# Ashish424/G.P.U-PathTracer

Hardware: AMD Instinct MI355X
Metric: Mrays/sec, cornell_dragon 1920x1080 (+ achieved GB/s against the memory roofline) (higher is better)
Workload: dtype f32; 1 GPU; cornell_dragon_800k (800032 tris) 1920x1080 depth 4 diff + reference 8-sphere room, 16 spp per step; kernel=auto, parallelism=1 GPU, closed_scene=True

## Files before the change

g.p.u-pathtracer_amd/_abi.py:

```python
import ctypes as C
import os

_HERE = os.path.dirname(os.path.abspath(__file__))
PTMI_PATH = os.environ.get("PT_LIBPTMI") or os.path.join(_HERE, "csrc", "libptmi.so")
PTHOST_PATH = os.path.join(_HERE, "host", "libpthost.so")


class Camera(C.Structure):
    _fields_ = [("pos", C.c_float * 3), ("front", C.c_float * 3), ("right", C.c_float * 3),
                ("up", C.c_float * 3), ("dist", C.c_float), ("aspect", C.c_float),
                ("fov", C.c_float), ("_pad", C.c_float)]


class Sphere(C.Structure):
    _fields_ = [("pos_rad", C.c_float * 4), ("emi", C.c_float * 3), ("col", C.c_float * 3),
                ("mat", C.c_int32)]


class Material(C.Structure):
    _fields_ = [("col", C.c_float * 3), ("emi", C.c_float * 3), ("mat", C.c_int32), ("phong_expo", C.c_float)]


class DenoiseParams(C.Structure):
    _fields_ = [("width", C.c_int32), ("height", C.c_int32), ("iterations", C.c_int32),
                ("sigma_color", C.c_float), ("sigma_normal", C.c_float), ("sigma_position", C.c_float)]


class TemporalParams(C.Structure):
    _fields_ = [("width", C.c_int32), ("height", C.c_int32), ("max_history", C.c_float),
                ("plane_tolerance", C.c_float), ("normal_threshold", C.c_float), ("_pad", C.c_int32)]


class Environment(C.Structure):
    _fields_ = [("width", C.c_int32), ("height", C.c_int32), ("front", C.c_float * 3), ("right", C.c_float * 3),
                ("up", C.c_float * 3), ("scale", C.c_float * 3), ("filter", C.c_int32), ("_pad", C.c_int32)]


class CheckpointInfo(C.Structure):
    _fields_ = [("width", C.c_int32), ("height", C.c_int32), ("next_frame", C.c_uint64),
                ("constant_pdf", C.c_uint64), ("scene_tag", C.c_uint64)]


class Params(C.Structure):
    _fields_ = [("width", C.c_int32), ("height", C.c_int32), ("depth", C.c_uint32),
                ("cull_backfaces", C.c_int32), ("frame", C.c_uint64), ("sample_index", C.c_uint64),
                ("tri_mat", C.c_int32), ("tri_col", C.c_float * 3), ("tri_emi", C.c_float * 3),
                ("bk_color", C.c_float * 3), ("air_ior", C.c_float), ("glass_ior", C.c_float),
                ("phong_expo", C.c_float), ("flags", C.c_uint32),
                ("part_index", C.c_int32), ("part_count", C.c_int32), ("part_rows", C.c_int32),
                ("_pad", C.c_int32)]


class Counters(C.Structure):
    _fields_ = [("rays", C.c_uint64), ("inner", C.c_uint64), ("tris", C.c_uint64),
                ("leaves", C.c_uint64), ("hits", C.c_uint64), ("paths", C.c_uint64)]


class BuildParams(C.Structure):
    _fields_ = [("max_leaf_size", C.c_int32), ("min_leaf_size", C.c_int32), ("max_depth", C.c_int32),
                ("n_bins", C.c_int32), ("sah_node_cost", C.c_float), ("sah_tri_cost", C.c_float),
                ("split_alpha", C.c_float), ("n_spatial_bins", C.c_int32), ("optimize_passes", C.c_int32)]


class BvhStats(C.Structure):
    _fields_ = [("n_inner", C.c_uint64), ("n_leaves", C.c_uint64), ("n_tri_refs", C.c_uint64),
                ("max_depth", C.c_uint32), ("sah_cost", C.c_float), ("build_ms", C.c_double),
                ("opt_cost_before", C.c_float), ("opt_cost_after", C.c_float)]


MAT_DIFF, MAT_METAL, MAT_SPEC, MAT_REFR = 0, 1, 2, 3
FLAG_METAL_LITERAL_W = 1 << 0
FLAG_WRITE_RGBA = 1 << 1
FLAG_FACE_FORWARD, FLAG_COSINE_DIFF, FLAG_GLASS_FIX, FLAG_RUSSIAN_ROULETTE, FLAG_MISS_KEEPS_PATH = 1 << 2, 1 << 3, 1 << 4, 1 << 5, 1 << 6
FLAG_RR_CPU_TRACER = 1 << 7
FLAG_NEE = 1 << 8
FLAGS_SMALLPT = FLAG_FACE_FORWARD | FLAG_COSINE_DIFF | FLAG_RUSSIAN_ROULETTE | FLAG_MISS_KEEPS_PATH
FLAGS_CPU_TRACER = FLAG_FACE_FORWARD | FLAG_COSINE_DIFF | FLAG_RR_CPU_TRACER | FLAG_MISS_KEEPS_PATH
RAYS_CLAMPED, RAYS_HDR = 0, 1
ENV_NEAREST, ENV_BILINEAR = 0, 1
KERNEL_AUTO, KERNEL_MEGA_BVH2, KERNEL_PERSISTENT, KERNEL_WAVEFRONT = 0, 1, 3, 5
OPT_KERNEL, OPT_COUNTERS, OPT_TIMING, OPT_BATCH, OPT_TOP_NODES, OPT_OCCUPANCY, OPT_LDS_STACK, OPT_WALK, OPT_LEAF_MAX, OPT_TRI_TEST, OPT_REFILL, OPT_VOTE_NODE, OPT_VOTE_REC, OPT_WAVE_BATCH, OPT_SPHERE_LDS, OPT_BUILD_ALGO, OPT_REBUILD, OPT_PRESPLIT, OPT_WAVE_BLOCKS, OPT_OVERLAP, OPT_OPTIMIZE, OPT_WAVE_SAMPLES = 1, 2, 3, 4, 5, 6, 7, 8, 9, 10, 11, 12, 13, 14, 15, 16, 17, 18, 19, 21, 24, 25
OPT_FIRST_WALK, OPT_PACKET_STACK, OPT_FUSE_STAGES, OPT_LAST_ANYHIT = 26, 27, 28, 29
OPT_ROOT_CULL = 30
OPT_ROOT_ENTRY = 33
OPT_PATH_HISTORY = 34
OPT_ENV_LIGHT = 35

_vp, _sz, _i, _u32 = C.c_void_p, C.c_size_t, C.c_int, C.c_uint32
PTMI_SYMBOLS = [
    ("pt_abi_version", _i, []),
    ("pt_device_count", _i, []),
    ("pt_create", _i, [_i, C.POINTER(_vp)]),
    ("pt_destroy", _i, [_vp]),
    ("pt_last_error", C.c_char_p, [_vp]),
    ("pt_set_stream", _i, [_vp, _vp]),
    ("pt_set_option", _i, [_vp, _i, _i]),
    ("pt_sync", _i, [_vp]),
    ("pt_malloc", _i, [_vp, _sz, C.POINTER(_vp)]),
    ("pt_free", _i, [_vp, _vp]),
    ("pt_memset", _i, [_vp, _vp, _i, _sz]),
    ("pt_download", _i, [_vp, _vp, _vp, _sz]),
    ("pt_upload", _i, [_vp, _vp, _vp, _sz]),
    ("pt_upload_bvh", _i, [_vp, _vp, _sz, _vp, _sz, _vp, _sz]),
    ("pt_upload_spheres", _i, [_vp, C.POINTER(Sphere), _sz]),
    ("pt_render", _i, [_vp, _vp, _vp, C.POINTER(Camera), C.POINTER(Params), _u32]),
    ("pt_render_moments", _i, [_vp, _vp, _vp, _vp, C.POINTER(Camera), C.POINTER(Params), _u32]),
    ("pt_frame_error", _i, [_vp, _vp, C.c_int32, C.c_int32, C.c_uint64, C.c_float, C.POINTER(C.c_double), C.POINTER(C.c_uint64)]),
    ("pt_trace_rays", _i, [_vp, _vp, _sz, _i, _vp, _vp, _vp]),
    ("pt_closest_hits", _i, [_vp, _vp, _sz, _i, _vp, _vp, _vp]),
    ("pt_any_hits", _i, [_vp, _vp, _sz, _i, _vp]),
    ("pt_render_rays", _i, [_vp, _vp, _sz, C.c_uint64, _vp, C.POINTER(Params), _u32, _i]),
    ("pt_upload_environment", _i, [_vp, C.POINTER(Environment), _vp]),
    ("pt_eval_environment", _i, [_vp, _vp, _sz, _vp]),
    ("pt_environment_is_light", _i, [_vp, C.POINTER(_i)]),
    ("pt_sample_environment", _i, [_vp, _vp, _sz, _vp, _vp]),
    ("pt_environment_pdf", _i, [_vp, _vp, _sz, _vp]),
    ("pt_render_aux", _i, [_vp, C.POINTER(Camera), C.POINTER(Params), _vp, _vp, _vp, _vp]),
    ("pt_denoise", _i, [_vp, C.POINTER(DenoiseParams), _vp, _vp, _vp, _vp, _vp, _vp]),
    ("pt_temporal", _i, [_vp, C.POINTER(TemporalParams), C.POINTER(Camera), _vp, _vp, _vp, _vp, _vp, _vp, _vp, _vp, _vp, _vp, _vp, _vp]),
    ("pt_build_bvh", _i, [_vp, _vp, C.c_size_t, _vp, C.c_size_t]),
    ("pt_last_build_ms", _i, [_vp, C.POINTER(C.c_float)]),
    ("pt_refit_bvh", _i, [_vp, _vp, _sz, _vp]),
    ("pt_upload_tri_materials", _i, [_vp, C.POINTER(Material), C.c_size_t, C.POINTER(C.c_int32), C.c_size_t]),
    ("pt_get_counters", _i, [_vp, C.POINTER(Counters)]),
    ("pt_get_wave_stats", _i, [_vp, C.POINTER(C.c_uint64), _i]),
    ("pt_last_kernel_ms", _i, [_vp, C.POINTER(C.c_float)]),
    ("pt_get_stage_ms", _i, [_vp, C.POINTER(C.c_float), _i]),
    ("pt_auto_choice", _i, [_vp, C.POINTER(C.c_int), C.POINTER(C.c_float), C.POINTER(C.c_float)]),
    ("pt_tree_cost", _i, [_vp, C.POINTER(C.c_double), C.POINTER(C.c_double)]),
    ("pt_tree_items", _i, [_vp, C.POINTER(_vp), C.POINTER(C.c_uint64), C.POINTER(C.c_uint64), C.POINTER(C.c_uint64), C.POINTER(C.c_uint32)]),
    ("pt_scene_info", _i, [_vp, C.POINTER(C.c_uint64), C.POINTER(C.c_uint64), C.POINTER(C.c_uint64),
                           C.POINTER(C.c_uint32), C.POINTER(C.c_uint64)]),
]

PTHOST_SYMBOLS = [
    ("pth_last_error", C.c_char_p, []),
    ("pth_default_build_params", None, [C.POINTER(BuildParams)]),
    ("pth_mesh_create", _vp, [_vp, _sz, _vp, _sz]),
    ("pth_mesh_load_obj", _vp, [C.c_char_p]),
    ("pth_mesh_load_ptmesh", _vp, [C.c_char_p]),
    ("pth_mesh_append", _i, [_vp, _vp, _vp]),
    ("pth_mesh_n_verts", _sz, [_vp]),
    ("pth_mesh_n_tris", _sz, [_vp]),
    ("pth_mesh_verts", _vp, [_vp]),
    ("pth_mesh_tris", _vp, [_vp]),
    ("pth_mesh_bounds", None, [_vp, C.POINTER(C.c_float * 3), C.POINTER(C.c_float * 3)]),
    ("pth_mesh_save_ptmesh", _i, [_vp, C.c_char_p]),
    ("pth_mesh_n_materials", _sz, [_vp]),
    ("pth_mesh_materials", _vp, [_vp]),
    ("pth_mesh_tri_materials", _vp, [_vp]),
    ("pth_mesh_set_materials", _i, [_vp, C.POINTER(Material), _sz, _vp]),
    ("pth_mesh_free", None, [_vp]),
    ("pth_bvh_build", _vp, [_vp, C.POINTER(BuildParams)]),
    ("pth_bvh_nodes", _vp, [_vp]),
    ("pth_bvh_n_node_vec4", _sz, [_vp]),
    ("pth_bvh_tris", _vp, [_vp]),
    ("pth_bvh_n_tri_vec4", _sz, [_vp]),
    ("pth_bvh_index", _vp, [_vp]),
    ("pth_bvh_n_index", _sz, [_vp]),
    ("pth_bvh_get_stats", None, [_vp, C.POINTER(BvhStats)]),
    ("pth_bvh_free", None, [_vp]),
    ("pth_write_ppm", _i, [C.c_char_p, _vp, _i, _i]),
    ("pth_write_png", _i, [C.c_char_p, _vp, _i, _i]),
    ("pth_write_pfm", _i, [C.c_char_p, _vp, _i, _i]),
    ("pth_read_pfm", _i, [C.c_char_p, C.POINTER(_i), C.POINTER(_i), C.POINTER(_vp)]),
    ("pth_free_pfm", None, [_vp]),
    ("pth_checkpoint_save", _i, [C.c_char_p, C.POINTER(CheckpointInfo), _vp]),
    ("pth_checkpoint_load", _i, [C.c_char_p, C.POINTER(CheckpointInfo), _vp]),
    ("pth_frame_hash", C.c_uint64, [C.c_uint64]),
]


def _load(path, symbols):
    if not os.path.exists(path):
        raise ImportError(f"{path} is missing - run `python -c 'import __graft_entry__ as g; g.build()'` "
                          "(there is no CPU or PyTorch fallback for the path tracer)")
    lib = C.CDLL(path, mode=C.RTLD_GLOBAL)
    for name, res, args in symbols:
        fn = getattr(lib, name)
        fn.restype = res
        fn.argtypes = args
    return lib


_ptmi = None
_pthost = None


def ptmi():
    global _ptmi
    if _ptmi is None:
        _ptmi = _load(PTMI_PATH, PTMI_SYMBOLS)
    return _ptmi


def pthost():
    global _pthost
    if _pthost is None:
        _pthost = _load(PTHOST_PATH, PTHOST_SYMBOLS)
    return _pthost
```

g.p.u-pathtracer_amd/csrc/pt_ctx.h:

```cpp
#pragma once
#include <hip/hip_runtime.h>

#include <algorithm>
#include <climits>
#include <cstdint>
#include <cstring>
#include <string>
#include <type_traits>
#include <vector>

#include "../../include/ptmi.h"
#include "pt_kernels.h"

#ifndef PT_FIRST_WALK_DEFAULT
#define PT_FIRST_WALK_DEFAULT 1
#endif

struct TreeState {
    float4* d_nodes = nullptr;
    bool records_woop = false;
    bool has_bvh = false;
    uint64_t wide_root = 0;
    uint64_t n_wide = 0, n_inner = 0, n_refs = 0, n_leaves = 0, scene_bytes = 0;
    uint32_t wide_top_layout = 0, wide_depth = 0;
    uint32_t n_top_layout = 0;
    uint32_t max_depth = 0;
    int32_t max_tri_id = -1;
    float build_ms = -1.f;
    double opt_cost[2] = {0.0, 0.0};
};

struct DevTree {
    TreeState s;
    DevTree() = default;
    DevTree(DevTree&& o) noexcept : s(o.release()) {}
    DevTree& operator=(DevTree&& o) noexcept {
        if (this != &o) { (void)hipFree(s.d_nodes); s = o.release(); }
        return *this;
    }
    ~DevTree() { (void)hipFree(s.d_nodes); }
    TreeState release() { const TreeState r = s; s = TreeState(); return r; }
};

struct pt_ctx {
    int device = 0;
    hipStream_t own_stream = nullptr;
    hipStream_t stream = nullptr;
    hipEvent_t switch_ev = nullptr;
    std::string err;
    TreeState tree;
    pt_sphere_d* d_spheres = nullptr;
    int* d_tri_matid = nullptr;
    float4* d_mat_table = nullptr;
    size_t n_tri_matid = 0;
    std::vector<int32_t> emissive_ids;
    int32_t* d_light_slot = nullptr;
    float4* d_tri_lights = nullptr;
    uint64_t mat_gen = 0, lights_key = ~0ull;
    uint64_t lights_geom = 0;
    hipEvent_t lights_ev = nullptr;
    uint64_t lights_gen = 0;
    int n_spheres = 0;
    pt_sphere_d h_spheres[PT_KSPHERES];
    KEnv env = {};
    uint64_t env_gen = 0;
    int opt_kernel = PT_KERNEL_AUTO;
    int opt_counters = 0;
    int opt_timing = 0;
    unsigned long long* d_counters = nullptr;
    unsigned int* d_queue = nullptr;
    float* d_samples = nullptr;
    size_t samples_bytes = 0;
    int n_cu = 0;
    int opt_batch = 36;
    int opt_presplit = 0;
    int opt_optimize = 0;
    int opt_rebuild = 0;
    int opt_build_algo = 1;
    int opt_sph_lds = 1;
    int opt_vote_node = 1, opt_vote_rec = 1;
    int opt_refill = 8;
    int opt_top = 64;
    int opt_occ = 6;
    int opt_lstk = 16;
    int opt_walk = 2;
    int opt_leaf_max = 2;
    int opt_tri_test = 0;
    void* d_wave = nullptr;
    size_t wave_bytes = 0;
    int opt_wave_batch = 16;
    int opt_wave_samples = 16;
    int opt_wave_blocks = 8;
    int opt_first_walk = PT_FIRST_WALK_DEFAULT;
    int opt_packet_stack = PT_PACKET_STACK_MAX;
    int opt_fuse_stages = 1;
    int opt_last_anyhit = 1;
    int opt_root_cull = 1;
    int opt_root_entry = 1;
    int opt_env_light = 0;
    int opt_path_history = 1;
    struct AutoPick {
        static constexpr int TRIALS = 4, PENDING = 4, DECIDED = 5;
        uint64_t key = 0;
        int phase = 0;
        int choice = PT_KERNEL_PERSISTENT;
        hipEvent_t e[2 * TRIALS] = {nullptr, nullptr, nullptr, nullptr, nullptr, nullptr, nullptr, nullptr};
        float ms[2] = {0.f, 0.f};
        uint64_t used = 0;
    };
    static constexpr int N_PICKS = 8;
    AutoPick picks[N_PICKS];
    int pick_last = -1;
    uint64_t pick_tick = 0;
    uint64_t scene_gen = 0;
    uint64_t geom_gen = 0;
    hipEvent_t geom_ev = nullptr;
    struct Refit {
        uint64_t scene_gen = 0;
        const float4* items = nullptr;
        void* d_mem = nullptr;
        int4* bin_list = nullptr;
        int4* wide_list = nullptr;
        float* bin_box = nullptr;
        float* wide_box = nullptr;
        float* rec_box = nullptr;
        uint32_t* first_use = nullptr;
        std::vector<uint32_t> bin_off, wide_off;
    } refit;
    void* d_denoise = nullptr;
    size_t denoise_bytes = 0;
    void* d_frame_err = nullptr;
    size_t frame_err_bytes = 0;
    int opt_overlap = 1;
    struct Side {
        hipStream_t stream = nullptr;
        hipEvent_t traced = nullptr, folded = nullptr;
        bool fold_pending = false;
        float* samples = nullptr;
        size_t samples_bytes = 0;
        unsigned int* queue = nullptr;
        uint64_t lights_seen = 0;
        uint64_t geom_seen = 0;
    } side[2];
    int side_next = 0;
    hipEvent_t ev0 = nullptr, ev1 = nullptr;
    bool timed = false;
    std::vector<hipEvent_t> stage_ev;
    std::vector<int> stage_kind;
    size_t stage_used = 0;
};

namespace ptmi {

extern thread_local std::string g_err;

inline int fail(pt_ctx* c, int code, const std::string& msg) {
    if (c) c->err = msg;
    g_err = msg;
    return code;
}
inline int hip_fail(pt_ctx* c, hipError_t e, const char* what) {
    return fail(c, PT_ERR_DEVICE, std::string(what) + ": " + hipGetErrorString(e));
}

struct DevTemp {
    std::vector<void*> ptrs;
    ~DevTemp() { for (void* p : ptrs) (void)hipFree(p); }
    template <class T> hipError_t get(T** out, size_t count) {
        void* p = nullptr;
        const hipError_t e = hipMalloc(&p, std::max<size_t>(count, 1) * sizeof(T));
        if (e == hipSuccess) ptrs.push_back(p);
        *out = (T*)p;
        return e;
    }
};

inline size_t lds_fit(int& n_top, int stack_n, int block) {
    const size_t stack = (size_t)stack_n * block * 4;
    while (n_top > 0 && (size_t)n_top * 64 + stack > 160 * 1024) n_top /= 2;
    return (size_t)n_top * 64 + stack;
}

template <typename K>
hipError_t allow_lds(K kernel, size_t bytes) {
    return hipFuncSetAttribute((const void*)kernel, hipFuncAttributeMaxDynamicSharedMemorySize, (int)bytes);
}

inline bool wide_walk_fits(const TreeState& t, int cap) { return t.has_bvh && 3 * t.wide_depth + 2 <= (uint32_t)cap; }
inline int choose_walk(pt_ctx* c, const char* who, bool postponed) {
    const bool wide_ok = wide_walk_fits(c->tree, PT_STACK_CAP);
    if (c->tree.has_bvh && c->tree.records_woop)
        return wide_ok ? 3 : fail(c, PT_ERR_UNSUPPORTED, std::string(who) + ": Woop records need the wide walk and this tree is too deep for it");
    const int walk = c->opt_walk == 4 && !postponed ? 2 : c->opt_walk;
    return walk >= 2 && !wide_ok ? 1 : walk;
}
inline bool path_history_holds(const KParams& P) {
    if ((P.flags & (PT_FLAG_NEE | PT_FLAG_RUSSIAN_ROULETTE | PT_FLAG_RR_CPU_TRACER)) || P.tri_matid || P.sc.n_spheres > PT_KSPHERES ||
        P.tri_mat == PT_MAT_REFR || P.depth > PT_HIST_MAX_DEPTH)
        return false;
    for (int i = 0; i < P.sc.n_spheres; i++)
        if (P.ksph[i].mat == PT_MAT_REFR) return false;
    return true;
}
inline void scene_view(const pt_ctx* c, KScene& sc, pt_sphere_d* ksph = nullptr) {
    sc = KScene();
    sc.nodes = sc.tris = c->tree.d_nodes;
    sc.has_bvh = c->tree.has_bvh ? 1 : 0;
    sc.wide_root = (int)c->tree.wide_root;
    if (!ksph) return;
    sc.spheres = c->d_spheres; sc.n_spheres = c->n_spheres;
    std::memcpy(ksph, c->h_spheres, sizeof c->h_spheres);
}
inline size_t binary_ray_layout(const pt_ctx* c, KScene& sc) {
    sc.stack_n = PT_STACK_CAP; sc.top_base = 0;
    sc.n_top = (int)std::min<uint32_t>((uint32_t)c->opt_top, c->tree.n_top_layout);
    return lds_fit(sc.n_top, sc.stack_n, PT_BLOCK_RAYS);
}
constexpr size_t QUEUE_BYTES = PT_SHARDS * PT_SHARD_STRIDE * sizeof(unsigned int);
inline hipError_t queue_alloc(unsigned int** q) { return hipMalloc((void**)q, QUEUE_BYTES); }
inline hipError_t queue_reset(unsigned int* q, hipStream_t st) { return hipMemsetAsync(q, 0, QUEUE_BYTES, st); }
inline int queue_chunk(const pt_ctx* c, uint64_t slots) {
    const uint64_t waves = (uint64_t)c->n_cu * 20;
    return slots / 64 >= 4 * waves ? 64 : (slots / 32 >= 4 * waves ? 32 : 16);
}
inline void queue_params(const pt_ctx* c, unsigned int* queue, KParams& P) {
    P.queue = queue; P.batch = c->opt_batch;
    P.refill = std::min(c->opt_refill, c->opt_batch);
    P.vote_node = c->opt_vote_node; P.vote_rec = c->opt_vote_rec;
}
inline int lds_sphere_table(size_t& lds) { lds += 15 * PT_KSPHERES * 4; return (int)(lds / 4) - 15 * PT_KSPHERES; }
inline hipError_t span_begin(pt_ctx* c) { return c->opt_timing ? hipEventRecord(c->ev0, c->stream) : hipSuccess; }
inline hipError_t span_end(pt_ctx* c) {
    const hipError_t e = c->opt_timing ? hipEventRecord(c->ev1, c->stream) : hipSuccess;
    if (c->opt_timing && e == hipSuccess) c->timed = true;
    return e;
}

template <int V> constexpr std::integral_constant<int, V> int_c{};
template <class F>
auto with_bool(bool v, F&& f) { return v ? f(std::true_type{}) : f(std::false_type{}); }
template <int V0, int... Vs, class F>
auto with_int(int v, F&& f) {
    if constexpr (sizeof...(Vs) == 0) return f(int_c<V0>);
    else return v == V0 ? f(int_c<V0>) : with_int<Vs...>(v, f);
}

template <class K, class... A>
hipError_t launch_resident(K kernel, size_t lds, int max_per_cu, int n_cu, size_t work_cap, hipStream_t st, const A&... args) {
    int per_cu = 0;
    const hipError_t e = allow_lds(kernel, lds);
    if (e != hipSuccess) return e;
    if (hipOccupancyMaxActiveBlocksPerMultiprocessor(&per_cu, kernel, PT_BLOCK, lds) != hipSuccess || per_cu < 1) per_cu = 1;
    per_cu = std::min(per_cu, max_per_cu);
    hipLaunchKernelGGL(kernel, dim3((unsigned)std::min<size_t>((size_t)per_cu * n_cu, work_cap)), dim3(PT_BLOCK), lds, st, args...);
    return hipGetLastError();
}

struct LaunchCfg {
    bool count;
    int occ;
    int lstk;
    int walk;
    size_t lds;
    int blocks;
    int work_blocks;
    int n_cu;
    bool moments;
    int env;
};
hipError_t launch_mega(const LaunchCfg& L, const KParams& P, hipStream_t st);
hipError_t launch_rays(const KScene& sc, size_t lds, const float4* rays, size_t n, int cull, float* t_out, int* tri_out,
                       float* n_out, hipStream_t st);
hipError_t launch_persist(const LaunchCfg& L, const KParams& P, hipStream_t st);
hipError_t launch_fold(const KParams& P, float2* moments, hipStream_t st);
int render_wavefront(pt_ctx* c, KParams& P, const LaunchCfg& L, int work_tiles, bool& folded);
inline uint32_t wave_sample_group_log2(uint32_t spp, int cap) {
    for (int k = 6; k >= 2; k--)
        if ((1 << k) <= cap && (spp & ((1u << k) - 1u)) == 0u) return (uint32_t)k;
    return 0u;
}
int wave_reserve(pt_ctx* c, const KParams& P, int work_tiles);
struct QueryCall {
    const float* rays;
    size_t n;
    int cull;
    float* t;
    int32_t* tri;
    float* normal;
    uint8_t* hit;
};
hipError_t launch_query(pt_ctx* c, const QueryCall& q);
struct RaysCall {
    const float* rays;
    float* out;
    uint64_t first_index;
    size_t n;
    int hdr;
};
hipError_t launch_render_rays(const pt_ctx* c, int walk, bool nee, size_t lds, int work_blocks, const KParams& P, const RaysCall& r);
hipError_t launch_fold_rays(const pt_ctx* c, const KParams& P, const RaysCall& r);
int stage_mark(pt_ctx* c, int kind_of_work_since_last_mark);
int build_bvh_impl(pt_ctx* c, const float* verts, size_t n_verts, const int32_t* tris, size_t n_tris, DevTree& out,
                   const int32_t* id_map = nullptr);
void refit_release(pt_ctx* c);
void denoise_release(pt_ctx* c);
void env_release(pt_ctx* c);

}

#define HIP_TRY(ctx, call)                                                \
    do {                                                                  \
        hipError_t e_ = (call);                                           \
        if (e_ != hipSuccess) return ptmi::hip_fail((ctx), e_, #call);    \
    } while (0)
```

g.p.u-pathtracer_amd/csrc/pt_k_wave.hip:

```cpp
#include "pt_ctx.h"

__device__ __forceinline__ int wf_block_rank(bool keep, int& total, int* s_cnt) {
    const unsigned long long m = __ballot(keep);
    const int w = threadIdx.x >> 6;
    const int in_wave = (int)__builtin_amdgcn_mbcnt_hi((uint32_t)(m >> 32), __builtin_amdgcn_mbcnt_lo((uint32_t)m, 0u));
    if ((threadIdx.x & 63) == 0) s_cnt[w] = __popcll(m);
    __syncthreads();
    int base = 0, tot = 0;
#pragma unroll
    for (int k = 0; k < PT_BLOCK / 64; k++) {
        const int c = s_cnt[k];
        if (k < w) base += c;
        tot += c;
    }
    total = tot;
    return base + in_wave;
}

constexpr int WF_TRI_ROW = 15 * PT_KSPHERES - 4;
template <bool HIST = false>
__device__ __forceinline__ void wf_sphere_table() {
    if (threadIdx.x < 11 * PT_KSPHERES) {
        PT_KARGS(K);
        const float v = ((const __attribute__((address_space(4))) float*)&K.ksph[0])[threadIdx.x];
        ((float*)s_dyn)[threadIdx.x] = v;
        if (threadIdx.x % 11 < 4) ((float*)s_dyn)[88 + 4 * (threadIdx.x / 11) + threadIdx.x % 11] = v;
    }
    if (HIST && threadIdx.x >= 128 && threadIdx.x < 134) {
        PT_KARGS(K);
        const int k = (int)threadIdx.x - 128;
        ((float*)s_dyn)[WF_TRI_ROW + (k < 3 ? 7 + k : 1 + k)] = ((const __attribute__((address_space(4))) float*)&K.tri_col[0])[k];
    }
    __syncthreads();
}

__device__ __forceinline__ const float* wf_history_row(uint32_t code) {
    return (const float*)s_dyn + (code == PT_HIST_TRI ? (uint32_t)WF_TRI_ROW : 11u * code);
}
__device__ __forceinline__ void wf_history_replay(uint32_t word, uint32_t n, v3& mask, v3& accu) {
    mask = V3(1.f, 1.f, 1.f);
    accu = V3(0.f, 0.f, 0.f);
    for (uint32_t k = 0; k < n; k++) {
        const float* t = wf_history_row(pt_hist_code(word, k));
        accu = vadd(accu, vmul(mask, V3(t[4], t[5], t[6])));
        mask = vmul(mask, V3(t[7], t[8], t[9]));
    }
}

__global__ void __launch_bounds__(256) k_wf_prepare(const KParams P) {
    for (uint32_t i = threadIdx.x; i < P.spp; i += 256) P.wf.hashes[i] = pt_wang64(P.frame + i);
    for (uint32_t i = threadIdx.x; i < P.wf.queues_words; i += 256) P.wf.queues_all[i] = 0u;
}

__device__ __forceinline__ bool wf_slot_pixel(const KParams& P, uint32_t slot, uint32_t& s_idx, int& px, int& py) {
    if (slot >= P.wf.n_slots) return false;
    return pt_slot_pixel(P, slot, s_idx, px, py);
}

__device__ __forceinline__ float wf_anyhit_start(float ts) {
    return ts < PT_F32_MAX ? __uint_as_float(__float_as_uint(ts) + 1u) : ts;
}

template <bool COUNT, int OCC, int LSTK, bool FIRST, bool ANY = false, bool ENTRY = false>
__global__ void __launch_bounds__(PT_BLOCK, OCC) k_wf_extend(const KParams P) {
    static_assert(!(FIRST && ENTRY), "bounce 0's rays come from the camera: nobody ran their root step");
    const int tid = threadIdx.x;
    const int lane = tid & 63;
    TravOverflow<LSTK> stk_ovf;
    TravStack<LSTK, PT_BLOCK> stk(__builtin_amdgcn_readfirstlane(tid & ~63), stk_ovf);
    const bool cull = P.cull != 0;
    const uint32_t n_regions = (uint32_t)P.wf.n_regions;
    const uint32_t shard_regions = (n_regions + PT_SHARDS - 1) / PT_SHARDS;
    const int batch = P.batch;

    uint32_t next = 0, end = 0;
    bool empty = false;
    int shard = (int)(blockIdx.x & (PT_SHARDS - 1));

    bool live = false;
    uint32_t idx = 0;
    v3 o = V3(0.f, 0.f, 0.f), d = V3(0.f, 0.f, 0.f);
    TravState ts;
    ts.idx = ts.idy = ts.idz = ts.oodx = ts.oody = ts.oodz = 0.f;
    ts.node = PT_SENTINEL; ts.leaf = 0; ts.sp = 0;
    ts.h = pt_no_hit();
    TravCount tc;
    uint32_t n_rays = 0, it_begin = 0, act_begin = 0, it_loop = 0;
    int root_l0 = 0, root_l1 = 0, root_l2 = 0, root_l3 = 0;
    if (ENTRY) {
        const float4 q2 = pt_uld4(P.sc.nodes, P.sc.wide_root + 2), q3 = pt_uld4(P.sc.nodes, P.sc.wide_root + 3);
        root_l0 = __float_as_int(q2.z); root_l1 = __float_as_int(q2.w);
        root_l2 = __float_as_int(q3.x); root_l3 = __float_as_int(q3.y);
    }

    for (;;) {
        if (COUNT) it_loop++;
        const unsigned long long idle = __ballot(!live);
        const int n_idle = __popcll(idle);
        if (!empty && (n_idle >= batch || n_idle == 64)) {
            const uint32_t rank = __builtin_amdgcn_mbcnt_hi((uint32_t)(idle >> 32), __builtin_amdgcn_mbcnt_lo((uint32_t)idle, 0u));
            uint32_t served = 0;
            for (int round = 0; round < 8 && served < (uint32_t)n_idle; round++) {
                if (next == end) {
                    bool got = false;
                    for (int tries = 0; tries < PT_SHARDS && !got; tries++) {
                        uint32_t k = 0;
                        if (lane == 0) k = atomicAdd(P.wf.queue + shard * PT_SHARD_STRIDE, 1u);
                        k = (uint32_t)__builtin_amdgcn_readfirstlane((int)k);
                        const uint32_t r = k * PT_SHARDS + (uint32_t)shard;
                        if (k < shard_regions && r < n_regions) {
                            next = r * PT_REGION;
                            if (FIRST) end = min(next + (uint32_t)PT_REGION, P.wf.n_slots);
                            else end = next + (uint32_t)__builtin_amdgcn_readfirstlane(P.wf.walk_in[r]);
                            got = true;
                        } else {
                            shard = (shard + 1) & (PT_SHARDS - 1);
                        }
                    }
                    if (!got) { empty = true; break; }
                }
                const uint32_t take = min((uint32_t)n_idle - served, end - next);
                if (!live && rank >= served && rank < served + take) {
                    idx = next + (rank - served);
                    float bound = PT_F32_MAX, b_w = 0.f;
                    if (FIRST) {
                        uint32_t s_idx = 0;
                        int px = 0, py = 0;
                        if (wf_slot_pixel(P, idx, s_idx, px, py)) {
                            PathState ps;
                            path_begin_hashed(P, px, py, (uint64_t)((uint32_t)py * (uint32_t)P.W + (uint32_t)px), P.wf.hashes[s_idx], ps);
                            o = ps.o;
                            d = ps.d;
                            live = true;
                        }
                    } else {
                        const float4 a = pt_sld4(P.wf.ray0_in + idx), b = pt_sld4(P.wf.ray1_in + idx);
                        if (ANY) bound = pt_sld1((const float*)(P.wf.hit + idx));
                        o = V3(a.x, a.y, a.z);
                        d = V3(a.w, b.x, b.y);
                        b_w = b.w;
                        live = true;
                    }
                    if (live) trav_begin(ts, o, d, stk, P.sc.wide_root);
                    if (ANY) ts.h.t = wf_anyhit_start(bound);
                    if constexpr (ENTRY) {
                        const uint32_t code = __float_as_uint(b_w) >> PT_REC_ENTRY_SHIFT, n = pt_entry_count(code);
                        auto link = [&](uint32_t k) {
                            const uint32_t c = pt_entry_child(code, k);
                            return c == 0u ? root_l0 : (c == 1u ? root_l1 : (c == 2u ? root_l2 : root_l3));
                        };
                        if (n == 4u) { ts.sp++; stk.put(ts.sp, link(3)); }
                        if (n >= 3u) { ts.sp++; stk.put(ts.sp, link(2)); }
                        if (n >= 2u) { ts.sp++; stk.put(ts.sp, link(1)); }
                        ts.node = link(0);
                        if (COUNT && ts.node < 0) tc.leaves++;
                    }
                }
                next += take;
                served += take;
            }
            if (COUNT && served) { it_begin++; act_begin += served; }
        }
        const unsigned long long busy = __ballot(live);
        if (!busy) {
            if (empty) break;
            continue;
        }
        const int n_dead = empty ? 64 - __popcll(busy) : 0;
        if (live) {
            const bool fin = trav_run_wide<COUNT, true, false, true, ANY>(ts, P.sc, o, d, cull, stk, tc, n_dead, batch);
            if (fin) {
                if (ANY) { if (ts.h.t == 0.0f) pt_sst1((float*)(P.wf.hit + idx), 0.0f); }
                else pt_sst2(P.wf.hit + idx, make_float2(ts.h.t, __int_as_float(ts.h.rec)));
                live = false;
                if (COUNT) n_rays++;
            }
        }
    }

    if (COUNT) {
        const uint32_t w_ovf = wave_sum_u32(stk.n_ovf), w_rays = ANY ? wave_sum_u32(n_rays) : 0u;
        pt_book_walk<true>(P, lane == 0, n_rays, tc);
        if (lane == 0) {
            if (ANY) atomicAdd(&P.counters[PT_CNT_ANY_RAYS], (unsigned long long)w_rays);
            atomicAdd(&P.counters[PT_CNT_IT_BEGIN], (unsigned long long)it_begin);
            atomicAdd(&P.counters[PT_CNT_ACT_BEGIN], (unsigned long long)act_begin);
            atomicAdd(&P.counters[PT_CNT_IT_LOOP], (unsigned long long)it_loop);
            atomicAdd(&P.counters[PT_CNT_STACK_OVF], (unsigned long long)w_ovf);
        }
    }
}

template <bool COUNT>
__global__ void __launch_bounds__(PT_BLOCK, 8) k_wf_extend_packet(const KParams P) {
    const uint32_t n_groups = P.wf.n_slots / 64u;
    const uint32_t stride = gridDim.x * (uint32_t)(PT_BLOCK / 64);
    TravCount tc;
    uint32_t n_rays = 0, n_walked = 0;
    for (uint32_t group = (uint32_t)__builtin_amdgcn_readfirstlane((int)(blockIdx.x * (PT_BLOCK / 64) + (threadIdx.x >> 6)));
         group < n_groups; group += stride) {
        const uint32_t slot = group * 64u + (threadIdx.x & 63u);
        uint32_t s_idx = 0;
        int px = 0, py = 0;
        v3 o = V3(0.f, 0.f, 0.f), d = V3(0.f, 0.f, 0.f);
        const bool in = wf_slot_pixel(P, slot, s_idx, px, py);
        if (in) {
            PathState ps;
            path_begin_hashed(P, px, py, (uint64_t)((uint32_t)py * (uint32_t)P.W + (uint32_t)px), P.wf.hashes[s_idx], ps);
            o = ps.o;
            d = ps.d;
        }
        const Hit h = trav_packet_wide<COUNT>(P.sc, o, d, P.cull != 0, in, tc);
        if (in) pt_sst2(P.wf.hit + slot, make_float2(h.t, __int_as_float(h.rec)));
        if (COUNT) { n_rays += in ? 1u : 0u; n_walked++; }
    }
    if (COUNT && n_walked) {
        pt_book_walk<true>(P, (threadIdx.x & 63) == 0, n_rays, tc);
        if ((threadIdx.x & 63) == 0) atomicAdd(&P.counters[PT_CNT_PACKET_GROUPS], (unsigned long long)n_walked);
    }
}

#ifndef PT_SURVIVOR_RANK
#define PT_SURVIVOR_RANK(P, alive, ps, total, s_cnt) wf_block_rank(alive, total, s_cnt)
#endif

template <bool FIRST>
__device__ __forceinline__ void wf_shade_miss(float* smp, v3 mask) {
    PT_KARGS(K);
    if (FIRST && (K.flags & PT_FLAG_MISS_KEEPS_PATH)) {
        smp[0] = 0.f + mask.x * K.bk[0]; smp[1] = 0.f + mask.y * K.bk[1]; smp[2] = 0.f + mask.z * K.bk[2];
    } else if (K.flags & PT_FLAG_MISS_KEEPS_PATH) {
        smp[0] += mask.x * K.bk[0]; smp[1] += mask.y * K.bk[1]; smp[2] += mask.z * K.bk[2];
    } else {
        smp[0] = K.bk[0]; smp[1] = K.bk[1]; smp[2] = K.bk[2];
    }
}
__device__ __forceinline__ void wf_shade_miss_history(float* smp, v3 accu, v3 mask) {
    PT_KARGS(K);
    if (K.flags & PT_FLAG_MISS_KEEPS_PATH) pt_sst3(smp, V3(accu.x + mask.x * K.bk[0], accu.y + mask.y * K.bk[1], accu.z + mask.z * K.bk[2]));
    else pt_sst3(smp, V3(K.bk[0], K.bk[1], K.bk[2]));
}
__device__ __forceinline__ void wf_add_emission(float* smp, v3 e) {
    if (!(e.x == 0.f) || !(e.y == 0.f) || !(e.z == 0.f)) {
        smp[0] += e.x; smp[1] += e.y; smp[2] += e.z;
    }
}

template <bool NEE, bool FIRST, bool LAST, bool HIST = false>
__device__ __forceinline__ bool wf_shade_segment(const KParams& P, PathState& ps, const Hit& h, bool tri_hit, float* smp, NeeReq* req, uint32_t& code) {
    static_assert(!(NEE && HIST), "k_wf_resolve adds to the sample colour in place");
    v3 tri_n = V3(0.f, 0.f, 0.f);
    if (!LAST && tri_hit) {
        const float4 q3 = P.sc.nodes[h.rec + 3];
        tri_n = V3(q3.x, q3.y, q3.z);
    }
    const SceneHit sh = pt_closest_sphere(P, ps.o, ps.d, h, 0);
    if (sh.geom == 3) {
        if (HIST) wf_shade_miss_history(smp, ps.accu, ps.mask);
        else wf_shade_miss<FIRST>(smp, ps.mask);
        return false;
    }
    v3 col;
    if (HIST) {
        code = sh.geom == 1 ? (uint32_t)sh.sph_id : PT_HIST_TRI;
        if (LAST) {
            pt_sst3(smp, vadd(ps.accu, path_last_emission(P, ps, h, sh, 0)));
            return false;
        }
        const bool ended = path_shade_hit(P, ps, h, sh, tri_n, col, 0, nullptr);
        if (ended) pt_sst3(smp, FIRST ? V3(0.f + col.x, 0.f + col.y, 0.f + col.z) : col);
        return !ended;
    }
    const bool done = LAST ? true : path_shade_hit(P, ps, h, sh, tri_n, col, 0, NEE ? req : nullptr);
    if (LAST) col = path_last_emission(P, ps, h, sh, 0);
    const v3 e = done ? col : ps.accu;
    if (FIRST) {
        pt_sst3(smp, V3(0.f + e.x, 0.f + e.y, 0.f + e.z));
    } else wf_add_emission(smp, e);
    return !done;
}

template <int LP>
__device__ __forceinline__ void wf_fold_region(const KParams& P, uint32_t region) {
    if (threadIdx.x >= 64) return;
    uint32_t s_idx = 0;
    int px = 0, py = 0;
    const bool in = wf_slot_pixel(P, region * PT_REGION + (threadIdx.x / LP) * (4u * LP), s_idx, px, py);
    pt_fold_pixel_grouped<LP>(P, in, in ? (size_t)py * (size_t)P.W + (size_t)px : 0, (int)(threadIdx.x % LP));
}

__device__ __forceinline__ float2 wf_sphere_bound(const KParams& P, const PathState& ps) {
    const SceneHit sh = pt_closest_sphere(P, ps.o, ps.d, pt_no_hit(), 0);
    return make_float2(sh.t, __int_as_float(sh.sph_id));
}

template <bool BOUND>
__device__ __forceinline__ int wf_survivor_slot(const KParams& P, bool alive, const PathState& ps, float ts, bool& walk_free, int& n_walk,
                                                int& total, int* s_cnt, int* s_cnt_free, uint32_t& entry) {
    walk_free = false;
    entry = 0u;
    if (P.wf.root_cull) {
        const WideNode root = wide_node_load_uniform(P.sc, P.sc.wide_root);
        if (alive) {
            TravState s;
            trav_ray(s, ps.o, ps.d);
            uint32_t key[4];
            wide_node_keys_raw(root, s.idx, s.idy, s.idz, s.oodx, s.oody, s.oodz, BOUND ? wf_anyhit_start(ts) : PT_F32_MAX, key);
            walk_free = (key[0] & key[1] & key[2] & key[3]) == 0xffffffffu;
            if (P.wf.root_entry && !walk_free) {
                wide_sort4(key);
                const uint32_t n = 1u + (key[1] != 0xffffffffu ? 1u : 0u) + (key[2] != 0xffffffffu ? 1u : 0u) + (key[3] != 0xffffffffu ? 1u : 0u);
                entry = pt_entry_pack(n, key[0], key[1], key[2]) << PT_REC_ENTRY_SHIFT;
            }
        }
    }
    const int r = PT_SURVIVOR_RANK(P, alive && !walk_free, ps, n_walk, s_cnt);
    total = n_walk;
    if (!P.wf.root_cull) return r;
    int n_free;
    const int rf = PT_SURVIVOR_RANK(P, walk_free, ps, n_free, s_cnt_free);
    total += n_free;
    return walk_free ? n_walk + rf : r;
}

template <bool COUNT>
__device__ __forceinline__ void wf_region_counts(const KParams& P, uint32_t region, int n_walk, int total) {
    if (threadIdx.x != 0) return;
    P.wf.cnt_out[region] = total;
    P.wf.walk_out[region] = n_walk;
    if (COUNT && total != n_walk) {
        atomicAdd(&P.counters[PT_CNT_RAYS], (unsigned long long)(total - n_walk));
        atomicAdd(&P.counters[PT_CNT_WALK_FREE], (unsigned long long)(total - n_walk));
    }
}

template <bool COUNT, bool NEE, bool FIRST, bool LAST = false, int FOLD = 0, bool BOUND = false, bool HIST = false>
__global__ void __launch_bounds__(PT_BLOCK) k_wf_shade(const KParams P) {
    __shared__ int s_cnt[PT_BLOCK / 64];
    __shared__ int s_cnt2[PT_BLOCK / 64];
    __shared__ int s_cnt_free[PT_BLOCK / 64];
    const uint32_t region = blockIdx.x;
    const int n_in = FIRST ? PT_REGION : P.wf.cnt_in[region];
    const bool last = LAST || P.wf.bounce + 1 >= P.depth;
    if (n_in == 0) {
        if (!last) wf_region_counts<false>(P, region, 0, 0);
        if (NEE && threadIdx.x == 0) P.wf.s_cnt[region] = 0;
        if constexpr (FOLD > 0) wf_fold_region<FOLD>(P, region);
        return;
    }
    wf_sphere_table<HIST>();
    const size_t i = (size_t)region * PT_REGION + threadIdx.x;
    bool have = (int)threadIdx.x < n_in;
    bool alive = false, tri_hit = false;
    uint32_t hist = 0, code = 0;
    PathState ps;
    NeeReq req;
    req.want = false;
    uint32_t pix = 0, s_idx = 0;
    int px = 0, py = 0;
    if (FIRST) have = wf_slot_pixel(P, (uint32_t)i, s_idx, px, py);
    if (have) {
        if (FIRST) {
            pix = (uint32_t)py * (uint32_t)P.W + (uint32_t)px;
            path_begin_hashed(P, px, py, (uint64_t)pix, P.wf.hashes[s_idx], ps);
        } else {
            const float4 a = pt_sld4(P.wf.ray0_in + i), b = pt_sld4(P.wf.ray1_in + i);
            ps.o = V3(a.x, a.y, a.z);
            ps.d = V3(a.w, b.x, b.y);
            pix = __float_as_uint(b.z);
            ps.nee_mask = 0;
            uint32_t sn = __float_as_uint(b.w);
            if (NEE) {
                ps.nee_mask = (pix >> PT_REC_PIXEL_BITS) | ((sn >> PT_REC_LIGHT_BIT) << 8);
                pix &= (1u << PT_REC_PIXEL_BITS) - 1u;
                sn &= (1u << PT_REC_LIGHT_BIT) - 1u;
            } else if (P.wf.root_entry) sn &= (1u << PT_REC_ENTRY_SHIFT) - 1u;
            s_idx = sn >> PT_REC_DRAW_BITS;
            if (HIST) {
                hist = __float_as_uint(pt_sld1(P.wf.mask_in + i));
                wf_history_replay(hist, P.wf.bounce, ps.mask, ps.accu);
            } else {
                ps.mask = V3(pt_sld1(P.wf.mask_in + i), pt_sld1(P.wf.mask_in + (size_t)P.wf.cap + i), pt_sld1(P.wf.mask_in + 2 * (size_t)P.wf.cap + i));
                ps.accu = V3(0.f, 0.f, 0.f);
            }
            ps.depth = P.wf.bounce;
            ps.rng = pt_rng_init(P.wf.hashes[s_idx], (uint64_t)pix);
            ps.rng.n = sn & (PT_REC_MAX_DRAWS - 1u);
        }
        const float2 hh = pt_sld2(P.wf.hit + i);
        Hit h;
        h.t = hh.x;
        h.rec = __float_as_int(hh.y);
        h.tri = -1;
        tri_hit = h.t < PT_F32_MAX;
        if (tri_hit) {
            h.tri = 0;
            if (P.tri_matid) h.tri = __float_as_int(P.sc.nodes[h.rec].w);
        }
        alive = wf_shade_segment<NEE, FIRST, LAST, HIST>(P, ps, h, tri_hit, pt_sample_ptr(P, s_idx, (size_t)pix), &req, code);
    }
    float2 bound = make_float2(PT_F32_MAX, __int_as_float(-1));
    if (BOUND && alive) bound = wf_sphere_bound(P, ps);
    if (COUNT) {
        const uint32_t nh = wave_sum_u32(tri_hit ? 1u : 0u), np = wave_sum_u32(have && !alive ? 1u : 0u);
        if ((threadIdx.x & 63) == 0) {
            atomicAdd(&P.counters[PT_CNT_HITS], (unsigned long long)nh);
            atomicAdd(&P.counters[PT_CNT_PATHS], (unsigned long long)np);
        }
    }
    if (NEE) {
        int n_sh;
        const int rs = wf_block_rank(req.want, n_sh, s_cnt2);
        if (req.want) {
            const size_t j = (size_t)region * PT_REGION + (size_t)rs;
            P.wf.s_ray0[j] = make_float4(req.o.x, req.o.y, req.o.z, req.d.x);
            P.wf.s_ray1[j] = make_float4(req.d.y, req.d.z, __uint_as_float(pix), __uint_as_float(s_idx));
            P.wf.s_con[j] = make_float4(req.contrib.x, req.contrib.y, req.contrib.z, req.t_max);
        }
        if (threadIdx.x == 0) P.wf.s_cnt[region] = n_sh;
    }
    if (last) {
        if constexpr (FOLD > 0) {
            __syncthreads();
            wf_fold_region<FOLD>(P, region);
        }
        return;
    }
    int n_walk, total;
    bool walk_free;
    uint32_t entry;
    const int r = wf_survivor_slot<BOUND>(P, alive, ps, bound.x, walk_free, n_walk, total, s_cnt, s_cnt_free, entry);
    if (alive) {
        const size_t j = (size_t)region * PT_REGION + (size_t)r;
        pt_sst4(P.wf.ray0_out + j, make_float4(ps.o.x, ps.o.y, ps.o.z, ps.d.x));
        pt_sst4(P.wf.ray1_out + j, make_float4(ps.d.y, ps.d.z, __uint_as_float(NEE ? (pix | ((ps.nee_mask & 0xffu) << PT_REC_PIXEL_BITS)) : pix),
                                              __uint_as_float((s_idx << PT_REC_DRAW_BITS) | ps.rng.n | (NEE ? (ps.nee_mask >> 8) << PT_REC_LIGHT_BIT : entry))));
        if (HIST) pt_sst1(P.wf.mask_out + j, __uint_as_float(pt_hist_push(hist, P.wf.bounce, code)));
        else {
            pt_sst1(P.wf.mask_out + j, ps.mask.x);
            pt_sst1(P.wf.mask_out + (size_t)P.wf.cap + j, ps.mask.y);
            pt_sst1(P.wf.mask_out + 2 * (size_t)P.wf.cap + j, ps.mask.z);
        }
        if (BOUND) pt_sst2(P.wf.hit + j, bound);
        else if (walk_free) pt_sst2(P.wf.hit + j, make_float2(pt_no_hit().t, __int_as_float(pt_no_hit().rec)));
    }
    wf_region_counts<COUNT>(P, region, n_walk, total);
}

template <bool COUNT, int FOLD, bool HIST = false>
__global__ void __launch_bounds__(PT_BLOCK) k_wf_shade_last_any(const KParams P) {
    const uint32_t region = blockIdx.x;
    const int n_in = P.wf.cnt_in[region];
    if (n_in == 0) {
        if constexpr (FOLD > 0) wf_fold_region<FOLD>(P, region);
        return;
    }
    wf_sphere_table<HIST>();
    const size_t i = (size_t)region * PT_REGION + threadIdx.x;
    const bool have = (int)threadIdx.x < n_in;
    bool tri_hit = false;
    if (have) {
        const float4 b = pt_sld4(P.wf.ray1_in + i);
        const float2 hh = pt_sld2(P.wf.hit + i);
        v3 mask, accu = V3(0.f, 0.f, 0.f);
        if (HIST) wf_history_replay(__float_as_uint(pt_sld1(P.wf.mask_in + i)), P.wf.bounce, mask, accu);
        else mask = V3(pt_sld1(P.wf.mask_in + i), pt_sld1(P.wf.mask_in + (size_t)P.wf.cap + i), pt_sld1(P.wf.mask_in + 2 * (size_t)P.wf.cap + i));
        const uint32_t pix = __float_as_uint(b.z);
        const uint32_t s_idx = (__float_as_uint(b.w) & (P.wf.root_entry ? (1u << PT_REC_ENTRY_SHIFT) - 1u : ~0u)) >> PT_REC_DRAW_BITS;
        float* smp = pt_sample_ptr(P, s_idx, (size_t)pix);
        const int sph = __float_as_int(hh.y);
        tri_hit = hh.x == 0.0f;
        if (HIST) {
            if (tri_hit) pt_sst3(smp, accu);
            else if (sph >= 0) {
                const float* t = (const float*)s_dyn + 11 * sph;
                pt_sst3(smp, vadd(accu, vadd(V3(0.f, 0.f, 0.f), vmul(mask, V3(t[4], t[5], t[6])))));
            } else wf_shade_miss_history(smp, accu, mask);
        } else if (!tri_hit && sph >= 0) {
            const float* t = (const float*)s_dyn + 11 * sph;
            wf_add_emission(smp, vadd(V3(0.f, 0.f, 0.f), vmul(mask, V3(t[4], t[5], t[6]))));
        } else if (!tri_hit) {
            wf_shade_miss<false>(smp, mask);
        }
    }
    if (COUNT) {
        const uint32_t nh = wave_sum_u32(tri_hit ? 1u : 0u), np = wave_sum_u32(have ? 1u : 0u);
        if ((threadIdx.x & 63) == 0) {
            atomicAdd(&P.counters[PT_CNT_HITS], (unsigned long long)nh);
            atomicAdd(&P.counters[PT_CNT_PATHS], (unsigned long long)np);
        }
    }
    if constexpr (FOLD > 0) {
        __syncthreads();
        wf_fold_region<FOLD>(P, region);
    }
}

template <bool BOUND, bool HIST = false>
__global__ void __launch_bounds__(PT_BLOCK, 8) k_wf_extend_packet_shade(const KParams P) {
    __shared__ int s_cnt[PT_BLOCK / 64];
    __shared__ int s_cnt_free[PT_BLOCK / 64];
    wf_sphere_table<HIST>();
    const uint32_t region = blockIdx.x;
    const size_t i = (size_t)region * PT_REGION + threadIdx.x;
    uint32_t s_idx = 0;
    int px = 0, py = 0;
    const bool have = wf_slot_pixel(P, (uint32_t)i, s_idx, px, py);
    const uint32_t pix = (uint32_t)py * (uint32_t)P.W + (uint32_t)px;
    PathState ps;
    ps.o = ps.d = V3(0.f, 0.f, 0.f);
    if (have) path_begin_hashed(P, px, py, (uint64_t)pix, P.wf.hashes[s_idx], ps);
    TravCount tc;
    Hit h = trav_packet_wide<false>(P.sc, ps.o, ps.d, P.cull != 0, have, tc);
    bool alive = false;
    uint32_t code = 0;
    if (have) {
        const bool tri_hit = h.t < PT_F32_MAX;
        if (tri_hit && !P.tri_matid) h.tri = 0;
        alive = wf_shade_segment<false, true, false, HIST>(P, ps, h, tri_hit, pt_sample_ptr(P, s_idx, (size_t)pix), nullptr, code);
    }
    if (P.wf.bounce + 1 >= P.depth) return;
    float2 bound = make_float2(PT_F32_MAX, __int_as_float(-1));
    if (BOUND && alive) bound = wf_sphere_bound(P, ps);
    int n_walk, total;
    bool walk_free;
    uint32_t entry;
    const int r = wf_survivor_slot<BOUND>(P, alive, ps, bound.x, walk_free, n_walk, total, s_cnt, s_cnt_free, entry);
    if (alive) {
        const size_t j = (size_t)region * PT_REGION + (size_t)r;
        pt_sst4(P.wf.ray0_out + j, make_float4(ps.o.x, ps.o.y, ps.o.z, ps.d.x));
        pt_sst4(P.wf.ray1_out + j, make_float4(ps.d.y, ps.d.z, __uint_as_float(pix), __uint_as_float((s_idx << PT_REC_DRAW_BITS) | ps.rng.n | entry)));
        if (HIST) pt_sst1(P.wf.mask_out + j, __uint_as_float(pt_hist_push(0u, 0u, code)));
        else {
            pt_sst1(P.wf.mask_out + j, ps.mask.x);
            pt_sst1(P.wf.mask_out + (size_t)P.wf.cap + j, ps.mask.y);
            pt_sst1(P.wf.mask_out + 2 * (size_t)P.wf.cap + j, ps.mask.z);
        }
        if (BOUND) pt_sst2(P.wf.hit + j, bound);
        else if (walk_free) pt_sst2(P.wf.hit + j, make_float2(pt_no_hit().t, __int_as_float(pt_no_hit().rec)));
    }
    wf_region_counts<false>(P, region, n_walk, total);
}

__global__ void __launch_bounds__(PT_BLOCK) k_wf_resolve(const KParams P) {
    const int n_in = P.wf.s_cnt[blockIdx.x];
    if ((int)threadIdx.x >= n_in) return;
    const size_t i = (size_t)blockIdx.x * PT_REGION + threadIdx.x;
    const float4 c = P.wf.s_con[i];
    const float2 hh = P.wf.s_hit[i];
    if (hh.x < c.w) return;
    const float4 b = P.wf.s_ray1[i];
    const uint32_t pix = __float_as_uint(b.z), s_idx = __float_as_uint(b.w);
    float* smp = pt_sample_ptr(P, s_idx, (size_t)pix);
    smp[0] += c.x; smp[1] += c.y; smp[2] += c.z;
}

namespace ptmi {

struct WaveLayout {
    size_t n_regions, cap, b_ray, b_mask, b_hit, b_cnt, b_hash, q_words, b_q, b_nee, need;
    bool nee;
};

static uint32_t draws_per_bounce(uint32_t flags) {
    uint32_t k = (flags & PT_FLAG_COSINE_DIFF) ? 2u : 4u;
    if (flags & PT_FLAG_NEE) k += 3u;
    if (flags & PT_FLAG_RUSSIAN_ROULETTE) k += 1u;
    if (flags & PT_FLAG_RR_CPU_TRACER) k += 1u;
    return k;
}

static int wave_layout(pt_ctx* c, const KParams& P, int work_tiles, WaveLayout& w) {
    if ((uint64_t)P.depth * draws_per_bounce(P.flags) + 2u >= PT_REC_MAX_DRAWS || P.spp >= PT_REC_MAX_SAMPLES)
        return fail(c, PT_ERR_UNSUPPORTED, "pt_render: PT_KERNEL_WAVEFRONT packs < " + std::to_string(PT_REC_MAX_DRAWS) + " RNG draws per path (2 + depth x 4..9, by flags) and < " +
                                           std::to_string(PT_REC_MAX_SAMPLES) + " samples per call into a path record");
    w.n_regions = ((size_t)work_tiles + PT_REGION / 64 - 1) / (PT_REGION / 64);
    w.cap = w.n_regions * PT_REGION;
    if (w.cap >= (1ull << 31)) return fail(c, PT_ERR_INVALID, "pt_render: too many path records for one call");
    w.b_ray = w.cap * 16; w.b_mask = w.cap * 12; w.b_hit = w.cap * 8; w.b_cnt = ((w.n_regions * 4 + 255) / 256) * 256;
    w.b_hash = (((size_t)P.spp * 8 + 255) / 256) * 256;
    w.nee = (P.flags & PT_FLAG_NEE) != 0;
    if (w.nee && P.spp >= PT_REC_MAX_SAMPLES_NEE) return fail(c, PT_ERR_UNSUPPORTED, "pt_render: PT_FLAG_NEE in the stage-split pipeline packs < " + std::to_string(PT_REC_MAX_SAMPLES_NEE) + " samples per call into a path record");
    w.q_words = (size_t)P.depth * (w.nee ? 2 : 1) * PT_SHARDS * PT_SHARD_STRIDE;
    w.b_q = w.q_words * 4;
    w.b_nee = w.nee ? 3 * w.b_ray + w.b_hit + w.b_cnt : 0;
    w.need = 4 * w.b_ray + 2 * w.b_mask + w.b_hit + 4 * w.b_cnt + w.b_hash + w.b_q + w.b_nee;
    return PT_OK;
}

static int wave_reserve(pt_ctx* c, const WaveLayout& w) {
    if (w.need > c->wave_bytes) {
        HIP_TRY(c, hipStreamSynchronize(c->stream));
        (void)hipFree(c->d_wave);
        c->d_wave = nullptr;
        c->wave_bytes = 0;
        HIP_TRY(c, hipMalloc(&c->d_wave, w.need));
        c->wave_bytes = w.need;
    }
    return PT_OK;
}

int wave_reserve(pt_ctx* c, const KParams& P, int work_tiles) {
    WaveLayout w;
    const int rc = wave_layout(c, P, work_tiles, w);
    return rc != PT_OK ? rc : wave_reserve(c, w);
}

struct WaveBuffers {
    float4 *ray0[2], *ray1[2];
    float* mask[2];
    float2* hit;
    int* cnt[2];
    int* walk[2];
    unsigned long long* hashes;
    unsigned int* queues;
    char* nee;
};
static WaveBuffers wave_carve(char* base, const WaveLayout& w) {
    WaveBuffers b;
    for (int g = 0; g < 2; g++) {
        b.ray0[g] = (float4*)(base + g * w.b_ray);
        b.ray1[g] = (float4*)(base + (2 + g) * w.b_ray);
        b.mask[g] = (float*)(base + 4 * w.b_ray + g * w.b_mask);
    }
    base += 4 * w.b_ray + 2 * w.b_mask;
    b.hit = (float2*)base;
    base += w.b_hit;
    b.cnt[0] = (int*)base;
    b.cnt[1] = (int*)(base + w.b_cnt);
    b.walk[0] = (int*)(base + 2 * w.b_cnt);
    b.walk[1] = (int*)(base + 3 * w.b_cnt);
    base += 4 * w.b_cnt;
    b.hashes = (unsigned long long*)base;
    base += w.b_hash;
    b.queues = (unsigned int*)base;
    b.nee = base + w.b_q;
    return b;
}

enum WaveExtend { EXT_CLOSEST, EXT_ANY, EXT_FIRST, EXT_PACKET, EXT_FUSED };
enum WaveShade { SHADE_PLAIN, SHADE_BOUND, SHADE_LAST, SHADE_LAST_ANY, SHADE_NONE };
struct WavePlan {
    bool count, nee, deep_stack;
    bool packet;
    bool fuse_first;
    int fold_lp;
    bool anyhit;
    bool root_cull;
    bool root_entry;
    bool history;
    WaveExtend extend(uint32_t b, uint32_t depth) const {
        if (b == 0) return fuse_first ? EXT_FUSED : packet ? EXT_PACKET : EXT_FIRST;
        return anyhit && b + 1 == depth ? EXT_ANY : EXT_CLOSEST;
    }
    WaveShade shade(uint32_t b, uint32_t depth) const {
        if (b == 0 && fuse_first) return SHADE_NONE;
        if (anyhit && b + 1 >= depth) return SHADE_LAST_ANY;
        if (anyhit && b + 2 == depth) return SHADE_BOUND;
        if (b != 0 && !nee && !count && b + 1 >= depth) return SHADE_LAST;
        return SHADE_PLAIN;
    }
};
static WavePlan wave_plan(const pt_ctx* c, const KParams& P, const LaunchCfg& L, bool nee) {
    WavePlan p;
    p.count = L.count; p.nee = nee; p.deep_stack = L.lstk == 24;
    p.packet = c->opt_first_walk == 1 && wide_walk_fits(c->tree, c->opt_packet_stack);
    const bool fuse = c->opt_fuse_stages != 0 && !nee && !L.count, tri_dark = P.tri_emi[0] == 0.f && P.tri_emi[1] == 0.f && P.tri_emi[2] == 0.f;
    p.fuse_first = fuse && p.packet;
    p.fold_lp = fuse && !L.moments && P.depth >= 2 && P.sgroup_log2 >= 2 && P.sgroup_log2 <= 4 && P.spp == (1u << P.sgroup_log2) ? (int)P.spp / 4 : 0;
    p.anyhit = (L.count ? c->opt_last_anyhit == 2 : c->opt_last_anyhit >= 1) && P.depth >= 2 && !nee && !P.tri_matid && tri_dark &&
               P.sc.n_spheres <= PT_KSPHERES && !c->tree.records_woop;
    p.root_cull = L.count ? c->opt_root_cull == 2 : c->opt_root_cull >= 1;
    p.history = (L.count ? c->opt_path_history == 2 : c->opt_path_history >= 1) && path_history_holds(P);
    p.root_entry = p.root_cull && !nee && P.spp < PT_REC_MAX_SAMPLES_ENTRY && (L.count ? c->opt_root_entry == 2 : c->opt_root_entry >= 1);
    return p;
}

constexpr size_t WF_LDS_SHADE = (15 * PT_KSPHERES + 6) * 4;
static hipError_t launch_extend(const WavePlan& p, WaveExtend kind, const KParams& Q, const LaunchCfg& L, int blocks_per_cu, hipStream_t s) {
    auto plain = [&](auto kernel, size_t n_blk, size_t lds) {
        hipLaunchKernelGGL(kernel, dim3((unsigned)n_blk), dim3(PT_BLOCK), lds, s, Q);
        return hipGetLastError();
    };
    const size_t n_reg = (size_t)Q.wf.n_regions;
    if (kind == EXT_FUSED)
        return with_bool(p.history, [&](auto hist) {
            return p.anyhit && Q.depth == 2 ? plain(k_wf_extend_packet_shade<true, hist()>, n_reg, WF_LDS_SHADE) : plain(k_wf_extend_packet_shade<false, hist()>, n_reg, WF_LDS_SHADE);
        });
    if (kind == EXT_PACKET) {
#ifdef PT_PACKET_RESIDENT_GRID
        const bool resident = true;
#else
        const bool resident = p.count;
#endif
        const size_t n_blk = resident ? std::min<size_t>(n_reg, (size_t)8 * L.n_cu) : n_reg;
        return p.count ? plain(k_wf_extend_packet<true>, n_blk, 0) : plain(k_wf_extend_packet<false>, n_blk, 0);
    }
    return with_bool(p.count, [&](auto count) {
        return with_bool(p.deep_stack, [&](auto deep) {
            constexpr int OCC = deep() ? 6 : 8, LSTK = deep() ? 24 : 16;
            auto go = [&](auto first, auto any, auto entry) {
                return launch_resident(k_wf_extend<count(), OCC, LSTK, first(), any(), entry()>, (size_t)LSTK * PT_BLOCK * 4, blocks_per_cu, L.n_cu,
                                       (size_t)Q.wf.n_regions, s, Q);
            };
            if (kind == EXT_FIRST) return go(std::true_type{}, std::false_type{}, std::false_type{});
            return with_bool(p.root_entry, [&](auto entry) {
                if (kind == EXT_ANY) return go(std::false_type{}, std::true_type{}, entry);
                return go(std::false_type{}, std::false_type{}, entry);
            });
        });
    });
}

static hipError_t launch_shade(const WavePlan& p, WaveShade kind, bool first, const KParams& Q, hipStream_t s) {
    auto go = [&](auto kernel) {
        hipLaunchKernelGGL(kernel, dim3((unsigned)Q.wf.n_regions), dim3(PT_BLOCK), WF_LDS_SHADE, s, Q);
        return hipGetLastError();
    };
    if (p.nee) return with_bool(p.count, [&](auto count) {
        return with_bool(first, [&](auto f) { return go(k_wf_shade<count(), true, f()>); });
    });
    return with_bool(p.history, [&](auto hist) {
        if (p.count) {
            if (kind == SHADE_LAST_ANY) return go(k_wf_shade_last_any<true, 0, hist()>);
            return with_bool(first, [&](auto f) {
                if (kind == SHADE_BOUND) return go(k_wf_shade<true, false, f(), false, 0, true, hist()>);
                return go(k_wf_shade<true, false, f(), false, 0, false, hist()>);
            });
        }
        if (kind == SHADE_LAST_ANY) return with_int<4, 2, 1, 0>(p.fold_lp, [&](auto lp) { return go(k_wf_shade_last_any<false, lp(), hist()>); });
        if (kind == SHADE_LAST) return with_int<4, 2, 1, 0>(p.fold_lp, [&](auto lp) { return go(k_wf_shade<false, false, false, true, lp(), false, hist()>); });
        return with_bool(first, [&](auto f) {
            if (kind == SHADE_BOUND) return go(k_wf_shade<false, false, f(), false, 0, true, hist()>);
            return go(k_wf_shade<false, false, f(), false, 0, false, hist()>);
        });
    });
}

int render_wavefront(pt_ctx* c, KParams& P, const LaunchCfg& L, int work_tiles, bool& folded) {
    folded = false;
    WaveLayout w;
    int rc = wave_layout(c, P, work_tiles, w);
    if (rc == PT_OK) rc = wave_reserve(c, w);
    if (rc != PT_OK) return rc;
    const WaveBuffers buf = wave_carve((char*)c->d_wave, w);
    const WavePlan plan = wave_plan(c, P, L, w.nee);
    folded = plan.fold_lp != 0;
    P.wf.nee = w.nee ? 1 : 0;
    P.wf.root_cull = plan.root_cull ? 1 : 0;
    P.wf.root_entry = plan.root_entry ? 1 : 0;
    if (w.nee) {
        P.wf.s_ray0 = (float4*)buf.nee;
        P.wf.s_ray1 = (float4*)(buf.nee + w.b_ray);
        P.wf.s_con = (float4*)(buf.nee + 2 * w.b_ray);
        P.wf.s_hit = (float2*)(buf.nee + 3 * w.b_ray);
        P.wf.s_cnt = (int*)(buf.nee + 3 * w.b_ray + w.b_hit);
    }

    hipStream_t st = c->stream;
    P.sc.n_top = 0;
    P.sph_tab = 0;
    P.batch = c->opt_wave_batch;
    P.wf.hit = buf.hit;
    P.wf.hashes = buf.hashes;
    P.wf.queues_all = buf.queues;
    P.wf.queues_words = (uint32_t)w.q_words;
    P.wf.cap = (uint32_t)w.cap;
    P.wf.n_regions = (int)w.n_regions;
    P.wf.n_slots = (uint32_t)((size_t)work_tiles * 64);
    P.wf.bounce = 0;
    hipLaunchKernelGGL(k_wf_prepare, dim3(1), dim3(256), 0, st, P);
    HIP_TRY(c, hipGetLastError());
    if (stage_mark(c, PT_STAGE_GENERATE) != PT_OK) return PT_ERR_DEVICE;

    for (uint32_t b = 0; b < P.depth; b++) {
        const int g = (int)(b & 1u);
        P.wf.bounce = b;
        P.wf.ray0_in = buf.ray0[g]; P.wf.ray1_in = buf.ray1[g]; P.wf.mask_in = buf.mask[g]; P.wf.cnt_in = buf.cnt[g]; P.wf.walk_in = buf.walk[g];
        P.wf.ray0_out = buf.ray0[g ^ 1]; P.wf.ray1_out = buf.ray1[g ^ 1]; P.wf.mask_out = buf.mask[g ^ 1]; P.wf.cnt_out = buf.cnt[g ^ 1]; P.wf.walk_out = buf.walk[g ^ 1];
        P.wf.queue = buf.queues + (size_t)b * PT_SHARDS * PT_SHARD_STRIDE;
        HIP_TRY(c, launch_extend(plan, plan.extend(b, P.depth), P, L, c->opt_wave_blocks, st));
        if (stage_mark(c, PT_STAGE_EXTEND) != PT_OK) return PT_ERR_DEVICE;
        const WaveShade shade = plan.shade(b, P.depth);
        if (shade == SHADE_NONE) continue;
        HIP_TRY(c, launch_shade(plan, shade, b == 0, P, st));
        if (stage_mark(c, PT_STAGE_SHADE) != PT_OK) return PT_ERR_DEVICE;
        if (w.nee) {
            KParams S = P;
            S.wf.ray0_in = P.wf.s_ray0; S.wf.ray1_in = P.wf.s_ray1; S.wf.cnt_in = S.wf.walk_in = P.wf.s_cnt; S.wf.hit = P.wf.s_hit;
            S.wf.queue = buf.queues + ((size_t)P.depth + b) * PT_SHARDS * PT_SHARD_STRIDE;
            HIP_TRY(c, launch_extend(plan, EXT_CLOSEST, S, L, c->opt_wave_blocks, st));
            if (stage_mark(c, PT_STAGE_EXTEND) != PT_OK) return PT_ERR_DEVICE;
            hipLaunchKernelGGL(k_wf_resolve, dim3((unsigned)w.n_regions), dim3(PT_BLOCK), 0, st, P);
            HIP_TRY(c, hipGetLastError());
            if (stage_mark(c, PT_STAGE_SHADE) != PT_OK) return PT_ERR_DEVICE;
        }
    }
    return PT_OK;
}

}
```

g.p.u-pathtracer_amd/csrc/pt_kernels.h:

```cpp
#pragma once
#include "pt_math.h"
#include "pt_env.h"
#include "../../include/ptmi.h"

#define PT_BLOCK 256
#define PT_BLOCK_RAYS 256
#define PT_TILE 8
#define PT_MAX_TOP 1024
#define PT_STACK_CAP 72
#define PT_SHARDS 8
#define PT_SHARD_STRIDE 32
#define PT_REGION 256

struct KScene {
    const float4* __restrict__ nodes;
    const float4* __restrict__ tris;
    const pt_sphere_d* __restrict__ spheres;
    int n_spheres;
    int has_bvh;
    int n_top;
    int stack_n;
    int top_base;
    int wide_root;
};

#define PT_KSPHERES 8

constexpr uint32_t PT_REC_DRAW_BITS = 12;
constexpr uint32_t PT_REC_LIGHT_BIT = 31;
constexpr uint32_t PT_REC_PIXEL_BITS = 24;
constexpr uint32_t PT_REC_MAX_DRAWS = 1u << PT_REC_DRAW_BITS, PT_REC_MAX_SAMPLES = 1u << (32 - PT_REC_DRAW_BITS),
                   PT_REC_MAX_SAMPLES_NEE = 1u << (PT_REC_LIGHT_BIT - PT_REC_DRAW_BITS);
constexpr uint32_t PT_REC_ENTRY_BITS = 8, PT_REC_ENTRY_SHIFT = 32 - PT_REC_ENTRY_BITS;
constexpr uint32_t PT_REC_MAX_SAMPLES_ENTRY = 1u << (PT_REC_ENTRY_SHIFT - PT_REC_DRAW_BITS);
constexpr uint32_t pt_entry_pack(uint32_t n, uint32_t c0, uint32_t c1, uint32_t c2) {
    return (c0 & 3u) | ((c1 & 3u) << 2) | ((c2 & 3u) << 4) | ((n - 1u) << 6);
}
constexpr uint32_t pt_entry_count(uint32_t code) { return (code >> 6) + 1u; }
constexpr uint32_t pt_entry_child(uint32_t code, uint32_t k) {
    return k < 3u ? (code >> (2u * k)) & 3u : (code ^ (code >> 2) ^ (code >> 4)) & 3u;
}
constexpr bool pt_entry_round_trips() {
    uint32_t seen = 0;
    for (uint32_t n = 1; n <= 4; n++)
        for (uint32_t s = 0; s < 256; s++) {
            const uint32_t c[4] = {s & 3u, (s >> 2) & 3u, (s >> 4) & 3u, (s >> 6) & 3u};
            bool distinct = true;
            for (uint32_t i = 0; i < n; i++)
                for (uint32_t j = i + 1; j < n; j++) distinct = distinct && c[i] != c[j];
            bool rest_zero = true;
            for (uint32_t i = n; i < 4; i++) rest_zero = rest_zero && c[i] == 0u;
            if (!distinct || !rest_zero) continue;
            const uint32_t code = pt_entry_pack(n, c[0], c[1], c[2]);
            if (code >= (1u << PT_REC_ENTRY_BITS) || pt_entry_count(code) != n) return false;
            for (uint32_t k = 0; k < n; k++)
                if (pt_entry_child(code, k) != c[k]) return false;
            seen++;
        }
    return seen == 64u;
}
static_assert(pt_entry_round_trips(), "the entry code of PT_OPT_ROOT_ENTRY");
constexpr uint32_t PT_HIST_BITS = 4, PT_HIST_TRI = 8, PT_HIST_MAX_DEPTH = 32 / PT_HIST_BITS + 1;
constexpr uint32_t pt_hist_push(uint32_t word, uint32_t bounce, uint32_t code) { return word | (code << (PT_HIST_BITS * bounce)); }
constexpr uint32_t pt_hist_code(uint32_t word, uint32_t bounce) { return (word >> (PT_HIST_BITS * bounce)) & ((1u << PT_HIST_BITS) - 1u); }
constexpr bool pt_hist_round_trips() {
    for (uint32_t b = 0; b + 1 < PT_HIST_MAX_DEPTH; b++)
        for (uint32_t code = 0; code <= PT_HIST_TRI; code++) {
            uint32_t w = 0;
            for (uint32_t k = 0; k < b; k++) w = pt_hist_push(w, k, (code + k) % (PT_HIST_TRI + 1u));
            w = pt_hist_push(w, b, code);
            if (pt_hist_code(w, b) != code) return false;
            for (uint32_t k = 0; k < b; k++)
                if (pt_hist_code(w, k) != (code + k) % (PT_HIST_TRI + 1u)) return false;
        }
    return PT_HIST_TRI >= PT_KSPHERES && PT_HIST_TRI < (1u << PT_HIST_BITS);
}
static_assert(pt_hist_round_trips(), "the history word of PT_OPT_PATH_HISTORY");
struct KWave {
    const float4* __restrict__ ray0_in;
    const float4* __restrict__ ray1_in;
    const float* __restrict__ mask_in;
    float4* __restrict__ ray0_out;
    float4* __restrict__ ray1_out;
    float* __restrict__ mask_out;
    float2* __restrict__ hit;
    const int* __restrict__ walk_in;
    const int* __restrict__ cnt_in;
    int* __restrict__ cnt_out;
    int* __restrict__ walk_out;
    unsigned long long* hashes;
    unsigned int* queue;
    unsigned int* queues_all;
    uint32_t queues_words;
    uint32_t cap;
    int n_regions;
    uint32_t n_slots;
    float4* __restrict__ s_ray0;
    float4* __restrict__ s_ray1;
    float4* __restrict__ s_con;
    float2* __restrict__ s_hit;
    int* __restrict__ s_cnt;
    int nee;
    int root_cull;
    int root_entry;
    uint32_t bounce;
};

struct KParams {
    KScene sc;
    pt_sphere_d ksph[PT_KSPHERES];
    float* __restrict__ accum;
    uint32_t* __restrict__ rgba;
    unsigned long long* counters;
    pt_camera cam;
    int W, H;
    uint32_t depth;
    int cull;
    uint64_t frame, sample_index;
    uint32_t spp;
    int tri_mat;
    float tri_col[3], tri_emi[3], bk[3];
    float air_ior, glass_ior, phong;
    const int* tri_matid;
    const float4* mat_table;
    const float4* tri_lights;
    int n_tri_lights;
    uint32_t flags;
    int tiles_x, tile_rows, n_tiles;
    int part_index, part_count, stripe_tr;
    unsigned int* queue;
    int batch;
    int refill;
    int sph_tab;
    int vote_node, vote_rec;
    int chunk;
    float* __restrict__ samples;
    unsigned long long smp_ss;
    uint32_t smp_ps;
    uint32_t sgroup_log2;
    KWave wf;
};
static_assert(sizeof(KEnv) <= sizeof(KWave) && alignof(KEnv) <= alignof(KWave) && sizeof(KParams) == 872, "KParams must not grow: the map lies over wf");
#define PT_KENV(K) (*(pt_kenv*)&(K).wf)
inline void pt_set_env(KParams& P, const KEnv& e) { __builtin_memcpy(&P.wf, &e, sizeof e); }

__device__ __forceinline__ float* pt_sample_ptr(const KParams& P, uint32_t s, size_t pix) {
    return P.samples + 3 * ((size_t)s * (size_t)P.smp_ss + pix * (size_t)P.smp_ps);
}

struct Hit {
    float t;
    int tri;
    int rec;
};
__device__ __forceinline__ Hit pt_no_hit() {
    Hit h;
    h.t = PT_F32_MAX; h.tri = -1; h.rec = 0;
    return h;
}

__device__ __forceinline__ v3 pt_hit_normal(const KScene& sc, const Hit& h) {
    const float4 q3 = sc.nodes[h.rec + 3];
    return V3(q3.x, q3.y, q3.z);
}

__device__ __forceinline__ bool pt_first_active_lane() {
    const unsigned long long m = __ballot(true);
    return (__ffsll((long long)m) - 1) == (int)(__builtin_amdgcn_mbcnt_hi(~0u, __builtin_amdgcn_mbcnt_lo(~0u, 0u)));
}

struct TravCount {
    uint32_t inner = 0, tris = 0, leaves = 0;
    uint32_t it_node = 0, act_node = 0, it_rec = 0, act_rec = 0;
};

enum {
    PT_CNT_RAYS, PT_CNT_INNER, PT_CNT_TRIS, PT_CNT_LEAVES, PT_CNT_HITS, PT_CNT_PATHS,
    PT_CNT_WAVE, PT_CNT_IT_NODE = PT_CNT_WAVE, PT_CNT_ACT_NODE, PT_CNT_IT_REC, PT_CNT_ACT_REC,
    PT_CNT_IT_SHADE, PT_CNT_ACT_SHADE,
    PT_CNT_IT_BEGIN, PT_CNT_ACT_BEGIN,
    PT_CNT_IT_LOOP, PT_CNT_STACK_OVF,
    PT_CNT_WALK_FREE,
    PT_CNT_N,
    PT_CNT_PACKET_GROUPS = PT_CNT_IT_SHADE,
    PT_CNT_ANY_RAYS = PT_CNT_ACT_SHADE
};
static_assert(PT_CNT_WAVE == sizeof(pt_counters) / sizeof(uint64_t) && PT_CNT_N - PT_CNT_WAVE == PT_WAVE_STATS, "include/ptmi.h");

#include "pt_walks.h"
#include "pt_shade.h"

template <bool COUNT, int ALG, int ENV, class STK>
__device__ __forceinline__ v3 pt_get_sample(const KParams& P, int px, int py, uint64_t pix, uint64_t frame,
                                            STK& stk, const float4* __restrict__ s_top, TravCount& tc,
                                            uint32_t& n_rays, uint32_t& n_hits) {
    PathState ps;
    path_begin(P, px, py, pix, frame, ps);
    const bool cull = P.cull != 0;
    v3 col = V3(0.f, 0.f, 0.f);
    if (P.depth == 0) return col;
    for (;;) {
        Hit h = pt_no_hit();
        if (P.sc.has_bvh) {
            if (ALG >= 2) {
                TravState ts;
                trav_begin(ts, ps.o, ps.d, stk, P.sc.wide_root);
                trav_run_wide<COUNT, false, ALG == 3>(ts, P.sc, ps.o, ps.d, cull, stk, tc, 0, 0);
                h = ts.h;
            } else if (ALG == 1) {
                TravState ts;
                trav_begin(ts, ps.o, ps.d, stk);
                trav_run_unified<COUNT, false, STK>(ts, P.sc, ps.o, ps.d, cull, stk, tc, 0, 0);
                h = ts.h;
            } else {
                h = trav_bvh2<COUNT, true, STK>(P.sc, ps.o, ps.d, cull, stk, tc, s_top);
            }
        }
        if (COUNT) { n_rays++; n_hits += (h.tri != -1); }
        NeeReq req;
        req.want = false;
        const bool done = path_shade<ENV>(P, ps, h, col, -1, (P.flags & PT_FLAG_NEE) ? &req : nullptr);
        int done_v = done ? 1 : 0;
        asm volatile("" : "+v"(done_v));
        if (req.want) {
            Hit h2 = pt_no_hit();
            if (P.sc.has_bvh) {
                TravState ts;
                if (ALG >= 2) {
                    trav_begin(ts, req.o, req.d, stk, P.sc.wide_root);
                    trav_run_wide<COUNT, false, ALG == 3>(ts, P.sc, req.o, req.d, cull, stk, tc, 0, 0);
                } else if (ALG == 1) {
                    trav_begin(ts, req.o, req.d, stk);
                    trav_run_unified<COUNT, false, STK>(ts, P.sc, req.o, req.d, cull, stk, tc, 0, 0);
                } else {
                    trav_begin(ts, req.o, req.d, stk);
                    trav_run<COUNT, false, true, STK>(ts, P.sc, req.o, req.d, cull, stk, tc, 0, 0, s_top);
                }
                h2 = ts.h;
            }
            if (COUNT) n_rays++;
            if (!(h2.t < req.t_max)) {
                ps.accu = vadd(ps.accu, req.contrib);
                if (done) col = vadd(col, req.contrib);
            }
        }
        if (done_v) break;
    }
    return col;
}

__device__ __forceinline__ uint32_t wave_sum_u32(uint32_t v) {
#pragma unroll
    for (int off = 32; off > 0; off >>= 1) v += __shfl_xor(v, off, 64);
    return v;
}

template <bool STEPS>
__device__ __forceinline__ void pt_book_walk(const KParams& P, bool booker, uint32_t n_rays, const TravCount& tc) {
    const uint32_t v[8] = {n_rays, tc.inner, tc.tris, tc.leaves, tc.it_node, tc.act_node, tc.it_rec, tc.act_rec};
    const int word[8] = {PT_CNT_RAYS, PT_CNT_INNER, PT_CNT_TRIS, PT_CNT_LEAVES, PT_CNT_IT_NODE, PT_CNT_ACT_NODE, PT_CNT_IT_REC, PT_CNT_ACT_REC};
    uint32_t sum[8];
#pragma unroll
    for (int k = 0; k < (STEPS ? 8 : 4); k++) sum[k] = wave_sum_u32(v[k]);
    if (!booker) return;
#pragma unroll
    for (int k = 0; k < (STEPS ? 8 : 4); k++) atomicAdd(&P.counters[word[k]], (unsigned long long)sum[k]);
}

__device__ __forceinline__ bool pt_tile_coords(const KParams& P, int tile, int& tx, int& ty) {
    if (tile >= P.n_tiles) return false;
    const int lrow = tile / P.tiles_x;
    tx = tile - lrow * P.tiles_x;
    if (P.part_count > 1) {
        const int k = lrow / P.stripe_tr, within = lrow - k * P.stripe_tr;
        ty = (P.part_index + k * P.part_count) * P.stripe_tr + within;
    } else {
        ty = lrow;
    }
    return ty < P.tile_rows;
}

__device__ __forceinline__ bool pt_slot_pixel(const KParams& P, uint32_t slot, uint32_t& s_idx, int& px, int& py) {
    const uint32_t lg = P.sgroup_log2;
    int wt = (int)(slot >> 6);
    uint32_t k = slot & 63u, s_in = 0u;
    if (lg) {
        const uint32_t g1 = (1u << lg) - 1u;
        s_in = k & g1;
        k = ((uint32_t)wt & g1) * (64u >> lg) + (k >> lg);
        wt >>= lg;
    }
    const uint32_t grp = (uint32_t)(wt / P.n_tiles);
    wt -= (int)grp * P.n_tiles;
    s_idx = (grp << lg) + s_in;
    int tx = 0, ty = 0;
    if (s_idx >= P.spp || !pt_tile_coords(P, wt, tx, ty)) return false;
    if (lg) {
        px = tx * PT_TILE + (int)((k & 1u) | ((k >> 1) & 2u) | ((k >> 2) & 4u));
        py = ty * PT_TILE + (int)(((k >> 1) & 1u) | ((k >> 2) & 2u) | ((k >> 3) & 4u));
    } else {
        px = tx * PT_TILE + (int)(k & 7u);
        py = ty * PT_TILE + (int)((k >> 3) & 7u);
    }
    return px < P.W && py < P.H;
}
```

g.p.u-pathtracer_amd/csrc/pt_refit.hip:

```cpp
#include <cstring>
#include <vector>

#include "pt_ctx.h"
#include "pt_items.h"

#define PTR_BLOCK 256
#define PTR_LEAF_CAP 65535

namespace {

struct RefitArgs {
    float4* items;
    const float* verts;
    uint32_t n_rec;
    uint64_t rec_base;
    uint64_t wide_root;
    float* rec_box;
    float* bin_box;
    float* wide_box;
    const uint32_t* first_use;
    uint32_t* n_dropped;
};

__device__ __forceinline__ void ptr_set_empty(float* b) {
    for (int a = 0; a < 3; a++) { b[a] = 3.402823466e+38f; b[3 + a] = -3.402823466e+38f; }
}
__device__ __forceinline__ bool ptr_empty(const float* b) { return !(b[0] <= b[3]); }
__device__ __forceinline__ void ptr_grow(float* u, const float* b) {
    for (int a = 0; a < 3; a++) { u[a] = fminf(u[a], b[a]); u[3 + a] = fmaxf(u[3 + a], b[3 + a]); }
}
__device__ __forceinline__ void ptr_leaf_box(const float* __restrict__ rec_box, uint64_t j0, int n, float* b) {
    ptr_set_empty(b);
    for (int r = 0; r < n; r++) ptr_grow(b, rec_box + 6 * (j0 + (uint64_t)r));
}
template <int N>
__device__ __forceinline__ void ptr_fill_empty(float (*b)[6], int n) {
    float p[3] = {0.f, 0.f, 0.f};
    bool found = false;
#pragma unroll
    for (int k = 0; k < N; k++)
        if (k < n && !found && !ptr_empty(b[k])) { p[0] = b[k][0]; p[1] = b[k][1]; p[2] = b[k][2]; found = true; }
#pragma unroll
    for (int k = 0; k < N; k++)
        if (k < n && ptr_empty(b[k]))
            for (int a = 0; a < 3; a++) b[k][a] = b[k][3 + a] = p[a];
}

__global__ void __launch_bounds__(PTR_BLOCK) k_refit_records(const RefitArgs A) {
    const uint32_t i = blockIdx.x * PTR_BLOCK + threadIdx.x;
    bool count = false;
    if (i < A.n_rec) {
        float4* r = A.items + A.rec_base + 4 * (size_t)i;
        const int32_t id = __float_as_int(r[0].w), last = __float_as_int(r[1].w);
        float box[6];
        ptr_set_empty(box);
        if (id >= 0) {
            float v[9];
            bool finite = true;
            for (int k = 0; k < 9; k++) {
                v[k] = A.verts[9 * (size_t)id + k];
                finite = finite && fabsf(v[k]) <= 3.0e38f;
            }
            float rec[16];
            if (finite) {
                for (int a = 0; a < 3; a++) {
                    box[a] = fminf(v[a], fminf(v[3 + a], v[6 + a]));
                    box[3 + a] = fmaxf(v[a], fmaxf(v[3 + a], v[6 + a]));
                }
                if (v[0] == 0.f) v[0] = 0.f;
                pt_encode_record(v, v + 3, v + 6, id, last, rec);
            } else {
                const float z[3] = {0.f, 0.f, 0.f};
                pt_encode_record(z, z, z, id, last, rec);
                count = (A.first_use[i >> 5] >> (i & 31)) & 1u;
            }
            for (int k = 0; k < 4; k++) r[k] = make_float4(rec[4 * k], rec[4 * k + 1], rec[4 * k + 2], rec[4 * k + 3]);
        }
        for (int a = 0; a < 6; a++) A.rec_box[6 * (size_t)i + a] = box[a];
    }
    if (A.n_dropped) {
        const unsigned long long m = __ballot(count);
        if ((threadIdx.x & 63) == 0 && m) atomicAdd(A.n_dropped, (uint32_t)__popcll(m));
    }
}

__device__ __forceinline__ void ptr_binary_node(const RefitArgs& A, const int4 e) {
    float4* nd = A.items + 4 * (size_t)e.x;
    const float4 q3 = nd[3];
    const int32_t link[2] = {__float_as_int(q3.x), __float_as_int(q3.y)};
    const int cnt[2] = {e.y, e.z};
    float b[2][6], u[6];
    ptr_set_empty(u);
    for (int k = 0; k < 2; k++) {
        if (link[k] < 0) {
            ptr_leaf_box(A.rec_box, ((uint64_t)(uint32_t)~link[k] - A.rec_base) >> 2, cnt[k], b[k]);
        } else {
            const float* s = A.bin_box + 6 * (size_t)(link[k] >> 2);
            for (int a = 0; a < 6; a++) b[k][a] = s[a];
        }
        if (!ptr_empty(b[k])) ptr_grow(u, b[k]);
    }
    ptr_fill_empty<2>(b, 2);
    nd[0] = make_float4(b[0][0], b[0][3], b[0][1], b[0][4]);
    nd[1] = make_float4(b[1][0], b[1][3], b[1][1], b[1][4]);
    nd[2] = make_float4(b[0][2], b[0][5], b[1][2], b[1][5]);
    for (int a = 0; a < 6; a++) A.bin_box[6 * (size_t)e.x + a] = u[a];
}

__device__ __forceinline__ void ptr_wide_node(const RefitArgs& A, const int4 e) {
    float4* nd = A.items + A.wide_root + 4 * (size_t)e.x;
    const float4 q2 = nd[2], q3 = nd[3];
    const int32_t link[4] = {__float_as_int(q2.z), __float_as_int(q2.w), __float_as_int(q3.x), __float_as_int(q3.y)};
    const int n = e.y;
    const int cnt[4] = {e.z & 0xffff, (int)((uint32_t)e.z >> 16), e.w & 0xffff, (int)((uint32_t)e.w >> 16)};
    float b[4][6], u[6];
    ptr_set_empty(u);
#pragma unroll
    for (int k = 0; k < 4; k++) {
        if (k >= n) continue;
        if (link[k] < 0) {
            ptr_leaf_box(A.rec_box, ((uint64_t)(uint32_t)(~link[k] & ~3) - A.rec_base) >> 2, cnt[k], b[k]);
        } else {
            const float* s = A.wide_box + 6 * (size_t)(((uint64_t)(uint32_t)link[k] - A.wide_root) >> 2);
            for (int a = 0; a < 6; a++) b[k][a] = s[a];
        }
        if (!ptr_empty(b[k])) ptr_grow(u, b[k]);
    }
    ptr_fill_empty<4>(b, n);
    PtBox cb[4];
#pragma unroll
    for (int k = 0; k < 4; k++)
        for (int a = 0; a < 3; a++) { cb[k].lo[a] = b[k][a]; cb[k].hi[a] = b[k][3 + a]; }
    float d[16];
    switch (n) {
        case 1: pt_encode_wide_node(cb, 1, link, d); break;
        case 2: pt_encode_wide_node(cb, 2, link, d); break;
        case 3: pt_encode_wide_node(cb, 3, link, d); break;
        default: pt_encode_wide_node(cb, 4, link, d); break;
    }
    for (int k = 0; k < 4; k++) nd[k] = make_float4(d[4 * k], d[4 * k + 1], d[4 * k + 2], d[4 * k + 3]);
    for (int a = 0; a < 6; a++) A.wide_box[6 * (size_t)e.x + a] = u[a];
}

__global__ void __launch_bounds__(PTR_BLOCK) k_refit_shape(const float4* __restrict__ items, uint64_t n_bin, uint64_t n_rec, uint64_t n_wide,
                                                           int32_t* __restrict__ out) {
    const uint64_t i = (uint64_t)blockIdx.x * PTR_BLOCK + threadIdx.x;
    if (i < n_bin) {
        const float4 q3 = items[4 * i + 3];
        out[2 * i] = __float_as_int(q3.x);
        out[2 * i + 1] = __float_as_int(q3.y);
    } else if (i < n_bin + n_rec) {
        const uint64_t j = i - n_bin;
        const float4* r = items + 4 * n_bin + 4 * j;
        out[2 * i] = __float_as_int(r[0].w);
        out[2 * i + 1] = __float_as_int(r[1].w);
    } else if (i < n_bin + n_rec + n_wide) {
        const uint64_t k = i - n_bin - n_rec;
        const float4* w = items + 4 * (n_bin + n_rec) + 4 * k;
        const float4 q2 = w[2], q3 = w[3];
        int32_t* o = out + 2 * (n_bin + n_rec) + 4 * k;
        o[0] = __float_as_int(q2.z); o[1] = __float_as_int(q2.w); o[2] = __float_as_int(q3.x); o[3] = __float_as_int(q3.y);
    }
}

__global__ void __launch_bounds__(PTR_BLOCK) k_refit_level(const RefitArgs A, const int4* __restrict__ bin, uint32_t n_bin,
                                                           const int4* __restrict__ wide, uint32_t n_wide) {
    const uint32_t i = blockIdx.x * PTR_BLOCK + threadIdx.x;
    if (i < n_bin) ptr_binary_node(A, bin[i]);
    else if (i - n_bin < n_wide) ptr_wide_node(A, wide[i - n_bin]);
}

}

namespace ptmi {

void refit_release(pt_ctx* c) {
    (void)hipFree(c->refit.d_mem);
    c->refit = pt_ctx::Refit();
}

static int refit_prepare(pt_ctx* c) {
    refit_release(c);
    const uint64_t n_bin = c->tree.n_inner, n_rec = c->tree.n_refs, n_wide = c->tree.n_wide;
    const uint64_t rec_base = 4 * n_bin, wide_root = c->tree.wide_root;
    if (n_bin == 0 || n_rec == 0 || n_wide == 0 || wide_root != rec_base + 4 * n_rec || n_rec >= (1ull << 31))
        return fail(c, PT_ERR_UNSUPPORTED, "pt_refit_bvh: the tree on this context lacks the [binary nodes][records][wide nodes] layout");
    std::vector<int32_t> h(2 * (n_bin + n_rec) + 4 * n_wide);
    {
        int32_t* d_shape = nullptr;
        HIP_TRY(c, hipMalloc((void**)&d_shape, h.size() * sizeof(int32_t)));
        const uint64_t n_all = n_bin + n_rec + n_wide;
        hipLaunchKernelGGL(k_refit_shape, dim3((unsigned)((n_all + PTR_BLOCK - 1) / PTR_BLOCK)), dim3(PTR_BLOCK), 0, c->stream, c->tree.d_nodes, n_bin,
                           n_rec, n_wide, d_shape);
        hipError_t e = hipGetLastError();
        if (e == hipSuccess) e = hipMemcpyAsync(h.data(), d_shape, h.size() * sizeof(int32_t), hipMemcpyDeviceToHost, c->stream);
        if (e == hipSuccess) e = hipStreamSynchronize(c->stream);
        (void)hipFree(d_shape);
        if (e != hipSuccess) return hip_fail(c, e, "pt_refit_bvh: reading the tree's shape");
    }
    const int32_t* bl_links = h.data();
    const int32_t* rec_w = h.data() + 2 * n_bin;
    const int32_t* wl_links = h.data() + 2 * (n_bin + n_rec);
    auto bad = [&](const char* why) { return fail(c, PT_ERR_DEVICE, std::string("pt_refit_bvh: malformed tree: ") + why); };
    auto leaf_count = [&](int64_t r) -> int {
        if (r < (int64_t)rec_base || ((r - (int64_t)rec_base) & 3) != 0 || (uint64_t)(r - (int64_t)rec_base) / 4 >= n_rec) return 0;
        uint64_t j = (uint64_t)(r - (int64_t)rec_base) / 4;
        for (int n = 1; n <= PTR_LEAF_CAP && j < n_rec; n++, j++)
            if (rec_w[2 * j + 1] != 0) return n;
        return 0;
    };

    std::vector<int32_t> order{0}, hb(n_bin, -1);
    std::vector<int4> ent{make_int4(0, 0, 0, 0)};
    std::vector<uint8_t> seen(n_bin, 0);
    seen[0] = 1;
    for (size_t k = 0; k < order.size(); k++) {
        const int32_t link[2] = {bl_links[2 * (size_t)order[k]], bl_links[2 * (size_t)order[k] + 1]};
        int cnt[2] = {0, 0};
        for (int i = 0; i < 2; i++) {
            if (link[i] < 0) {
                if (!(cnt[i] = leaf_count((int64_t)(uint32_t)~link[i]))) return bad("binary leaf link");
            } else {
                const uint64_t ch = (uint64_t)link[i] / 4;
                if ((link[i] & 3) || ch >= n_bin || seen[ch]) return bad("binary inner link");
                seen[ch] = 1;
                order.push_back((int32_t)ch);
                ent.push_back(make_int4((int32_t)ch, 0, 0, 0));
            }
        }
        ent[k] = make_int4(order[k], cnt[0], cnt[1], 0);
    }
    int max_h = 0;
    for (size_t k = order.size(); k-- > 0;) {
        int ht = 0;
        for (int32_t l : {bl_links[2 * (size_t)order[k]], bl_links[2 * (size_t)order[k] + 1]})
            if (l >= 0) ht = std::max(ht, hb[(size_t)l / 4] + 1);
        hb[(size_t)order[k]] = ht;
        max_h = std::max(max_h, ht);
    }

    std::vector<int32_t> worder{0}, hw(n_wide, -1);
    std::vector<int4> went;
    std::vector<uint8_t> wseen(n_wide, 0);
    wseen[0] = 1;
    for (size_t k = 0; k < worder.size(); k++) {
        const int32_t* link = wl_links + 4 * (size_t)worder[k];
        int n = 1;
        while (n < 4 && link[n] != link[0]) n++;
        int cnt[4] = {0, 0, 0, 0};
        for (int i = 0; i < n; i++) {
            if (link[i] < 0) {
                if (!(cnt[i] = leaf_count((int64_t)(uint32_t)(~link[i] & ~3)))) return bad("wide leaf link");
            } else {
                const int64_t off = (int64_t)link[i] - (int64_t)wide_root;
                if (off < 0 || (off & 3) || (uint64_t)off / 4 >= n_wide || wseen[(size_t)off / 4]) return bad("wide inner link");
                wseen[(size_t)off / 4] = 1;
                worder.push_back((int32_t)(off / 4));
            }
        }
        went.push_back(make_int4(worder[k], n, (int32_t)((uint32_t)cnt[0] | (uint32_t)cnt[1] << 16), (int32_t)((uint32_t)cnt[2] | (uint32_t)cnt[3] << 16)));
    }
    for (size_t k = worder.size(); k-- > 0;) {
        const int32_t* link = wl_links + 4 * (size_t)worder[k];
        int ht = 0;
        for (int32_t l : {link[0], link[1], link[2], link[3]})
            if (l >= 0) ht = std::max(ht, hw[(size_t)(((int64_t)l - (int64_t)wide_root) / 4)] + 1);
        hw[(size_t)worder[k]] = ht;
        max_h = std::max(max_h, ht);
    }

    pt_ctx::Refit& R = c->refit;
    auto by_height = [&](const std::vector<int4>& in, const std::vector<int32_t>& ht, std::vector<uint32_t>& off) {
        off.assign((size_t)max_h + 2, 0);
        for (const int4& e : in) off[(size_t)ht[(size_t)e.x] + 1]++;
        for (size_t i = 1; i < off.size(); i++) off[i] += off[i - 1];
        std::vector<uint32_t> pos(off.begin(), off.end() - 1);
        std::vector<int4> out(in.size());
        for (const int4& e : in) out[pos[(size_t)ht[(size_t)e.x]]++] = e;
        return out;
    };
    const std::vector<int4> bl = by_height(ent, hb, R.bin_off), wl = by_height(went, hw, R.wide_off);
    std::vector<uint32_t> first((n_rec + 31) / 32, 0u);
    {
        std::vector<uint8_t> id_seen((size_t)std::max<int32_t>(c->tree.max_tri_id, 0) + 1, 0);
        for (uint64_t j = 0; j < n_rec; j++) {
            const int32_t id = rec_w[2 * j];
            if (id < 0 || id > c->tree.max_tri_id || id_seen[(size_t)id]) continue;
            id_seen[(size_t)id] = 1;
            first[j >> 5] |= 1u << (j & 31);
        }
    }
    auto up16 = [](size_t b) { return (b + 15) & ~(size_t)15; };
    const size_t b_bl = up16(bl.size() * sizeof(int4)), b_wl = up16(wl.size() * sizeof(int4));
    const size_t b_bb = up16(6 * n_bin * sizeof(float)), b_wb = up16(6 * n_wide * sizeof(float)), b_rb = up16(6 * n_rec * sizeof(float));
    const size_t b_fu = up16(first.size() * sizeof(uint32_t));
    char* m = nullptr;
    HIP_TRY(c, hipMalloc((void**)&m, b_bl + b_wl + b_bb + b_wb + b_rb + b_fu));
    R.d_mem = m;
    R.bin_list = (int4*)m; m += b_bl;
    R.wide_list = (int4*)m; m += b_wl;
    R.bin_box = (float*)m; m += b_bb;
    R.wide_box = (float*)m; m += b_wb;
    R.rec_box = (float*)m; m += b_rb;
    R.first_use = (uint32_t*)m;
    HIP_TRY(c, hipMemcpy(R.bin_list, bl.data(), bl.size() * sizeof(int4), hipMemcpyHostToDevice));
    HIP_TRY(c, hipMemcpy(R.wide_list, wl.data(), wl.size() * sizeof(int4), hipMemcpyHostToDevice));
    HIP_TRY(c, hipMemcpy(R.first_use, first.data(), first.size() * sizeof(uint32_t), hipMemcpyHostToDevice));
    R.scene_gen = c->scene_gen;
    R.items = c->tree.d_nodes;
    return PT_OK;
}

}

using namespace ptmi;

extern "C" int pt_refit_bvh(pt_ctx* c, const float* tri_verts_dev, size_t n_tris, uint32_t* n_dropped_dev) {
    if (!c) return fail(nullptr, PT_ERR_INVALID, "null ctx");
    if (!tri_verts_dev) return fail(c, PT_ERR_INVALID, "pt_refit_bvh: null vertex array");
    if (!c->tree.has_bvh) return fail(c, PT_ERR_NO_SCENE, "pt_refit_bvh: no BVH on this context");
    if (c->tree.records_woop) return fail(c, PT_ERR_UNSUPPORTED, "pt_refit_bvh: Woop records are made on the host only (PT_OPT_TRI_TEST 0)");
    if (c->tree.max_tri_id < 0 || n_tris <= (size_t)c->tree.max_tri_id)
        return fail(c, PT_ERR_INVALID, "pt_refit_bvh: n_tris does not cover the triangle ids of the tree");
    HIP_TRY(c, hipSetDevice(c->device));
    pt_ctx::Refit& R = c->refit;
    if (!R.d_mem || R.scene_gen != c->scene_gen || R.items != c->tree.d_nodes) {
        const int rc = refit_prepare(c);
        if (rc != PT_OK) { refit_release(c); return rc; }
    }
    RefitArgs A;
    A.items = c->tree.d_nodes;
    A.verts = tri_verts_dev;
    A.n_rec = (uint32_t)c->tree.n_refs;
    A.rec_base = 4 * c->tree.n_inner;
    A.wide_root = c->tree.wide_root;
    A.rec_box = R.rec_box;
    A.bin_box = R.bin_box;
    A.wide_box = R.wide_box;
    A.first_use = R.first_use;
    A.n_dropped = n_dropped_dev;
    hipStream_t st = c->stream;
    HIP_TRY(c, span_begin(c));
    if (n_dropped_dev) HIP_TRY(c, hipMemsetAsync(n_dropped_dev, 0, sizeof(uint32_t), st));
    hipLaunchKernelGGL(k_refit_records, dim3((A.n_rec + PTR_BLOCK - 1) / PTR_BLOCK), dim3(PTR_BLOCK), 0, st, A);
    for (size_t ht = 0; ht + 1 < R.bin_off.size(); ht++) {
        const uint32_t nb = R.bin_off[ht + 1] - R.bin_off[ht], nw = R.wide_off[ht + 1] - R.wide_off[ht];
        if (nb + nw == 0) continue;
        hipLaunchKernelGGL(k_refit_level, dim3((nb + nw + PTR_BLOCK - 1) / PTR_BLOCK), dim3(PTR_BLOCK), 0, st, A, R.bin_list + R.bin_off[ht], nb,
                           R.wide_list + R.wide_off[ht], nw);
    }
    HIP_TRY(c, hipGetLastError());
    HIP_TRY(c, span_end(c));
    if (!c->geom_ev) HIP_TRY(c, hipEventCreateWithFlags(&c->geom_ev, hipEventDisableTiming));
    HIP_TRY(c, hipEventRecord(c->geom_ev, st));
    c->geom_gen++;
    return PT_OK;
}
```

g.p.u-pathtracer_amd/csrc/pt_tree.hip:

```cpp
#include <cstring>
#include <utility>

#include "pt_ctx.h"
#include "pt_scene_build.h"

using namespace ptmi;

extern "C" __global__ void __launch_bounds__(256) k_tree_cost(const float4* __restrict__ items, uint64_t wide_root, uint32_t n_wide, double* out) {
    const uint32_t i = blockIdx.x * 256u + threadIdx.x;
    double inner = 0.0, leaf = 0.0, root = 0.0;
    if (i < n_wide) {
        const float4* nd = items + wide_root + 4 * (size_t)i;
        const float4 q0 = nd[0], q1 = nd[1], q2 = nd[2], q3 = nd[3];
        const float sc[3] = {q0.w, q3.z, q3.w};
        const uint32_t ql[3] = {__float_as_uint(q1.x), __float_as_uint(q1.y), __float_as_uint(q1.z)};
        const uint32_t qh[3] = {__float_as_uint(q1.w), __float_as_uint(q2.x), __float_as_uint(q2.y)};
        const int link[4] = {__float_as_int(q2.z), __float_as_int(q2.w), __float_as_int(q3.x), __float_as_int(q3.y)};
        float lo[3] = {3.0e38f, 3.0e38f, 3.0e38f}, hi[3] = {-3.0e38f, -3.0e38f, -3.0e38f};
        for (int k = 0; k < 4; k++) {
            float d[3];
            bool used = true;
            for (int a = 0; a < 3; a++) {
                const int l = (int)((ql[a] >> (8 * k)) & 0xffu), h = (int)((qh[a] >> (8 * k)) & 0xffu);
                if (l > h) used = false;
                d[a] = (float)(h - l) * sc[a];
                if (l <= h) { lo[a] = fminf(lo[a], (float)l * sc[a]); hi[a] = fmaxf(hi[a], (float)h * sc[a]); }
            }
            if (!used) continue;
            const double area = 2.0 * ((double)d[0] * d[1] + (double)d[1] * d[2] + (double)d[2] * d[0]);
            if (link[k] >= 0) {
                inner += area;
            } else {
                int n = 0;
                for (size_t r = (size_t)(~link[k] & ~3);; r += 4) {
                    n++;
                    if (__float_as_int(items[r + 1].w) != 0 || n >= 64) break;
                }
                leaf += area * (double)n;
            }
        }
        if (i == 0) {
            const double dx = hi[0] - lo[0], dy = hi[1] - lo[1], dz = hi[2] - lo[2];
            root = 2.0 * (dx * dy + dy * dz + dz * dx);
        }
    }
    __shared__ double s_in[256], s_lf[256];
    s_in[threadIdx.x] = inner; s_lf[threadIdx.x] = leaf;
    __syncthreads();
    for (int off = 128; off > 0; off >>= 1) {
        if ((int)threadIdx.x < off) { s_in[threadIdx.x] += s_in[threadIdx.x + off]; s_lf[threadIdx.x] += s_lf[threadIdx.x + off]; }
        __syncthreads();
    }
    if (threadIdx.x == 0) { out[1 + 2 * (size_t)blockIdx.x] = s_in[0]; out[2 + 2 * (size_t)blockIdx.x] = s_lf[0]; }
    if (i == 0) out[0] = root;
}

namespace ptmi {

static int tree_cost(pt_ctx* c, const TreeState& t, double* node_visits, double* tri_tests) {
    const unsigned n_blocks = (unsigned)((t.n_wide + 255) / 256);
    const size_t n_out = 1 + 2 * (size_t)n_blocks;
    double* d_out = nullptr;
    HIP_TRY(c, hipMalloc((void**)&d_out, n_out * sizeof(double)));
    hipLaunchKernelGGL(k_tree_cost, dim3(n_blocks), dim3(256), 0, c->stream, t.d_nodes, t.wide_root, (uint32_t)t.n_wide, d_out);
    hipError_t e = hipGetLastError();
    std::vector<double> h(n_out, 0.0);
    if (e == hipSuccess) e = hipMemcpyAsync(h.data(), d_out, n_out * sizeof(double), hipMemcpyDeviceToHost, c->stream);
    if (e == hipSuccess) e = hipStreamSynchronize(c->stream);
    (void)hipFree(d_out);
    if (e != hipSuccess) return hip_fail(c, e, "tree cost (k_tree_cost)");
    if (!(h[0] > 0.0)) return fail(c, PT_ERR_INVALID, "tree cost: degenerate root box");
    double inner = 0.0, leaf = 0.0;
    for (unsigned b = 0; b < n_blocks; b++) { inner += h[1 + 2 * (size_t)b]; leaf += h[2 + 2 * (size_t)b]; }
    *node_visits = (h[0] + inner) / h[0];
    *tri_tests = leaf / h[0];
    return PT_OK;
}

static int tree_from_host(pt_ctx* c, ptscene::Tree& X, int32_t max_id, DevTree& out) {
    DevTree made;
    TreeState& t = made.s;
    ptscene::refine(X, (uint32_t)c->opt_leaf_max);
    if (c->opt_optimize > 0 && c->opt_tri_test == 0) {
        double before = 0.0, after = 0.0;
        if (ptscene::optimize(X, c->opt_optimize, 64, before, after)) { t.opt_cost[0] = before; t.opt_cost[1] = after; }
    }
    ptscene::Output O;
    ptscene::emit(X, PT_MAX_TOP, O, c->opt_tri_test == 1);
    const size_t nb = O.bin.size() * sizeof(float), tb = O.rec.size() * sizeof(float), wb = O.wide.size() * sizeof(float);
    if ((nb + tb + wb) / 16 >= (size_t)PT_SENTINEL) return fail(c, PT_ERR_INVALID, "tree from a host hierarchy: too large for 32-bit links");
    HIP_TRY(c, hipSetDevice(c->device));
    HIP_TRY(c, hipMalloc((void**)&t.d_nodes, nb + tb + wb));
    HIP_TRY(c, hipMemcpy(t.d_nodes, O.bin.data(), nb, hipMemcpyHostToDevice));
    HIP_TRY(c, hipMemcpy((char*)t.d_nodes + nb, O.rec.data(), tb, hipMemcpyHostToDevice));
    HIP_TRY(c, hipMemcpy((char*)t.d_nodes + nb + tb, O.wide.data(), wb, hipMemcpyHostToDevice));
    t.records_woop = c->opt_tri_test == 1;
    t.wide_root = O.wide_root_f4;
    t.wide_top_layout = O.n_top_wide;
    t.wide_depth = O.depth_wide;
    t.n_wide = O.wide.size() / 16;
    t.n_top_layout = O.n_top_bin;
    t.n_inner = O.bin.size() / 16;
    t.n_refs = O.n_refs;
    t.n_leaves = O.n_leaves;
    t.max_depth = O.depth_bin;
    t.scene_bytes = nb + tb + wb;
    t.max_tri_id = max_id;
    t.has_bvh = true;
    out = std::move(made);
    return PT_OK;
}

static int optimise_device_tree(pt_ctx* c, DevTree& tree, const float* soup, const int32_t* ids, size_t n) {
    const TreeState& in = tree.s;
    if (c->opt_optimize <= 0 || in.records_woop) return PT_OK;
    std::vector<const float*> by_id((size_t)in.max_tri_id + 1, nullptr);
    for (size_t k = 0; k < n; k++) by_id[ids ? (size_t)ids[k] : k] = soup + 9 * k;
    std::vector<float> bin(16 * (size_t)in.n_inner), rec(16 * (size_t)in.n_refs);
    HIP_TRY(c, hipSetDevice(c->device));
    HIP_TRY(c, hipStreamSynchronize(c->stream));
    HIP_TRY(c, hipMemcpy(bin.data(), in.d_nodes, bin.size() * sizeof(float), hipMemcpyDeviceToHost));
    HIP_TRY(c, hipMemcpy(rec.data(), (const char*)in.d_nodes + bin.size() * sizeof(float), rec.size() * sizeof(float), hipMemcpyDeviceToHost));
    ptscene::Tree X;
    std::string why;
    if (!ptscene::from_items(bin.data(), (size_t)in.n_inner, rec.data(), (size_t)in.n_refs, by_id, X, why))
        return fail(c, PT_ERR_DEVICE, "device-built tree: " + why);
    const float device_ms = in.build_ms;
    const int rc = tree_from_host(c, X, in.max_tri_id, tree);
    if (rc == PT_OK) tree.s.build_ms = device_ms;
    return rc;
}

static int adopt_tree(pt_ctx* c, DevTree&& t) {
    HIP_TRY(c, hipSetDevice(c->device));
    HIP_TRY(c, hipStreamSynchronize(c->stream));
    refit_release(c);
    (void)hipFree(c->tree.d_nodes);
    c->tree = t.release();
    c->scene_gen++;
    return PT_OK;
}
}

extern "C" {

int pt_upload_bvh(pt_ctx* c, const float* nodes, size_t n_node_vec4, const float* tri_verts, size_t n_tri_vec4,
                  const int32_t* tri_index, size_t n_index) {
    if (!c) return fail(nullptr, PT_ERR_INVALID, "null ctx");
    if (!nodes || !tri_verts || !tri_index) return fail(c, PT_ERR_INVALID, "pt_upload_bvh: null array");
    if (n_node_vec4 < 4 || (n_node_vec4 % 4) != 0) return fail(c, PT_ERR_INVALID, "pt_upload_bvh: node array must hold whole 4-vec4 nodes");
    if (n_index != n_tri_vec4) return fail(c, PT_ERR_INVALID, "pt_upload_bvh: index array must parallel the triangle array");
    if (n_node_vec4 * 16 >= (size_t)PT_SENTINEL || n_tri_vec4 >= (size_t)0x7fffffff)
        return fail(c, PT_ERR_INVALID, "pt_upload_bvh: scene too large for 32-bit links");

    ptscene::Tree T;
    std::string perr;
    if (!ptscene::parse(nodes, n_node_vec4, tri_verts, n_tri_vec4, tri_index, T, perr))
        return fail(c, PT_ERR_INVALID, "pt_upload_bvh: " + perr);
    int32_t max_id = -1;
    for (const ptscene::Ref& r : T.refs) max_id = std::max(max_id, r.id);
    if (c->d_tri_matid && (size_t)max_id >= c->n_tri_matid)
        return fail(c, PT_ERR_INVALID, "pt_upload_bvh: the triangle-material array on this context does not cover this BVH's triangle ids (clear or re-upload it first)");
    const int rebuild = c->opt_tri_test == 0 ? c->opt_rebuild : 0;
    std::vector<int32_t> ids;
    std::vector<float> verts;
    if (rebuild) {
        std::vector<const ptscene::Ref*> sorted;
        sorted.reserve(T.refs.size());
        for (const ptscene::Ref& r : T.refs) sorted.push_back(&r);
        std::sort(sorted.begin(), sorted.end(), [](const ptscene::Ref* a, const ptscene::Ref* b) { return a->id < b->id; });
        for (const ptscene::Ref* r : sorted) {
            if (!ids.empty() && ids.back() == r->id) continue;
            ids.push_back(r->id);
            verts.insert(verts.end(), r->v, r->v + 9);
        }
    }
    auto reclustered = [&](DevTree& out) -> int {
        std::vector<int32_t> tri_rows(3 * ids.size());
        for (size_t i = 0; i < tri_rows.size(); i++) tri_rows[i] = (int32_t)i;
        const int rc = build_bvh_impl(c, verts.data(), verts.size() / 3, tri_rows.data(), ids.size(), out, ids.data());
        return rc == PT_OK ? optimise_device_tree(c, out, verts.data(), ids.data(), ids.size()) : rc;
    };
    DevTree a;
    int rc = rebuild == 1 ? reclustered(a) : tree_from_host(c, T, max_id, a);
    if (rc != PT_OK) return rc;
    double cost_a = 0.0, cost_b = 0.0, unused = 0.0;
    if (rebuild == 2 && a.s.n_wide > 0 && tree_cost(c, a.s, &cost_a, &unused) == PT_OK) {
        DevTree b;
        if (reclustered(b) == PT_OK && tree_cost(c, b.s, &cost_b, &unused) == PT_OK && cost_b < cost_a) a = std::move(b);
        else c->err.clear();
    }
    return adopt_tree(c, std::move(a));
}

int pt_build_bvh(pt_ctx* c, const float* verts, size_t n_verts, const int32_t* tris, size_t n_tris) {
    if (!c) return fail(nullptr, PT_ERR_INVALID, "null ctx");
    DevTree t;
    int rc = build_bvh_impl(c, verts, n_verts, tris, n_tris, t);
    if (rc == PT_OK && c->opt_optimize > 0 && c->opt_presplit == 0) {
        std::vector<float> flat(9 * n_tris);
        for (size_t i = 0; i < 3 * n_tris; i++) std::memcpy(&flat[3 * i], verts + 3 * (size_t)tris[i], 3 * sizeof(float));
        rc = optimise_device_tree(c, t, flat.data(), nullptr, n_tris);
    }
    return rc == PT_OK ? adopt_tree(c, std::move(t)) : rc;
}

int pt_last_build_ms(pt_ctx* c, float* ms) {
    if (!c || !ms) return fail(c, PT_ERR_INVALID, "pt_last_build_ms: null argument");
    if (c->tree.build_ms < 0.f) return fail(c, PT_ERR_INVALID, "pt_last_build_ms: the tree on this context was not built on the device");
    *ms = c->tree.build_ms;
    return PT_OK;
}

int pt_scene_info(pt_ctx* c, uint64_t* n_inner, uint64_t* n_refs, uint64_t* n_leaves, uint32_t* max_depth, uint64_t* bytes) {
    if (!c) return fail(nullptr, PT_ERR_INVALID, "null ctx");
    if (!c->tree.has_bvh) return fail(c, PT_ERR_NO_SCENE, "pt_scene_info: no BVH uploaded");
    if (n_inner) *n_inner = c->tree.n_inner;
    if (n_refs) *n_refs = c->tree.n_refs;
    if (n_leaves) *n_leaves = c->tree.n_leaves;
    if (max_depth) *max_depth = c->tree.max_depth;
    if (bytes) *bytes = c->tree.scene_bytes;
    return PT_OK;
}

int pt_tree_cost(pt_ctx* c, double* node_visits, double* tri_tests) {
    if (!c || !node_visits || !tri_tests) return fail(c, PT_ERR_INVALID, "pt_tree_cost: null argument");
    if (!c->tree.has_bvh || c->tree.wide_root == 0 || c->tree.n_wide == 0) return fail(c, PT_ERR_NO_SCENE, "pt_tree_cost: no 4-wide tree on this context");
    if (c->tree.records_woop) return fail(c, PT_ERR_UNSUPPORTED, "pt_tree_cost: reads the Moller-Trumbore records' leaf terminators");
    HIP_TRY(c, hipSetDevice(c->device));
    return tree_cost(c, c->tree, node_visits, tri_tests);
}

int pt_tree_items(pt_ctx* c, const void** items_dev, uint64_t* n_binary, uint64_t* n_records, uint64_t* n_wide, uint32_t* wide_depth) {
    if (!c || !items_dev) return fail(c, PT_ERR_INVALID, "pt_tree_items: null argument");
    if (!c->tree.has_bvh || !c->tree.d_nodes) return fail(c, PT_ERR_NO_SCENE, "pt_tree_items: no BVH on this context");
    HIP_TRY(c, hipSetDevice(c->device));
    HIP_TRY(c, hipStreamSynchronize(c->stream));
    *items_dev = c->tree.d_nodes;
    if (n_binary) *n_binary = c->tree.n_inner;
    if (n_records) *n_records = c->tree.n_refs;
    if (n_wide) *n_wide = c->tree.n_wide;
    if (wide_depth) *wide_depth = c->tree.wide_depth;
    return PT_OK;
}

}
```

g.p.u-pathtracer_amd/csrc/ptmi.hip:

```cpp
#include <hip/hip_runtime.h>

#include <algorithm>
#include <cmath>
#include <cstdio>
#include <cstring>
#include <string>
#include <vector>

#include "pt_ctx.h"

static_assert(sizeof(pt_sphere) == 44, "pt_sphere must match the reference Sphere (44 B)");
static_assert(sizeof(pt_sphere_d) == sizeof(pt_sphere), "device sphere mirror");
static_assert(sizeof(pt_params) == 104 && sizeof(pt_camera) == 64 && sizeof(pt_counters) == 48, "ABI struct sizes (tests/test_host_and_abi.py)");

namespace ptmi {
thread_local std::string g_err;
}
using namespace ptmi;

namespace ptmi {
static bool auto_decide(pt_ctx* c, pt_ctx::AutoPick& a, bool wait) {
    using AP = pt_ctx::AutoPick;
    if (a.phase != AP::PENDING) return a.phase == AP::DECIDED;
    for (int t = 0; t < AP::TRIALS; t++) {
        const hipError_t e = wait ? hipEventSynchronize(a.e[2 * t + 1]) : hipEventQuery(a.e[2 * t + 1]);
        if (e != hipSuccess) { (void)hipGetLastError(); return false; }
    }
    float best[2] = {3.0e38f, 3.0e38f};
    bool ok = true;
    for (int t = 0; t < AP::TRIALS; t++) {
        float ms = 0.f;
        ok = ok && hipEventElapsedTime(&ms, a.e[2 * t], a.e[2 * t + 1]) == hipSuccess;
        best[t & 1] = std::min(best[t & 1], ms);
    }
    a.ms[0] = best[0]; a.ms[1] = best[1];
    a.choice = ok && a.ms[1] < a.ms[0] ? PT_KERNEL_WAVEFRONT : PT_KERNEL_PERSISTENT;
    a.phase = AP::DECIDED;
    bool wave_wanted = false;
    for (const AP& o : c->picks)
        if (o.key && (o.phase < AP::DECIDED || o.choice == PT_KERNEL_WAVEFRONT)) wave_wanted = true;
    if (!wave_wanted && c->d_wave) {
        (void)hipFree(c->d_wave);
        c->d_wave = nullptr;
        c->wave_bytes = 0;
    }
    return true;
}

int stage_mark(pt_ctx* c, int kind) {
    if (!c->opt_timing) return PT_OK;
    if (c->stage_used == c->stage_ev.size()) {
        hipEvent_t e = nullptr;
        HIP_TRY(c, hipEventCreate(&e));
        c->stage_ev.push_back(e);
        c->stage_kind.push_back(0);
    }
    HIP_TRY(c, hipEventRecord(c->stage_ev[c->stage_used], c->stream));
    c->stage_kind[c->stage_used] = kind;
    c->stage_used++;
    return PT_OK;
}

struct OptionRow {
    enum Rule { FLAG, RANGE, SET };
    int id;
    int pt_ctx::*field;
    Rule rule;
    int v[4];
    int code;
    const char* msg;
};
static const OptionRow OPTIONS[] = {
    {PT_OPT_KERNEL, &pt_ctx::opt_kernel, OptionRow::SET, {PT_KERNEL_AUTO, PT_KERNEL_MEGA_BVH2, PT_KERNEL_PERSISTENT, PT_KERNEL_WAVEFRONT}, PT_ERR_UNSUPPORTED, "pt_set_option: kernel variant not available in this build"},
    {PT_OPT_COUNTERS, &pt_ctx::opt_counters, OptionRow::FLAG, {}, PT_OK, ""},
    {PT_OPT_TIMING, &pt_ctx::opt_timing, OptionRow::FLAG, {}, PT_OK, ""},
    {PT_OPT_SPHERE_LDS, &pt_ctx::opt_sph_lds, OptionRow::FLAG, {}, PT_OK, ""},
    {PT_OPT_OVERLAP, &pt_ctx::opt_overlap, OptionRow::FLAG, {}, PT_OK, ""},
    {PT_OPT_TOP_NODES, &pt_ctx::opt_top, OptionRow::RANGE, {0, PT_MAX_TOP}, PT_ERR_INVALID, "pt_set_option: top nodes must be 0..1024"},
    {PT_OPT_OCCUPANCY, &pt_ctx::opt_occ, OptionRow::SET, {4, 5, 6, 8}, PT_ERR_INVALID, "pt_set_option: occupancy must be 4, 5 (runs as 6), 6 or 8 waves per SIMD"},
    {PT_OPT_TRI_TEST, &pt_ctx::opt_tri_test, OptionRow::RANGE, {0, 1}, PT_ERR_INVALID, "pt_set_option: tri test must be 0 (Moller-Trumbore) or 1 (Woop)"},
    {PT_OPT_LEAF_MAX, &pt_ctx::opt_leaf_max, OptionRow::RANGE, {0, 1024}, PT_ERR_INVALID, "pt_set_option: leaf_max must be 0 (keep) .. 1024"},
    {PT_OPT_WALK, &pt_ctx::opt_walk, OptionRow::SET, {0, 1, 2, 4}, PT_ERR_INVALID, "pt_set_option: walk must be 0 (while-while), 1 (unified-step), 2 (wide) or 4 (wide, postponed leaf)"},
    {PT_OPT_REBUILD, &pt_ctx::opt_rebuild, OptionRow::RANGE, {0, 2}, PT_ERR_INVALID, "pt_set_option: rebuild must be 0 (keep the hierarchy), 1 (re-cluster) or 2 (keep the cheaper tree)"},
    {PT_OPT_PRESPLIT, &pt_ctx::opt_presplit, OptionRow::RANGE, {0, 100000}, PT_ERR_INVALID, "pt_set_option: presplit must be 0 (off) .. 100000 (per cent of diag/sqrt(n))"},
    {PT_OPT_BUILD_ALGO, &pt_ctx::opt_build_algo, OptionRow::RANGE, {0, 1}, PT_ERR_INVALID, "pt_set_option: build algorithm must be 0 (LBVH) or 1 (PLOC)"},
    {PT_OPT_WAVE_BATCH, &pt_ctx::opt_wave_batch, OptionRow::RANGE, {1, 64}, PT_ERR_INVALID, "pt_set_option: wave batch must be 1..64"},
    {PT_OPT_VOTE_NODE, &pt_ctx::opt_vote_node, OptionRow::RANGE, {1, 64}, PT_ERR_INVALID, "pt_set_option: vote weight must be 1..64"},
    {PT_OPT_VOTE_REC, &pt_ctx::opt_vote_rec, OptionRow::RANGE, {1, 64}, PT_ERR_INVALID, "pt_set_option: vote weight must be 1..64"},
    {PT_OPT_OPTIMIZE, &pt_ctx::opt_optimize, OptionRow::RANGE, {0, 16}, PT_ERR_INVALID, "pt_set_option: optimize passes must be 0 (off) .. 16"},
    {PT_OPT_WAVE_SAMPLES, &pt_ctx::opt_wave_samples, OptionRow::RANGE, {1, 64}, PT_ERR_INVALID, "pt_set_option: wave samples must be 1 (one sample of a tile per wave) .. 64"},
    {PT_OPT_WAVE_BLOCKS, &pt_ctx::opt_wave_blocks, OptionRow::RANGE, {1, 8}, PT_ERR_INVALID, "pt_set_option: wave blocks must be 1..8 per CU"},
    {PT_OPT_LDS_STACK, &pt_ctx::opt_lstk, OptionRow::SET, {0, 16, 24, 24}, PT_ERR_INVALID, "pt_set_option: LDS stack must be 0 (all 72 entries in LDS), 16 or 24 entries"},
    {PT_OPT_REFILL, &pt_ctx::opt_refill, OptionRow::RANGE, {1, 64}, PT_ERR_INVALID, "pt_set_option: refill must be 1..64"},
    {PT_OPT_BATCH, &pt_ctx::opt_batch, OptionRow::RANGE, {1, 64}, PT_ERR_INVALID, "pt_set_option: batch must be 1..64"},
    {PT_OPT_FIRST_WALK, &pt_ctx::opt_first_walk, OptionRow::RANGE, {0, 1}, PT_ERR_INVALID, "pt_set_option: first walk must be 0 (per lane) or 1 (wave-wide packets)"},
    {PT_OPT_PACKET_STACK, &pt_ctx::opt_packet_stack, OptionRow::RANGE, {2, PT_PACKET_STACK_MAX}, PT_ERR_INVALID, "pt_set_option: packet stack must be 2..72 entries"},
    {PT_OPT_FUSE_STAGES, &pt_ctx::opt_fuse_stages, OptionRow::RANGE, {0, 1}, PT_ERR_INVALID, "pt_set_option: fuse stages must be 0 (separate launches) or 1"},
    {PT_OPT_LAST_ANYHIT, &pt_ctx::opt_last_anyhit, OptionRow::RANGE, {0, 2}, PT_ERR_INVALID, "pt_set_option: last any-hit must be 0 (off), 1 (product launches) or 2 (instrumented launches too)"},
    {PT_OPT_ROOT_CULL, &pt_ctx::opt_root_cull, OptionRow::RANGE, {0, 2}, PT_ERR_INVALID, "pt_set_option: root cull must be 0 (off), 1 (product launches) or 2 (instrumented launches too)"},
    {PT_OPT_ROOT_ENTRY, &pt_ctx::opt_root_entry, OptionRow::RANGE, {0, 2}, PT_ERR_INVALID, "pt_set_option: root entry must be 0 (off), 1 (product launches) or 2 (instrumented launches too)"},
    {PT_OPT_ENV_LIGHT, &pt_ctx::opt_env_light, OptionRow::RANGE, {0, 1}, PT_ERR_INVALID, "pt_set_option: env light must be 0 (the map is no light) or 1 (sampled under PT_FLAG_NEE)"},
    {PT_OPT_PATH_HISTORY, &pt_ctx::opt_path_history, OptionRow::RANGE, {0, 2}, PT_ERR_INVALID, "pt_set_option: path history must be 0 (off), 1 (product launches) or 2 (instrumented launches too)"},
};
}

extern "C" {

int pt_abi_version(void) { return PTMI_ABI_VERSION; }

int pt_device_count(void) {
    int n = 0;
    hipError_t e = hipGetDeviceCount(&n);
    if (e != hipSuccess) { g_err = std::string("hipGetDeviceCount: ") + hipGetErrorString(e); return PT_ERR_DEVICE; }
    return n;
}

const char* pt_last_error(const pt_ctx* ctx) { return ctx ? ctx->err.c_str() : g_err.c_str(); }

int pt_create(int device, pt_ctx** out) {
    if (!out) return fail(nullptr, PT_ERR_INVALID, "pt_create: out is null");
    *out = nullptr;
    int n = 0;
    hipError_t e = hipGetDeviceCount(&n);
    if (e != hipSuccess) return hip_fail(nullptr, e, "hipGetDeviceCount");
    if (device < 0 || device >= n) return fail(nullptr, PT_ERR_INVALID, "pt_create: no such device");
    pt_ctx* c = new pt_ctx();
    c->device = device;
    if ((e = hipSetDevice(device)) != hipSuccess) { delete c; return hip_fail(nullptr, e, "hipSetDevice"); }
    if ((e = hipStreamCreateWithFlags(&c->own_stream, hipStreamNonBlocking)) != hipSuccess) { delete c; return hip_fail(nullptr, e, "hipStreamCreate"); }
    c->stream = c->own_stream;
    if ((e = hipMalloc(&c->d_counters, PT_CNT_N * sizeof(unsigned long long))) != hipSuccess) { pt_destroy(c); return hip_fail(nullptr, e, "hipMalloc"); }
    if ((e = hipMemset(c->d_counters, 0, PT_CNT_N * sizeof(unsigned long long))) != hipSuccess) { pt_destroy(c); return hip_fail(nullptr, e, "hipMemset"); }
    if ((e = queue_alloc(&c->d_queue)) != hipSuccess) { pt_destroy(c); return hip_fail(nullptr, e, "hipMalloc"); }
    hipDeviceProp_t prop;
    if ((e = hipGetDeviceProperties(&prop, device)) != hipSuccess) { pt_destroy(c); return hip_fail(nullptr, e, "hipGetDeviceProperties"); }
    c->n_cu = prop.multiProcessorCount;
    if ((e = hipEventCreate(&c->ev0)) != hipSuccess || (e = hipEventCreate(&c->ev1)) != hipSuccess) { pt_destroy(c); return hip_fail(nullptr, e, "hipEventCreate"); }
    *out = c;
    return PT_OK;
}

int pt_destroy(pt_ctx* c) {
    if (!c) return PT_OK;
    (void)hipSetDevice(c->device);
    if (c->stream) (void)hipStreamSynchronize(c->stream);
    (void)hipFree(c->tree.d_nodes);
    (void)hipFree(c->d_spheres);
    (void)hipFree(c->d_tri_matid);
    (void)hipFree(c->d_mat_table);
    (void)hipFree(c->d_light_slot);
    (void)hipFree(c->d_tri_lights);
    (void)hipFree(c->d_counters);
    (void)hipFree(c->d_queue);
    (void)hipFree(c->d_samples);
    (void)hipFree(c->d_wave);
    refit_release(c);
    denoise_release(c);
    for (pt_ctx::Side& s : c->side) {
        if (s.stream) (void)hipStreamSynchronize(s.stream);
        (void)hipFree(s.samples);
        (void)hipFree(s.queue);
        if (s.traced) (void)hipEventDestroy(s.traced);
        if (s.folded) (void)hipEventDestroy(s.folded);
        if (s.stream) (void)hipStreamDestroy(s.stream);
    }
    env_release(c);
    for (hipEvent_t e : c->stage_ev) (void)hipEventDestroy(e);
    for (pt_ctx::AutoPick& a : c->picks)
        for (hipEvent_t e : a.e) if (e) (void)hipEventDestroy(e);
    if (c->lights_ev) (void)hipEventDestroy(c->lights_ev);
    if (c->geom_ev) (void)hipEventDestroy(c->geom_ev);
    if (c->switch_ev) (void)hipEventDestroy(c->switch_ev);
    if (c->ev0) (void)hipEventDestroy(c->ev0);
    if (c->ev1) (void)hipEventDestroy(c->ev1);
    if (c->own_stream) (void)hipStreamDestroy(c->own_stream);
    delete c;
    return PT_OK;
}

int pt_set_stream(pt_ctx* c, void* s) {
    if (!c) return fail(nullptr, PT_ERR_INVALID, "null ctx");
    hipStream_t next = s ? (hipStream_t)s : c->own_stream;
    if (next != c->stream) {
        HIP_TRY(c, hipSetDevice(c->device));
        if (!c->switch_ev) HIP_TRY(c, hipEventCreateWithFlags(&c->switch_ev, hipEventDisableTiming));
        HIP_TRY(c, hipEventRecord(c->switch_ev, c->stream));
        HIP_TRY(c, hipStreamWaitEvent(next, c->switch_ev, 0));
    }
    c->stream = next;
    return PT_OK;
}

int pt_set_option(pt_ctx* c, int option, int value) {
    if (!c) return fail(nullptr, PT_ERR_INVALID, "null ctx");
    for (const OptionRow& o : OPTIONS) {
        if (o.id != option) continue;
        bool ok = true;
        if (o.rule == OptionRow::RANGE) ok = value >= o.v[0] && value <= o.v[1];
        if (o.rule == OptionRow::SET) ok = std::find(o.v, o.v + 4, value) != o.v + 4;
        if (!ok) return fail(c, o.code, o.msg);
        c->*o.field = o.rule == OptionRow::FLAG ? value != 0 : value;
        return PT_OK;
    }
    return fail(c, PT_ERR_INVALID, "pt_set_option: unknown option");
}

int pt_sync(pt_ctx* c) {
    if (!c) return fail(nullptr, PT_ERR_INVALID, "null ctx");
    HIP_TRY(c, hipSetDevice(c->device));
    HIP_TRY(c, hipStreamSynchronize(c->stream));
    return PT_OK;
}

int pt_malloc(pt_ctx* c, size_t bytes, void** out) {
    if (!c || !out || bytes == 0) return fail(c, PT_ERR_INVALID, "pt_malloc: bad argument");
    HIP_TRY(c, hipSetDevice(c->device));
    HIP_TRY(c, hipMalloc(out, bytes));
    return PT_OK;
}
int pt_free(pt_ctx* c, void* p) {
    if (!c) return fail(nullptr, PT_ERR_INVALID, "null ctx");
    HIP_TRY(c, hipSetDevice(c->device));
    HIP_TRY(c, hipStreamSynchronize(c->stream));
    HIP_TRY(c, hipFree(p));
    return PT_OK;
}
int pt_memset(pt_ctx* c, void* p, int v, size_t bytes) {
    if (!c || !p) return fail(c, PT_ERR_INVALID, "pt_memset: bad argument");
    HIP_TRY(c, hipSetDevice(c->device));
    HIP_TRY(c, hipMemsetAsync(p, v, bytes, c->stream));
    return PT_OK;
}
int pt_download(pt_ctx* c, void* dst, const void* src, size_t bytes) {
    if (!c || !dst || !src) return fail(c, PT_ERR_INVALID, "pt_download: bad argument");
    HIP_TRY(c, hipSetDevice(c->device));
    HIP_TRY(c, hipMemcpyAsync(dst, src, bytes, hipMemcpyDeviceToHost, c->stream));
    HIP_TRY(c, hipStreamSynchronize(c->stream));
    return PT_OK;
}
int pt_upload(pt_ctx* c, void* dst, const void* src, size_t bytes) {
    if (!c || !dst || !src) return fail(c, PT_ERR_INVALID, "pt_upload: bad argument");
    HIP_TRY(c, hipSetDevice(c->device));
    HIP_TRY(c, hipMemcpyAsync(dst, src, bytes, hipMemcpyHostToDevice, c->stream));
    HIP_TRY(c, hipStreamSynchronize(c->stream));
    return PT_OK;
}

int pt_upload_tri_materials(pt_ctx* c, const pt_material* table, size_t n_materials, const int32_t* tri_material, size_t n_tris) {
    if (!c) return fail(nullptr, PT_ERR_INVALID, "null ctx");
    HIP_TRY(c, hipSetDevice(c->device));
    if (n_materials == 0) {
        HIP_TRY(c, hipStreamSynchronize(c->stream));
        (void)hipFree(c->d_tri_matid); c->d_tri_matid = nullptr;
        (void)hipFree(c->d_mat_table); c->d_mat_table = nullptr;
        (void)hipFree(c->d_light_slot); c->d_light_slot = nullptr;
        (void)hipFree(c->d_tri_lights); c->d_tri_lights = nullptr;
        c->emissive_ids.clear();
        c->n_tri_matid = 0;
        c->mat_gen++;
        return PT_OK;
    }
    if (!table || !tri_material) return fail(c, PT_ERR_INVALID, "pt_upload_tri_materials: null array");
    if (n_materials > (1u << 24) || n_tris >= (size_t)0x7fffffff) return fail(c, PT_ERR_INVALID, "pt_upload_tri_materials: table too large");
    if (c->tree.has_bvh && (size_t)c->tree.max_tri_id >= n_tris && c->tree.max_tri_id >= 0)
        return fail(c, PT_ERR_INVALID, "pt_upload_tri_materials: n_tris does not cover the triangle ids of the uploaded BVH");
    for (size_t i = 0; i < n_materials; i++)
        if (table[i].mat < PT_MAT_DIFF || table[i].mat > PT_MAT_REFR) return fail(c, PT_ERR_INVALID, "pt_upload_tri_materials: bad material type");
    for (size_t i = 0; i < n_tris; i++)
        if (tri_material[i] < 0 || (size_t)tri_material[i] >= n_materials) return fail(c, PT_ERR_INVALID, "pt_upload_tri_materials: material index out of range");
    static_assert(sizeof(pt_material) == 32, "pt_material is two float4 rows");
    HIP_TRY(c, hipStreamSynchronize(c->stream));
    (void)hipFree(c->d_tri_matid); c->d_tri_matid = nullptr;
    (void)hipFree(c->d_mat_table); c->d_mat_table = nullptr;
    c->n_tri_matid = 0;
    HIP_TRY(c, hipMalloc((void**)&c->d_tri_matid, n_tris * sizeof(int32_t)));
    HIP_TRY(c, hipMalloc((void**)&c->d_mat_table, n_materials * sizeof(pt_material)));
    HIP_TRY(c, hipMemcpy(c->d_tri_matid, tri_material, n_tris * sizeof(int32_t), hipMemcpyHostToDevice));
    HIP_TRY(c, hipMemcpy(c->d_mat_table, table, n_materials * sizeof(pt_material), hipMemcpyHostToDevice));
    c->n_tri_matid = n_tris;
    (void)hipFree(c->d_light_slot); c->d_light_slot = nullptr;
    (void)hipFree(c->d_tri_lights); c->d_tri_lights = nullptr;
    c->emissive_ids.clear();
    c->mat_gen++;
    std::vector<int32_t> slot(n_tris, -1);
    for (size_t i = 0; i < n_tris; i++) {
        const pt_material& m = table[tri_material[i]];
        if (!(m.emi[0] == 0.0f && m.emi[1] == 0.0f && m.emi[2] == 0.0f)) {
            slot[i] = (int32_t)c->emissive_ids.size();
            c->emissive_ids.push_back((int32_t)i);
        }
    }
    if (!c->emissive_ids.empty()) {
        HIP_TRY(c, hipMalloc((void**)&c->d_light_slot, n_tris * sizeof(int32_t)));
        HIP_TRY(c, hipMalloc((void**)&c->d_tri_lights, c->emissive_ids.size() * 3 * sizeof(float4)));
        HIP_TRY(c, hipMemcpy(c->d_light_slot, slot.data(), n_tris * sizeof(int32_t), hipMemcpyHostToDevice));
    }
    return PT_OK;
}

__global__ void __launch_bounds__(256) k_collect_tri_lights(const float4* __restrict__ rec, uint32_t n_rec, const int32_t* __restrict__ slot,
                                                            uint32_t n_ids, const int* __restrict__ tri_matid, const float4* __restrict__ mat_table,
                                                            float4* __restrict__ lights) {
    const uint32_t i = blockIdx.x * 256u + threadIdx.x;
    if (i >= n_rec) return;
    const float4 q0 = rec[4 * (size_t)i];
    const int id = __float_as_int(q0.w);
    if (id < 0 || (uint32_t)id >= n_ids) return;
    const int s = slot[id];
    if (s < 0) return;
    const float4 q1 = rec[4 * (size_t)i + 1], q2 = rec[4 * (size_t)i + 2];
    const int row = tri_matid[id];
    const float4 m0 = mat_table[2 * row], m1 = mat_table[2 * row + 1];
    lights[3 * (size_t)s + 0] = make_float4(q0.x, q0.y, q0.z, m0.w);
    lights[3 * (size_t)s + 1] = make_float4(q1.x, q1.y, q1.z, m1.x);
    lights[3 * (size_t)s + 2] = make_float4(q2.x, q2.y, q2.z, m1.y);
}

int pt_upload_spheres(pt_ctx* c, const pt_sphere* spheres, size_t n) {
    if (!c) return fail(nullptr, PT_ERR_INVALID, "null ctx");
    if (n > 0 && !spheres) return fail(c, PT_ERR_INVALID, "pt_upload_spheres: null array");
    if (n > 4096) return fail(c, PT_ERR_INVALID, "pt_upload_spheres: too many spheres");
    for (size_t i = 0; i < n; i++)
        if (spheres[i].mat < PT_MAT_DIFF || spheres[i].mat > PT_MAT_REFR) return fail(c, PT_ERR_INVALID, "pt_upload_spheres: bad material");
    HIP_TRY(c, hipSetDevice(c->device));
    HIP_TRY(c, hipStreamSynchronize(c->stream));
    (void)hipFree(c->d_spheres); c->d_spheres = nullptr;
    c->n_spheres = 0;
    if (n) {
        HIP_TRY(c, hipMalloc((void**)&c->d_spheres, n * sizeof(pt_sphere)));
        HIP_TRY(c, hipMemcpy(c->d_spheres, spheres, n * sizeof(pt_sphere), hipMemcpyHostToDevice));
        c->n_spheres = (int)n;
        std::memcpy(c->h_spheres, spheres, std::min<size_t>(n, PT_KSPHERES) * sizeof(pt_sphere));
    }
    return PT_OK;
}

namespace ptmi {
static int check_call(pt_ctx* c, const float* accum_dev, const uint32_t* rgba_dev, const pt_camera* cam, const pt_params* p, uint32_t spp) {
    if (!c) return fail(nullptr, PT_ERR_INVALID, "null ctx");
    if (!accum_dev || !cam || !p) return fail(c, PT_ERR_INVALID, "pt_render: null argument");
    if (p->width < 2 || p->height < 2) return fail(c, PT_ERR_INVALID, "pt_render: image must be at least 2x2 (the camera divides by w-1, h-1)");
    if (spp == 0) return fail(c, PT_ERR_INVALID, "pt_render: spp must be >= 1");
    if (p->sample_index == 0) return fail(c, PT_ERR_INVALID, "pt_render: sample_index (constantPdf) starts at 1");
    if (p->tri_mat < PT_MAT_DIFF || p->tri_mat > PT_MAT_REFR) return fail(c, PT_ERR_INVALID, "pt_render: bad triangle material");
    if ((p->flags & PT_FLAG_WRITE_RGBA) && !rgba_dev) return fail(c, PT_ERR_INVALID, "pt_render: PT_FLAG_WRITE_RGBA needs rgba_dev");
    if ((p->flags & PT_FLAG_NEE) && !(p->flags & PT_FLAG_COSINE_DIFF)) return fail(c, PT_ERR_INVALID, "pt_render: PT_FLAG_NEE needs PT_FLAG_COSINE_DIFF (the reference's DIFF lobe has no density to weigh a light sample against)");
    if (!c->tree.has_bvh && c->n_spheres == 0) return fail(c, PT_ERR_NO_SCENE, "pt_render: no scene uploaded");
    if (p->part_count > 1) {
        if (p->part_index < 0 || p->part_index >= p->part_count) return fail(c, PT_ERR_INVALID, "pt_render: part_index out of range");
        if (p->part_rows <= 0 || (p->part_rows % PT_TILE) != 0) return fail(c, PT_ERR_INVALID, "pt_render: part_rows must be a positive multiple of 8");
    }
    return PT_OK;
}

static bool samples_tri_lights(const pt_ctx* c, const pt_params* p) {
    return (p->flags & PT_FLAG_NEE) && c->tree.has_bvh && !c->emissive_ids.empty();
}

static int refresh_tri_lights(pt_ctx* c, const pt_params* p) {
    if (!samples_tri_lights(c, p)) return PT_OK;
    if (c->tree.records_woop) return fail(c, PT_ERR_UNSUPPORTED, "pt_render: PT_FLAG_NEE over emissive triangles needs the exact (Moller-Trumbore) records");
    const uint64_t key = (c->scene_gen << 32) ^ c->mat_gen;
    if (c->lights_key == key && c->lights_geom == c->geom_gen) return PT_OK;
    const uint32_t n_rec = (uint32_t)c->tree.n_refs;
    HIP_TRY(c, hipMemsetAsync(c->d_tri_lights, 0, c->emissive_ids.size() * 3 * sizeof(float4), c->stream));
    hipLaunchKernelGGL(k_collect_tri_lights, dim3((n_rec + 255) / 256), dim3(256), 0, c->stream, c->tree.d_nodes + 4 * (size_t)c->tree.n_inner, n_rec,
                       c->d_light_slot, (uint32_t)c->n_tri_matid, c->d_tri_matid, c->d_mat_table, c->d_tri_lights);
    HIP_TRY(c, hipGetLastError());
    c->lights_key = key;
    c->lights_geom = c->geom_gen;
    if (!c->lights_ev) HIP_TRY(c, hipEventCreateWithFlags(&c->lights_ev, hipEventDisableTiming));
    HIP_TRY(c, hipEventRecord(c->lights_ev, c->stream));
    c->lights_gen++;
    return PT_OK;
}

static void fill_path_params(const pt_ctx* c, const pt_params* p, uint32_t spp, KParams& P) {
    std::memset(&P, 0, sizeof P);
    scene_view(c, P.sc, P.ksph);
    P.counters = c->d_counters;
    P.W = p->width; P.H = p->height;
    P.depth = p->depth;
    P.cull = p->cull_backfaces;
    P.frame = p->frame; P.sample_index = p->sample_index; P.spp = spp;
    P.tri_mat = p->tri_mat;
    for (int i = 0; i < 3; i++) { P.tri_col[i] = p->tri_col[i]; P.tri_emi[i] = p->tri_emi[i]; P.bk[i] = p->bk_color[i]; }
    P.air_ior = p->air_ior; P.glass_ior = p->glass_ior; P.phong = p->phong_expo;
    P.tri_matid = c->d_tri_matid;
    P.mat_table = c->d_mat_table;
    P.flags = p->flags;
    if (samples_tri_lights(c, p)) {
        P.tri_lights = c->d_tri_lights;
        P.n_tri_lights = (int)c->emissive_ids.size();
    }
    pt_set_env(P, c->env);
}

static int fill_params(pt_ctx* c, float* accum_dev, uint32_t* rgba_dev, const pt_camera* cam, const pt_params* p, uint32_t spp, KParams& P) {
    fill_path_params(c, p, spp, P);
    P.accum = accum_dev;
    P.rgba = rgba_dev;
    P.cam = *cam;
    P.smp_ss = (unsigned long long)p->width * (unsigned long long)p->height;
    P.smp_ps = 1u;
    P.tiles_x = (p->width + PT_TILE - 1) / PT_TILE;
    P.tile_rows = (p->height + PT_TILE - 1) / PT_TILE;
    if (p->part_count > 1) {
        P.part_index = p->part_index; P.part_count = p->part_count; P.stripe_tr = p->part_rows / PT_TILE;
        const int n_stripes = (P.tile_rows + P.stripe_tr - 1) / P.stripe_tr;
        const int owned = (n_stripes - p->part_index + p->part_count - 1) / p->part_count;
        P.n_tiles = owned * P.stripe_tr * P.tiles_x;
    } else {
        P.part_index = 0; P.part_count = 1; P.stripe_tr = 1;
        P.n_tiles = P.tile_rows * P.tiles_x;
    }
    if (P.n_tiles <= 0) return PT_OK;
    if ((uint64_t)P.n_tiles * 64u * (uint64_t)spp >= (1ull << 31)) return fail(c, PT_ERR_INVALID, "pt_render: width*height*spp too large for one call (split the samples over several calls)");
    return PT_OK;
}

static int auto_lookup(pt_ctx* c, const pt_params* p, uint32_t spp, bool moments, pt_ctx::AutoPick*& pick, int& probe) {
    using AP = pt_ctx::AutoPick;
    uint64_t key = 0xcbf29ce484222325ull;
    const uint64_t parts[] = {(uint64_t)p->width, (uint64_t)p->height, (uint64_t)spp, (uint64_t)p->depth,
                              (uint64_t)(p->part_count > 1 ? p->part_count : 1), (uint64_t)(p->part_count > 1 ? p->part_rows : 0), c->scene_gen,
                              (uint64_t)c->n_spheres, (uint64_t)p->tri_mat, (uint64_t)(p->flags & ~(uint32_t)PT_FLAG_WRITE_RGBA),
                              (uint64_t)moments, c->env_gen, c->mat_gen};
    for (uint64_t v : parts) { key ^= v; key *= 0x100000001b3ull; }
    if (key == 0) key = 1;
    int slot = -1, lru = 0;
    for (int i = 0; i < pt_ctx::N_PICKS; i++) {
        if (c->picks[i].key == key) { slot = i; break; }
        if (c->picks[i].used < c->picks[lru].used) lru = i;
    }
    if (slot < 0) {
        slot = lru;
        AP& n = c->picks[slot];
        if (n.phase > 0 && n.phase < AP::DECIDED)
            for (hipEvent_t e : n.e) if (e) (void)hipEventSynchronize(e);
        n.key = key; n.phase = 0; n.choice = PT_KERNEL_PERSISTENT; n.ms[0] = n.ms[1] = 0.f;
    }
    AP& a = c->picks[slot];
    a.used = ++c->pick_tick;
    c->pick_last = slot;
    pick = &a;
    probe = -1;
    (void)auto_decide(c, a, false);
    if (a.phase < AP::TRIALS) {
        for (hipEvent_t& e : a.e)
            if (!e) HIP_TRY(c, hipEventCreate(&e));
        probe = a.phase++;
    }
    return PT_OK;
}

struct CallPlan {
    int kernel;
    int probe;
    pt_ctx::AutoPick* pick;
    bool side;
    bool samples;
    uint32_t sgroup_log2;
    int n_top, sph_tab;
    int chunk, work_tiles;
    LaunchCfg L;
};

static int plan_call(pt_ctx* c, const pt_params* p, const KParams& P, uint32_t spp, bool moments, CallPlan& plan) {
    const TreeState& t = c->tree;
    LaunchCfg& L = plan.L;
    const bool nee = (p->flags & PT_FLAG_NEE) != 0;
    if ((L.walk = choose_walk(c, "pt_render", true)) < 0) return L.walk;
    const bool wave_ok = t.has_bvh && P.depth > 0 && L.walk == 2 && !c->env.texels;
    int kernel = c->opt_kernel;
    plan.probe = -1;
    plan.pick = nullptr;
    if (kernel == PT_KERNEL_AUTO) {
        kernel = PT_KERNEL_PERSISTENT;
        if (wave_ok && !c->opt_counters && !nee) {
            const int rc = auto_lookup(c, p, spp, moments, plan.pick, plan.probe);
            if (rc != PT_OK) return rc;
            if (plan.probe >= 0) kernel = (plan.probe & 1) ? PT_KERNEL_WAVEFRONT : PT_KERNEL_PERSISTENT;
            else if (plan.pick->phase == pt_ctx::AutoPick::DECIDED) kernel = plan.pick->choice;
        }
    }
    if (nee && kernel != PT_KERNEL_MEGA_BVH2)
        kernel = wave_ok && (uint64_t)p->width * (uint64_t)p->height <= (1ull << PT_REC_PIXEL_BITS) ? PT_KERNEL_WAVEFRONT : PT_KERNEL_MEGA_BVH2;
    if (kernel == PT_KERNEL_WAVEFRONT && !wave_ok) kernel = PT_KERNEL_PERSISTENT;
    if (kernel == PT_KERNEL_MEGA_BVH2 && L.walk == 3) kernel = PT_KERNEL_PERSISTENT;
    plan.kernel = kernel;
    const bool persistent = kernel == PT_KERNEL_PERSISTENT, wavefront = kernel == PT_KERNEL_WAVEFRONT;

    bool caller_idle = false;
    if (c->opt_overlap && !wavefront) {
        caller_idle = hipStreamQuery(c->stream) == hipSuccess;
        if (!caller_idle) (void)hipGetLastError();
    }
    plan.side = c->opt_overlap && !wavefront && !c->opt_counters && !c->opt_timing && plan.probe < 0 && !caller_idle;
    plan.samples = spp > 1 || wavefront || plan.side || moments;
    plan.sgroup_log2 = plan.samples && (wavefront || persistent) ? wave_sample_group_log2(spp, c->opt_wave_samples) : 0u;
    plan.work_tiles = P.n_tiles * (plan.samples ? (int)spp : 1);

    L.lstk = c->opt_lstk ? c->opt_lstk : PT_STACK_CAP;
    plan.n_top = t.has_bvh ? (int)std::min<uint32_t>((uint32_t)c->opt_top, L.walk >= 2 ? t.wide_top_layout : t.n_top_layout) : 0;
    if (L.walk >= 1) plan.n_top = 0;
    L.lds = lds_fit(plan.n_top, L.lstk, PT_BLOCK);
    plan.sph_tab = persistent && c->opt_sph_lds ? lds_sphere_table(L.lds) : -1;
    const long slots = (long)plan.work_tiles * 64;
    plan.chunk = queue_chunk(c, (uint64_t)slots);
    const int waves_per_block = PT_BLOCK / 64;
    L.count = c->opt_counters != 0;
    L.occ = c->opt_occ;
    L.blocks = (plan.work_tiles + waves_per_block - 1) / waves_per_block;
    L.work_blocks = (int)((slots + plan.chunk * waves_per_block - 1) / (plan.chunk * waves_per_block));
    L.n_cu = c->n_cu;
    L.moments = moments;
    L.env = c->env.texels ? (c->env.cx ? 2 : 1) : 0;
    return PT_OK;
}

static int side_acquire(pt_ctx* c, pt_ctx::Side*& sd) {
    sd = &c->side[c->side_next];
    c->side_next ^= 1;
    if (sd->stream) return PT_OK;
    int prio_lo = 0, prio_hi = 0;
    HIP_TRY(c, hipDeviceGetStreamPriorityRange(&prio_lo, &prio_hi));
    HIP_TRY(c, hipStreamCreateWithPriority(&sd->stream, hipStreamNonBlocking, prio_hi));
    HIP_TRY(c, hipEventCreateWithFlags(&sd->traced, hipEventDisableTiming));
    HIP_TRY(c, hipEventCreateWithFlags(&sd->folded, hipEventDisableTiming));
    HIP_TRY(c, queue_alloc(&sd->queue));
    return PT_OK;
}

static int samples_reserve(pt_ctx* c, pt_ctx::Side* sd, size_t need, KParams& P) {
    float*& buf = sd ? sd->samples : c->d_samples;
    size_t& have = sd ? sd->samples_bytes : c->samples_bytes;
    if (need > have) {
        HIP_TRY(c, hipStreamSynchronize(c->stream));
        (void)hipFree(buf);
        buf = nullptr;
        have = 0;
        HIP_TRY(c, hipMalloc((void**)&buf, need));
        have = need;
    }
    P.samples = buf;
    return PT_OK;
}

static int side_order(pt_ctx* c, pt_ctx::Side* sd, bool reads_lights) {
    if (sd->fold_pending) HIP_TRY(c, hipStreamWaitEvent(sd->stream, sd->folded, 0));
    if (reads_lights && sd->lights_seen != c->lights_gen) {
        HIP_TRY(c, hipStreamWaitEvent(sd->stream, c->lights_ev, 0));
        sd->lights_seen = c->lights_gen;
    }
    if (sd->geom_seen != c->geom_gen) {
        HIP_TRY(c, hipStreamWaitEvent(sd->stream, c->geom_ev, 0));
        sd->geom_seen = c->geom_gen;
    }
    return PT_OK;
}

static void apply_plan(const pt_ctx* c, const CallPlan& plan, const pt_ctx::Side* sd, KParams& P) {
    P.sgroup_log2 = plan.sgroup_log2;
    if (plan.sgroup_log2) {
        P.smp_ss = 1ull;
        P.smp_ps = P.spp;
    }
    P.sc.stack_n = plan.L.lstk;
    P.sc.top_base = plan.L.walk >= 2 ? P.sc.wide_root : 0;
    P.sc.n_top = plan.n_top;
    P.sph_tab = plan.sph_tab;
    P.chunk = plan.chunk;
    if (plan.kernel == PT_KERNEL_PERSISTENT) queue_params(c, sd ? sd->queue : c->d_queue, P);
}
}

int pt_render(pt_ctx* c, float* accum_dev, uint32_t* rgba_dev, const pt_camera* cam, const pt_params* p, uint32_t spp) {
    return pt_render_moments(c, accum_dev, rgba_dev, nullptr, cam, p, spp);
}

int pt_render_moments(pt_ctx* c, float* accum_dev, uint32_t* rgba_dev, float* moments_dev, const pt_camera* cam, const pt_params* p,
                      uint32_t spp) {
    int rc = check_call(c, accum_dev, rgba_dev, cam, p, spp);
    if (rc != PT_OK) return rc;
    HIP_TRY(c, hipSetDevice(c->device));
    if ((rc = refresh_tri_lights(c, p)) != PT_OK) return rc;
    KParams P;
    if ((rc = fill_params(c, accum_dev, rgba_dev, cam, p, spp, P)) != PT_OK || P.n_tiles <= 0) return rc;
    CallPlan plan;
    if ((rc = plan_call(c, p, P, spp, moments_dev != nullptr, plan)) != PT_OK) return rc;
    const int probe = plan.probe;

    pt_ctx::Side* sd = nullptr;
    if (plan.side && (rc = side_acquire(c, sd)) != PT_OK) return rc;
    if (plan.samples && (rc = samples_reserve(c, sd, (size_t)spp * (size_t)p->width * (size_t)p->height * 3 * sizeof(float), P)) != PT_OK) return rc;
    if (sd && (rc = side_order(c, sd, P.tri_lights != nullptr)) != PT_OK) return rc;
    hipStream_t trace_stream = sd ? sd->stream : c->stream;
    apply_plan(c, plan, sd, P);

    if (c->opt_counters) HIP_TRY(c, hipMemsetAsync(c->d_counters, 0, PT_CNT_N * sizeof(unsigned long long), c->stream));
    if (probe >= 0 && (probe & 1)) {
        rc = wave_reserve(c, P, plan.work_tiles);
        if (rc != PT_OK) return rc;
    }
    if (probe >= 0) HIP_TRY(c, hipEventRecord(plan.pick->e[2 * probe], c->stream));
    HIP_TRY(c, span_begin(c));
    if (c->opt_timing) {
        c->stage_used = 0;
        if (stage_mark(c, PT_STAGE_NONE) != PT_OK) return PT_ERR_DEVICE;
    }
    bool folded = false;
    if (plan.kernel == PT_KERNEL_WAVEFRONT) {
        rc = render_wavefront(c, P, plan.L, plan.work_tiles, folded);
        if (rc != PT_OK) return rc;
    } else if (plan.kernel == PT_KERNEL_PERSISTENT) {
        HIP_TRY(c, queue_reset(P.queue, trace_stream));
        HIP_TRY(c, launch_persist(plan.L, P, trace_stream));
        if (stage_mark(c, PT_STAGE_FRAME) != PT_OK) return PT_ERR_DEVICE;
    } else {
        HIP_TRY(c, launch_mega(plan.L, P, trace_stream));
        if (stage_mark(c, PT_STAGE_FRAME) != PT_OK) return PT_ERR_DEVICE;
    }
    if (sd) {
        HIP_TRY(c, hipEventRecord(sd->traced, sd->stream));
        HIP_TRY(c, hipStreamWaitEvent(c->stream, sd->traced, 0));
    }
    if (P.samples && !folded) {
        HIP_TRY(c, launch_fold(P, (float2*)moments_dev, c->stream));
        if (stage_mark(c, PT_STAGE_FOLD) != PT_OK) return PT_ERR_DEVICE;
    }
    if (sd) {
        HIP_TRY(c, hipEventRecord(sd->folded, c->stream));
        sd->fold_pending = true;
    }
    if (probe >= 0) HIP_TRY(c, hipEventRecord(plan.pick->e[2 * probe + 1], c->stream));
    HIP_TRY(c, span_end(c));
    return PT_OK;
}

int pt_auto_choice(pt_ctx* c, int* kernel, float* ms_persistent, float* ms_wavefront) {
    if (!c || !kernel) return fail(c, PT_ERR_INVALID, "pt_auto_choice: null argument");
    *kernel = PT_KERNEL_AUTO;
    if (ms_persistent) *ms_persistent = 0.f;
    if (ms_wavefront) *ms_wavefront = 0.f;
    if (c->pick_last < 0) return PT_OK;
    pt_ctx::AutoPick& a = c->picks[c->pick_last];
    if (auto_decide(c, a, true)) *kernel = a.choice;
    if (ms_persistent) *ms_persistent = a.ms[0];
    if (ms_wavefront) *ms_wavefront = a.ms[1];
    return PT_OK;
}

int pt_trace_rays(pt_ctx* c, const float* rays_dev, size_t n, int cull, float* t_dev, int32_t* tri_dev, float* normal_dev) {
    if (!c) return fail(nullptr, PT_ERR_INVALID, "null ctx");
    if (!c->tree.has_bvh) return fail(c, PT_ERR_NO_SCENE, "pt_trace_rays: no BVH uploaded");
    if (c->tree.records_woop) return fail(c, PT_ERR_UNSUPPORTED, "pt_trace_rays: the ray-batch kernel reads Moller-Trumbore records (upload with PT_OPT_TRI_TEST 0)");
    if (n == 0) return PT_OK;
    if (!rays_dev || !t_dev || !tri_dev) return fail(c, PT_ERR_INVALID, "pt_trace_rays: null argument");
    HIP_TRY(c, hipSetDevice(c->device));
    KScene sc;
    scene_view(c, sc);
    HIP_TRY(c, span_begin(c));
    const size_t lds = binary_ray_layout(c, sc);
    HIP_TRY(c, launch_rays(sc, lds, (const float4*)rays_dev, n, cull, t_dev, tri_dev, normal_dev, c->stream));
    HIP_TRY(c, span_end(c));
    return PT_OK;
}

static int query_call(pt_ctx* c, const char* who, bool outputs, const ptmi::QueryCall& q) {
    const std::string name(who);
    if (!c) return fail(nullptr, PT_ERR_INVALID, "null ctx");
    if (!c->tree.has_bvh) return fail(c, PT_ERR_NO_SCENE, name + ": no BVH uploaded");
    if (c->tree.records_woop) return fail(c, PT_ERR_UNSUPPORTED, name + ": ray-batch queries read Moller-Trumbore records (upload with PT_OPT_TRI_TEST 0)");
    if (q.n == 0) return PT_OK;
    if (!q.rays || !outputs) return fail(c, PT_ERR_INVALID, name + ": null argument");
    if (q.n >= (1ull << 32)) return fail(c, PT_ERR_INVALID, name + ": more than 2^32 - 1 rays in one call");
    HIP_TRY(c, hipSetDevice(c->device));
    HIP_TRY(c, span_begin(c));
    HIP_TRY(c, launch_query(c, q));
    HIP_TRY(c, span_end(c));
    return PT_OK;
}

int pt_closest_hits(pt_ctx* c, const float* rays_dev, size_t n, int cull, float* t_dev, int32_t* tri_dev, float* normal_dev) {
    return query_call(c, "pt_closest_hits", t_dev && tri_dev, ptmi::QueryCall{rays_dev, n, cull, t_dev, tri_dev, normal_dev, nullptr});
}

int pt_any_hits(pt_ctx* c, const float* rays_dev, size_t n, int cull, uint8_t* hit_dev) {
    return query_call(c, "pt_any_hits", hit_dev != nullptr, ptmi::QueryCall{rays_dev, n, cull, nullptr, nullptr, nullptr, hit_dev});
}

static constexpr uint64_t RAYS_MAX_SLOTS = 1ull << 26;

int pt_render_rays(pt_ctx* c, const float* rays_dev, size_t n_rays, uint64_t first_index, float* radiance_dev, const pt_params* p,
                   uint32_t spp, int mode) {
    if (!c) return fail(nullptr, PT_ERR_INVALID, "null ctx");
    if (!c->tree.has_bvh && c->n_spheres == 0) return fail(c, PT_ERR_NO_SCENE, "pt_render_rays: no scene uploaded");
    if (n_rays == 0 || spp == 0) return PT_OK;
    if (!rays_dev || !radiance_dev || !p) return fail(c, PT_ERR_INVALID, "pt_render_rays: null argument");
    if (mode != PT_RAYS_CLAMPED && mode != PT_RAYS_HDR) return fail(c, PT_ERR_INVALID, "pt_render_rays: mode must be PT_RAYS_CLAMPED or PT_RAYS_HDR");
    if (n_rays >= (1ull << 32)) return fail(c, PT_ERR_INVALID, "pt_render_rays: more than 2^32 - 1 rays in one call");
    if (p->sample_index == 0) return fail(c, PT_ERR_INVALID, "pt_render_rays: sample_index starts at 1");
    if (p->tri_mat < PT_MAT_DIFF || p->tri_mat > PT_MAT_REFR) return fail(c, PT_ERR_INVALID, "pt_render_rays: bad triangle material");
    if ((p->flags & PT_FLAG_NEE) && !(p->flags & PT_FLAG_COSINE_DIFF)) return fail(c, PT_ERR_INVALID, "pt_render_rays: PT_FLAG_NEE needs PT_FLAG_COSINE_DIFF");
    HIP_TRY(c, hipSetDevice(c->device));
    int rc = refresh_tri_lights(c, p);
    if (rc != PT_OK) return rc;
    const int walk = choose_walk(c, "pt_render_rays", false);
    if (walk < 0) return walk;
    KParams P;
    fill_path_params(c, p, spp, P);
    P.sc.stack_n = 16;
    P.sc.top_base = walk >= 2 ? P.sc.wide_root : 0;
    size_t lds = (size_t)16 * PT_BLOCK * 4;
    P.sph_tab = c->opt_sph_lds ? lds_sphere_table(lds) : -1;
    queue_params(c, c->d_queue, P);
    const ptmi::RaysCall R{rays_dev, radiance_dev, first_index, n_rays, mode == PT_RAYS_HDR};
    const uint32_t per_launch = (uint32_t)std::max<uint64_t>(1, std::min<uint64_t>(spp, RAYS_MAX_SLOTS / n_rays));
    if (per_launch > 1 && (rc = samples_reserve(c, nullptr, (size_t)per_launch * n_rays * 3 * sizeof(float), P)) != PT_OK) return rc;
    P.smp_ss = n_rays;
    P.smp_ps = 1u;
    HIP_TRY(c, span_begin(c));
    for (uint32_t s0 = 0; s0 < spp; s0 += per_launch) {
        P.spp = std::min(per_launch, spp - s0);
        P.frame = p->frame + s0;
        P.sample_index = p->sample_index + s0;
        const uint64_t slots = (uint64_t)n_rays * (per_launch > 1 ? P.spp : 1u);
        P.chunk = queue_chunk(c, slots);
        const int work_blocks = (int)std::min<uint64_t>((slots + (uint64_t)P.chunk * 4 - 1) / ((uint64_t)P.chunk * 4), (uint64_t)INT_MAX);
        HIP_TRY(c, queue_reset(P.queue, c->stream));
        HIP_TRY(c, launch_render_rays(c, walk, (p->flags & PT_FLAG_NEE) != 0, lds, work_blocks, P, R));
        if (per_launch > 1) HIP_TRY(c, launch_fold_rays(c, P, R));
    }
    HIP_TRY(c, span_end(c));
    return PT_OK;
}

int pt_get_counters(pt_ctx* c, pt_counters* out) {
    if (!c || !out) return fail(c, PT_ERR_INVALID, "pt_get_counters: null argument");
    unsigned long long h[PT_CNT_WAVE];
    HIP_TRY(c, hipSetDevice(c->device));
    HIP_TRY(c, hipMemcpyAsync(h, c->d_counters, sizeof h, hipMemcpyDeviceToHost, c->stream));
    HIP_TRY(c, hipStreamSynchronize(c->stream));
    out->rays = h[PT_CNT_RAYS]; out->inner = h[PT_CNT_INNER]; out->tris = h[PT_CNT_TRIS]; out->leaves = h[PT_CNT_LEAVES];
    out->hits = h[PT_CNT_HITS]; out->paths = h[PT_CNT_PATHS];
    return PT_OK;
}

int pt_get_wave_stats(pt_ctx* c, uint64_t* out, int n) {
    if (!c || !out || n < 0) return fail(c, PT_ERR_INVALID, "pt_get_wave_stats: bad argument");
    unsigned long long h[PT_CNT_N];
    HIP_TRY(c, hipSetDevice(c->device));
    HIP_TRY(c, hipMemcpyAsync(h, c->d_counters, sizeof h, hipMemcpyDeviceToHost, c->stream));
    HIP_TRY(c, hipStreamSynchronize(c->stream));
    for (int i = 0; i < n && i < PT_WAVE_STATS; i++) out[i] = h[PT_CNT_WAVE + i];
    return PT_OK;
}

int pt_get_stage_ms(pt_ctx* c, float* out, int n) {
    if (!c || !out || n < 0) return fail(c, PT_ERR_INVALID, "pt_get_stage_ms: bad argument");
    if (!c->timed || c->stage_used < 2) return fail(c, PT_ERR_INVALID, "pt_get_stage_ms: no timed pt_render (set PT_OPT_TIMING=1 first)");
    HIP_TRY(c, hipSetDevice(c->device));
    HIP_TRY(c, hipEventSynchronize(c->stage_ev[c->stage_used - 1]));
    for (int i = 0; i < n; i++) out[i] = 0.f;
    for (size_t i = 1; i < c->stage_used; i++) {
        float ms = 0.f;
        HIP_TRY(c, hipEventElapsedTime(&ms, c->stage_ev[i - 1], c->stage_ev[i]));
        const int k = c->stage_kind[i];
        if (k >= 0 && k < n) out[k] += ms;
    }
    return PT_OK;
}

int pt_last_kernel_ms(pt_ctx* c, float* ms) {
    if (!c || !ms) return fail(c, PT_ERR_INVALID, "pt_last_kernel_ms: null argument");
    if (!c->timed) return fail(c, PT_ERR_INVALID, "pt_last_kernel_ms: no timed launch (set PT_OPT_TIMING=1 first)");
    HIP_TRY(c, hipSetDevice(c->device));
    HIP_TRY(c, hipEventSynchronize(c->ev1));
    HIP_TRY(c, hipEventElapsedTime(ms, c->ev0, c->ev1));
    return PT_OK;
}

}
```

g.p.u-pathtracer_amd/tracer.py:

```python
import ctypes as C

import numpy as np

from . import _abi
from ._abi import Camera, Counters, DenoiseParams, Environment, Material, Params, Sphere, TemporalParams

DENOISE_DEFAULTS = dict(iterations=4, sigma_color=0.0, sigma_normal=1.0, sigma_position=0.03)
TEMPORAL_DEFAULTS = dict(max_history=32.0, plane_tolerance=0.02, normal_threshold=0.9)


class PtError(RuntimeError):
    def __init__(self, code, msg):
        super().__init__(f"ptmi error {code}: {msg}")
        self.code = code


class DeviceBuffer:

    def __init__(self, owner, nbytes):
        self.owner, self.nbytes = owner, nbytes
        p = C.c_void_p()
        owner._check(owner._lib.pt_malloc(owner._ctx, nbytes, C.byref(p)))
        self.ptr = p.value

    def zero(self):
        self.owner._check(self.owner._lib.pt_memset(self.owner._ctx, self.ptr, 0, self.nbytes))

    def download(self, dtype, shape):
        out = np.empty(shape, dtype)
        assert out.nbytes <= self.nbytes
        self.owner._check(self.owner._lib.pt_download(self.owner._ctx, out.ctypes.data, self.ptr, out.nbytes))
        return out

    def upload(self, arr):
        a = np.ascontiguousarray(arr)
        assert a.nbytes <= self.nbytes
        self.owner._check(self.owner._lib.pt_upload(self.owner._ctx, self.ptr, a.ctypes.data, a.nbytes))

    def free(self):
        if self.ptr:
            self.owner._lib.pt_free(self.owner._ctx, self.ptr)
            self.ptr = None


class PathTracer:
    def __init__(self, device=0):
        self._lib = _abi.ptmi()
        ctx = C.c_void_p()
        rc = self._lib.pt_create(device, C.byref(ctx))
        if rc != 0:
            raise PtError(rc, self._lib.pt_last_error(None).decode())
        self._ctx = ctx
        self.device = device

    def _check(self, rc):
        if rc != 0:
            raise PtError(rc, self._lib.pt_last_error(self._ctx).decode())

    def close(self):
        if getattr(self, "_ctx", None):
            if getattr(self, "_refit_buf", None) is not None:
                self._refit_buf.free()
                self._refit_buf = None
            self._lib.pt_destroy(self._ctx)
            self._ctx = None

    def __del__(self):
        try:
            self.close()
        except Exception:
            pass

    def set_stream(self, hip_stream_ptr):
        self._check(self._lib.pt_set_stream(self._ctx, hip_stream_ptr))

    def set_option(self, opt, value):
        self._check(self._lib.pt_set_option(self._ctx, opt, int(value)))

    def sync(self):
        self._check(self._lib.pt_sync(self._ctx))

    def malloc(self, nbytes):
        return DeviceBuffer(self, nbytes)

    def upload_bvh(self, bvh):
        n, t, i = (np.ascontiguousarray(bvh.nodes, np.float32), np.ascontiguousarray(bvh.tris, np.float32),
                   np.ascontiguousarray(bvh.index, np.int32))
        self._check(self._lib.pt_upload_bvh(self._ctx, n.ctypes.data, n.size // 4, t.ctypes.data, t.size // 4,
                                            i.ctypes.data, i.size))

    def upload_bvh_arrays(self, nodes, n_node_vec4, tris, n_tri_vec4, index, n_index):
        self._check(self._lib.pt_upload_bvh(self._ctx, nodes, n_node_vec4, tris, n_tri_vec4, index, n_index))

    def upload_spheres(self, spheres):
        n = len(spheres) if spheres is not None else 0
        self._check(self._lib.pt_upload_spheres(self._ctx, spheres if n else None, n))

    def build_bvh(self, mesh):
        v = np.ascontiguousarray(mesh.verts, np.float32)
        t = np.ascontiguousarray(mesh.tris, np.int32)
        self._check(self._lib.pt_build_bvh(self._ctx, v.ctypes.data, len(v), t.ctypes.data, len(t)))
        ms = C.c_float()
        self._check(self._lib.pt_last_build_ms(self._ctx, C.byref(ms)))
        return ms.value

    def refit_bvh(self, tri_verts, n_tris=None, n_dropped=None):
        if isinstance(tri_verts, np.ndarray):
            a = np.ascontiguousarray(tri_verts)
            if a.dtype != np.float32 or a.ndim not in (2, 3) or a.shape[1:] not in ((9,), (3, 3)):
                raise ValueError("refit_bvh: a float32 array of shape (n, 9) or (n, 3, 3) expected")
            if getattr(self, "_refit_buf", None) is None or self._refit_buf.nbytes < a.nbytes:
                if getattr(self, "_refit_buf", None) is not None:
                    self._refit_buf.free()
                self._refit_buf = DeviceBuffer(self, max(a.nbytes, 36))
            self._refit_buf.upload(a)
            ptr, n = self._refit_buf.ptr, len(a)
        elif isinstance(tri_verts, DeviceBuffer):
            ptr, n = tri_verts.ptr, tri_verts.nbytes // 36 if n_tris is None else n_tris
        else:
            if n_tris is None:
                raise ValueError("refit_bvh: a raw device pointer needs n_tris")
            ptr, n = tri_verts, n_tris
        nd = n_dropped.ptr if isinstance(n_dropped, DeviceBuffer) else n_dropped
        self._check(self._lib.pt_refit_bvh(self._ctx, ptr, int(n), nd))

    def upload_tri_materials(self, table, tri_material):
        if table is None or len(table) == 0:
            self._check(self._lib.pt_upload_tri_materials(self._ctx, None, 0, None, 0))
            return
        arr = (Material * len(table))(*table)
        ids = np.ascontiguousarray(tri_material, np.int32)
        self._check(self._lib.pt_upload_tri_materials(self._ctx, arr, len(table), ids.ctypes.data_as(C.POINTER(C.c_int32)), len(ids)))

    def scene_info(self):
        a, b, c_, e = C.c_uint64(), C.c_uint64(), C.c_uint64(), C.c_uint64()
        d = C.c_uint32()
        self._check(self._lib.pt_scene_info(self._ctx, C.byref(a), C.byref(b), C.byref(c_), C.byref(d), C.byref(e)))
        return {"n_inner": a.value, "n_tri_refs": b.value, "n_leaves": c_.value, "max_depth": d.value,
                "device_bytes": e.value}

    def alloc_frame(self, width, height):
        acc = self.malloc(width * height * 12)
        acc.zero()
        rgba = self.malloc(width * height * 4)
        rgba.zero()
        return acc, rgba

    def launch_kernel(self, accum_ptr, rgba_ptr, cam, params, spp=1, moments_ptr=None):
        if moments_ptr is None:
            self._check(self._lib.pt_render(self._ctx, accum_ptr, rgba_ptr, C.byref(cam), C.byref(params), spp))
        else:
            self._check(self._lib.pt_render_moments(self._ctx, accum_ptr, rgba_ptr, moments_ptr, C.byref(cam), C.byref(params), spp))

    def frame_error(self, moments_ptr, width, height, n_samples, threshold=0.0):
        mean, above = C.c_double(), C.c_uint64()
        self._check(self._lib.pt_frame_error(self._ctx, moments_ptr, int(width), int(height), int(n_samples), float(threshold),
                                             C.byref(mean), C.byref(above)))
        return mean.value, above.value

    def trace_rays(self, rays_ptr, n, cull, t_ptr, tri_ptr, normal_ptr=None):
        self._check(self._lib.pt_trace_rays(self._ctx, rays_ptr, n, int(cull), t_ptr, tri_ptr, normal_ptr))

    def closest_hits(self, rays_ptr, n, cull, t_ptr, tri_ptr, normal_ptr=None):
        self._check(self._lib.pt_closest_hits(self._ctx, rays_ptr, n, int(cull), t_ptr, tri_ptr, normal_ptr))

    def any_hits(self, rays_ptr, n, cull, hit_ptr):
        self._check(self._lib.pt_any_hits(self._ctx, rays_ptr, n, int(cull), hit_ptr))

    def render_rays(self, rays_ptr, n, out_ptr, params, spp=1, first_index=0, hdr=False):
        self._check(self._lib.pt_render_rays(self._ctx, rays_ptr, int(n), int(first_index), out_ptr, C.byref(params), int(spp),
                                             _abi.RAYS_HDR if hdr else _abi.RAYS_CLAMPED))

    def upload_environment(self, texels, front=(0, 0, -1), right=(1, 0, 0), up=(0, 1, 0), scale=(1, 1, 1), filter=_abi.ENV_BILINEAR, light=False):
        a = np.ascontiguousarray(texels, np.float32)
        if a.ndim != 3 or a.shape[2] != 3:
            raise ValueError("upload_environment: a float32 array of shape (H, W, 3) expected")
        ev = Environment()
        ev.width, ev.height = a.shape[1], a.shape[0]
        ev.front[:], ev.right[:], ev.up[:], ev.scale[:] = front, right, up, scale
        ev.filter = int(filter)
        self.set_option(_abi.OPT_ENV_LIGHT, 1 if light else 0)
        try:
            self._check(self._lib.pt_upload_environment(self._ctx, C.byref(ev), a.ctypes.data))
        finally:
            self.set_option(_abi.OPT_ENV_LIGHT, 0)

    def clear_environment(self):
        self._check(self._lib.pt_upload_environment(self._ctx, None, None))

    def eval_environment(self, rays_ptr, n, out_ptr):
        self._check(self._lib.pt_eval_environment(self._ctx, rays_ptr, int(n), out_ptr))

    def environment_is_light(self):
        out = C.c_int(0)
        self._check(self._lib.pt_environment_is_light(self._ctx, C.byref(out)))
        return bool(out.value)

    def sample_environment(self, u_ptr, n, dir_pdf_ptr, radiance_ptr=None):
        self._check(self._lib.pt_sample_environment(self._ctx, u_ptr, int(n), dir_pdf_ptr, radiance_ptr))

    def environment_pdf(self, rays_ptr, n, pdf_ptr):
        self._check(self._lib.pt_environment_pdf(self._ctx, rays_ptr, int(n), pdf_ptr))

    def render_aux(self, cam, params, albedo_ptr, normal_ptr, position_ptr, id_ptr=None):
        self._check(self._lib.pt_render_aux(self._ctx, C.byref(cam), C.byref(params), albedo_ptr, normal_ptr, position_ptr, id_ptr))

    def denoise(self, color_ptr, albedo_ptr, normal_ptr, position_ptr, width, height, out_ptr, rgba_ptr=None,
                iterations=DENOISE_DEFAULTS["iterations"], sigma_color=DENOISE_DEFAULTS["sigma_color"],
                sigma_normal=DENOISE_DEFAULTS["sigma_normal"], sigma_position=DENOISE_DEFAULTS["sigma_position"]):
        dp = DenoiseParams(int(width), int(height), int(iterations), float(sigma_color), float(sigma_normal), float(sigma_position))
        self._check(self._lib.pt_denoise(self._ctx, C.byref(dp), color_ptr, albedo_ptr, normal_ptr, position_ptr, out_ptr, rgba_ptr))

    def temporal(self, width, height, prev_cam, prev_color_ptr, prev_length_ptr, prev_normal_ptr, prev_position_ptr, prev_id_ptr,
                 cur_color_ptr, cur_normal_ptr, cur_position_ptr, cur_id_ptr, out_color_ptr, out_length_ptr, rgba_ptr=None,
                 max_history=TEMPORAL_DEFAULTS["max_history"], plane_tolerance=TEMPORAL_DEFAULTS["plane_tolerance"],
                 normal_threshold=TEMPORAL_DEFAULTS["normal_threshold"]):
        tp = TemporalParams(int(width), int(height), float(max_history), float(plane_tolerance), float(normal_threshold), 0)
        self._check(self._lib.pt_temporal(self._ctx, C.byref(tp), C.byref(prev_cam) if prev_cam is not None else None,
                                          prev_color_ptr, prev_length_ptr, prev_normal_ptr, prev_position_ptr, prev_id_ptr,
                                          cur_color_ptr, cur_normal_ptr, cur_position_ptr, cur_id_ptr, out_color_ptr, out_length_ptr, rgba_ptr))

    def counters(self):
        c = Counters()
        self._check(self._lib.pt_get_counters(self._ctx, C.byref(c)))
        return {f: getattr(c, f) for f, _ in Counters._fields_}

    def stage_ms(self):
        out = (C.c_float * 6)()
        self._check(self._lib.pt_get_stage_ms(self._ctx, out, 6))
        return dict(zip(("none", "frame", "generate", "extend", "shade", "fold"), [float(v) for v in out]))

    def auto_choice(self):
        k, a, b = C.c_int(), C.c_float(), C.c_float()
        self._check(self._lib.pt_auto_choice(self._ctx, C.byref(k), C.byref(a), C.byref(b)))
        return k.value, a.value, b.value

    def tree_cost(self):
        a, b = C.c_double(), C.c_double()
        self._check(self._lib.pt_tree_cost(self._ctx, C.byref(a), C.byref(b)))
        return a.value, b.value

    def tree_items(self):
        p, nb, nr, nw, d = C.c_void_p(), C.c_uint64(), C.c_uint64(), C.c_uint64(), C.c_uint32()
        self._check(self._lib.pt_tree_items(self._ctx, C.byref(p), C.byref(nb), C.byref(nr), C.byref(nw), C.byref(d)))
        n = nb.value + nr.value + nw.value
        buf = np.empty((n, 16), np.float32)
        self._check(self._lib.pt_download(self._ctx, buf.ctypes.data, p.value, buf.nbytes))
        return buf[:nb.value], buf[nb.value:nb.value + nr.value], buf[nb.value + nr.value:], d.value

    def wave_stats(self):
        out = (C.c_uint64 * 11)()
        self._check(self._lib.pt_get_wave_stats(self._ctx, out, 11))
        names = ("it_node", "act_node", "it_rec", "act_rec", "it_shade", "act_shade", "it_begin", "act_begin", "it_loop", "stack_overflows",
                 "walk_free")
        return dict(zip(names, [int(v) for v in out]))

    def last_build_ms(self):
        ms = C.c_float()
        if self._lib.pt_last_build_ms(self._ctx, C.byref(ms)) != 0:
            return -1.0
        return ms.value

    def last_kernel_ms(self):
        ms = C.c_float()
        self._check(self._lib.pt_last_kernel_ms(self._ctx, C.byref(ms)))
        return ms.value


class TemporalHistory:

    def __init__(self, tracer, width, height, with_ids=True):
        self.t, self.W, self.H = tracer, int(width), int(height)
        n = self.W * self.H
        self.color = [tracer.malloc(n * 12) for _ in range(2)]
        self.length = [tracer.malloc(n * 4) for _ in range(2)]
        self.guides = [[tracer.malloc(n * 16) for _ in range(3)] + [tracer.malloc(n * 4) if with_ids else None] for _ in range(2)]
        self.cam = None
        self.cur = 0

    def reset(self):
        self.cam = None

    def _ptrs(self, k):
        return [b.ptr if b is not None else None for b in self.guides[k]]

    def push(self, cam, params, color_ptr, rgba_ptr=None, **temporal):
        k, o = self.cur, 1 - self.cur
        alb, nrm, pos, ids = self._ptrs(k)
        self.t.render_aux(cam, params, alb, nrm, pos, ids)
        if self.cam is None:
            prev = (None,) * 6
        else:
            _, pn, pp, pi = self._ptrs(o)
            prev = (self.cam, self.color[o].ptr, self.length[o].ptr, pn, pp, pi)
        self.t.temporal(self.W, self.H, *prev, color_ptr, nrm, pos, ids, self.color[k].ptr, self.length[k].ptr, rgba_ptr, **temporal)
        self.cam = Camera.from_buffer_copy(cam)
        self.cur = o
        return self.color[k].ptr, self.length[k].ptr, (alb, nrm, pos, ids)

    def free(self):
        for b in self.color + self.length + [x for gset in self.guides for x in gset if x is not None]:
            b.free()
        self.color, self.length, self.guides, self.cam = [], [], [], None


def algorithmic_bytes(counters, n_spheres):
    return (64 * counters["inner"] + 48 * counters["tris"] + 16 * counters["leaves"] + 4 * counters["hits"]
            + 44 * n_spheres * counters["rays"] + 28 * counters["paths"])
```

include/ptmi.h:

```cpp
#ifndef PTMI_H
#define PTMI_H

#include <stddef.h>
#include <stdint.h>

#ifdef __cplusplus
extern "C" {
#endif

#define PTMI_ABI_VERSION 3

typedef struct pt_ctx pt_ctx;

typedef enum pt_status {
    PT_OK = 0,
    PT_ERR_INVALID = -1,
    PT_ERR_DEVICE = -2,
    PT_ERR_NO_SCENE = -3,
    PT_ERR_NOMEM = -4,
    PT_ERR_UNSUPPORTED = -5
} pt_status;

enum { PT_MAT_DIFF = 0, PT_MAT_METAL = 1, PT_MAT_SPEC = 2, PT_MAT_REFR = 3 };

enum {
    PT_FLAG_METAL_LITERAL_W = 1u << 0,
    PT_FLAG_WRITE_RGBA = 1u << 1,
    PT_FLAG_FACE_FORWARD = 1u << 2,
    PT_FLAG_COSINE_DIFF = 1u << 3,
    PT_FLAG_GLASS_FIX = 1u << 4,
    PT_FLAG_RUSSIAN_ROULETTE = 1u << 5,
    PT_FLAG_RR_CPU_TRACER = 1u << 7,
    PT_FLAG_NEE = 1u << 8,
    PT_FLAG_MISS_KEEPS_PATH = 1u << 6
};
#define PT_FLAGS_SMALLPT (PT_FLAG_FACE_FORWARD | PT_FLAG_COSINE_DIFF | PT_FLAG_RUSSIAN_ROULETTE | PT_FLAG_MISS_KEEPS_PATH)
#define PT_FLAGS_CPU_TRACER (PT_FLAG_FACE_FORWARD | PT_FLAG_COSINE_DIFF | PT_FLAG_RR_CPU_TRACER | PT_FLAG_MISS_KEEPS_PATH)

enum {
    PT_KERNEL_AUTO = 0,
    PT_KERNEL_MEGA_BVH2 = 1,
    PT_KERNEL_PERSISTENT = 3,
    PT_KERNEL_WAVEFRONT = 5
};

enum {
    PT_OPT_KERNEL = 1,
    PT_OPT_COUNTERS = 2,
    PT_OPT_TIMING = 3,
    PT_OPT_BATCH = 4,
    PT_OPT_TOP_NODES = 5,
    PT_OPT_OCCUPANCY = 6,
    PT_OPT_LDS_STACK = 7,
    PT_OPT_WALK = 8,
    PT_OPT_REFILL = 11,
    PT_OPT_VOTE_NODE = 12,
    PT_OPT_VOTE_REC = 13,
    PT_OPT_WAVE_BATCH = 14,
    PT_OPT_SPHERE_LDS = 15,
    PT_OPT_WAVE_BLOCKS = 19,
    PT_OPT_WAVE_SAMPLES = 25,
    PT_OPT_FIRST_WALK = 26,
    PT_OPT_PACKET_STACK = 27,
    PT_OPT_OVERLAP = 21,
    PT_OPT_BUILD_ALGO = 16,
    PT_OPT_REBUILD = 17,
    PT_OPT_OPTIMIZE = 24,
    PT_OPT_PRESPLIT = 18,
    PT_OPT_TRI_TEST = 10,
    PT_OPT_LEAF_MAX = 9,
    PT_OPT_FUSE_STAGES = 28,
    PT_OPT_LAST_ANYHIT = 29,
    PT_OPT_ROOT_CULL = 30,
    PT_OPT_ROOT_ENTRY = 33,
    PT_OPT_PATH_HISTORY = 34,
    PT_OPT_ENV_LIGHT = 35
};

typedef struct pt_camera {
    float pos[3];
    float front[3];
    float right[3];
    float up[3];
    float dist;
    float aspect;
    float fov;
    float _pad;
} pt_camera;

typedef struct pt_sphere {
    float pos_rad[4];
    float emi[3];
    float col[3];
    int32_t mat;
} pt_sphere;

typedef struct pt_params {
    int32_t width, height;
    uint32_t depth;
    int32_t cull_backfaces;
    uint64_t frame;
    uint64_t sample_index;
    int32_t tri_mat;
    float tri_col[3];
    float tri_emi[3];
    float bk_color[3];
    float air_ior;
    float glass_ior;
    float phong_expo;
    uint32_t flags;
    int32_t part_index, part_count, part_rows;
    int32_t _pad;
} pt_params;

typedef struct pt_counters {
    uint64_t rays;
    uint64_t inner;
    uint64_t tris;
    uint64_t leaves;
    uint64_t hits;
    uint64_t paths;
} pt_counters;

int pt_abi_version(void);
int pt_device_count(void);
int pt_create(int device, pt_ctx** out);
int pt_destroy(pt_ctx* ctx);
const char* pt_last_error(const pt_ctx* ctx);
int pt_set_stream(pt_ctx* ctx, void* hip_stream);
int pt_set_option(pt_ctx* ctx, int option, int value);
int pt_sync(pt_ctx* ctx);

int pt_malloc(pt_ctx* ctx, size_t bytes, void** dev_out);
int pt_free(pt_ctx* ctx, void* dev);
int pt_memset(pt_ctx* ctx, void* dev, int value, size_t bytes);
int pt_download(pt_ctx* ctx, void* host_dst, const void* dev_src, size_t bytes);
int pt_upload(pt_ctx* ctx, void* dev_dst, const void* host_src, size_t bytes);

int pt_upload_bvh(pt_ctx* ctx,
                  const float* nodes, size_t n_node_vec4,
                  const float* tri_verts, size_t n_tri_vec4,
                  const int32_t* tri_index, size_t n_index);
int pt_upload_spheres(pt_ctx* ctx, const pt_sphere* spheres, size_t n_spheres);

int pt_build_bvh(pt_ctx* ctx, const float* verts, size_t n_verts, const int32_t* tris, size_t n_tris);
int pt_last_build_ms(pt_ctx* ctx, float* ms_out);

int pt_refit_bvh(pt_ctx* ctx, const float* tri_verts_dev, size_t n_tris, uint32_t* n_dropped_dev);

typedef struct pt_material {
    float col[3];
    float emi[3];
    int32_t mat;
    float phong_expo;
} pt_material;
int pt_upload_tri_materials(pt_ctx* ctx, const pt_material* table, size_t n_materials,
                            const int32_t* tri_material, size_t n_tris);

int pt_render(pt_ctx* ctx, float* accum_dev, uint32_t* rgba_dev,
              const pt_camera* cam, const pt_params* params, uint32_t spp);

int pt_render_moments(pt_ctx* ctx, float* accum_dev, uint32_t* rgba_dev, float* moments_dev,
                      const pt_camera* cam, const pt_params* params, uint32_t spp);

int pt_frame_error(pt_ctx* ctx, const float* moments_dev, int32_t width, int32_t height,
                   uint64_t n_samples, float threshold, double* mean_rse, uint64_t* n_above);

int pt_trace_rays(pt_ctx* ctx, const float* rays_dev, size_t n_rays, int cull_backfaces,
                  float* t_dev, int32_t* tri_dev, float* normal_dev);

int pt_closest_hits(pt_ctx* ctx, const float* rays_dev, size_t n_rays, int cull_backfaces,
                    float* t_dev, int32_t* tri_dev, float* normal_dev);
int pt_any_hits(pt_ctx* ctx, const float* rays_dev, size_t n_rays, int cull_backfaces,
                uint8_t* hit_dev);

enum { PT_RAYS_CLAMPED = 0, PT_RAYS_HDR = 1 };
int pt_render_rays(pt_ctx* ctx, const float* rays_dev, size_t n_rays, uint64_t first_index,
                   float* radiance_dev, const pt_params* params, uint32_t spp, int mode);

enum { PT_ENV_NEAREST = 0, PT_ENV_BILINEAR = 1 };
typedef struct pt_environment {
    int32_t width, height;
    float front[3], right[3], up[3];
    float scale[3];
    int32_t filter;
    int32_t _pad;
} pt_environment;
int pt_upload_environment(pt_ctx* ctx, const pt_environment* env, const float* texels );
int pt_eval_environment(pt_ctx* ctx, const float* rays_dev, size_t n_rays, float* radiance_dev );
int pt_environment_is_light(pt_ctx* ctx, int* out);
int pt_sample_environment(pt_ctx* ctx, const float* u_dev, size_t n, float* dir_pdf_dev, float* radiance_dev);
int pt_environment_pdf(pt_ctx* ctx, const float* rays_dev, size_t n, float* pdf_dev);

int pt_render_aux(pt_ctx* ctx, const pt_camera* cam, const pt_params* params,
                  float* albedo_dev, float* normal_dev, float* position_dev, int32_t* id_dev);

typedef struct pt_denoise_params {
    int32_t width, height;
    int32_t iterations;
    float sigma_color, sigma_normal, sigma_position;
} pt_denoise_params;
int pt_denoise(pt_ctx* ctx, const pt_denoise_params* dp, const float* color_dev,
               const float* albedo_dev, const float* normal_dev, const float* position_dev,
               float* out_dev, uint32_t* rgba_dev);

typedef struct pt_temporal_params {
    int32_t width, height;
    float max_history;
    float plane_tolerance;
    float normal_threshold;
    int32_t _pad;
} pt_temporal_params;
int pt_temporal(pt_ctx* ctx, const pt_temporal_params* tp, const pt_camera* prev_cam,
                const float* prev_color_dev, const float* prev_length_dev,
                const float* prev_normal_dev, const float* prev_position_dev, const int32_t* prev_id_dev,
                const float* cur_color_dev,
                const float* cur_normal_dev, const float* cur_position_dev, const int32_t* cur_id_dev,
                float* out_color_dev, float* out_length_dev, uint32_t* rgba_dev);

int pt_get_counters(pt_ctx* ctx, pt_counters* out);
#define PT_WAVE_STATS 11
int pt_get_wave_stats(pt_ctx* ctx, uint64_t* out, int n);
int pt_last_kernel_ms(pt_ctx* ctx, float* ms_out);
enum {
    PT_STAGE_NONE = 0,
    PT_STAGE_FRAME = 1,
    PT_STAGE_GENERATE = 2,
    PT_STAGE_EXTEND = 3,
    PT_STAGE_SHADE = 4,
    PT_STAGE_FOLD = 5,
    PT_STAGE_COUNT = 6
};
int pt_get_stage_ms(pt_ctx* ctx, float* out, int n);
int pt_auto_choice(pt_ctx* ctx, int* kernel, float* ms_persistent, float* ms_wavefront);
int pt_tree_cost(pt_ctx* ctx, double* node_visits, double* tri_tests);
int pt_tree_items(pt_ctx* ctx, const void** items_dev, uint64_t* n_binary, uint64_t* n_records,
                  uint64_t* n_wide, uint32_t* wide_depth);
int pt_scene_info(pt_ctx* ctx, uint64_t* n_inner, uint64_t* n_tri_refs,
                  uint64_t* n_leaves, uint32_t* max_depth, uint64_t* device_bytes);

#ifdef __cplusplus
}
#endif
#endif
```

Measured before the change: 17970 Mrays/s.

## Pre-test last any-hit rays against a few large occluder triangles

```diff
diff --git a/g.p.u-pathtracer_amd/_abi.py b/g.p.u-pathtracer_amd/_abi.py
--- a/g.p.u-pathtracer_amd/_abi.py
+++ b/g.p.u-pathtracer_amd/_abi.py
@@ -85,6 +85,8 @@
 OPT_ROOT_ENTRY = 33
 OPT_PATH_HISTORY = 34
 OPT_ENV_LIGHT = 35
+OPT_LAST_OCCLUDERS = 36
+OCCLUDERS_MAX = 12
 
 _vp, _sz, _i, _u32 = C.c_void_p, C.c_size_t, C.c_int, C.c_uint32
 PTMI_SYMBOLS = [
@@ -121,6 +123,7 @@
     ("pt_build_bvh", _i, [_vp, _vp, C.c_size_t, _vp, C.c_size_t]),
     ("pt_last_build_ms", _i, [_vp, C.POINTER(C.c_float)]),
     ("pt_refit_bvh", _i, [_vp, _vp, _sz, _vp]),
+    ("pt_occluder_ids", _i, [_vp, _sz, _vp, _sz, _vp, _i]),
     ("pt_upload_tri_materials", _i, [_vp, C.POINTER(Material), C.c_size_t, C.POINTER(C.c_int32), C.c_size_t]),
     ("pt_get_counters", _i, [_vp, C.POINTER(Counters)]),
     ("pt_get_wave_stats", _i, [_vp, C.POINTER(C.c_uint64), _i]),
diff --git a/g.p.u-pathtracer_amd/csrc/pt_ctx.h b/g.p.u-pathtracer_amd/csrc/pt_ctx.h
--- a/g.p.u-pathtracer_amd/csrc/pt_ctx.h
+++ b/g.p.u-pathtracer_amd/csrc/pt_ctx.h
@@ -15,6 +15,10 @@
 #ifndef PT_FIRST_WALK_DEFAULT
 #define PT_FIRST_WALK_DEFAULT 1
 #endif
+#ifndef PT_OCCLUDERS_MAX
+#define PT_OCCLUDERS_MAX 12
+#endif
+#define PT_OCCLUDER_AREA_DIV 24
 
 struct TreeState {
     float4* d_nodes = nullptr;
@@ -28,6 +32,8 @@
     int32_t max_tri_id = -1;
     float build_ms = -1.f;
     double opt_cost[2] = {0.0, 0.0};
+    int32_t occ_ids[PT_OCCLUDERS_MAX] = {};
+    uint32_t n_occ = 0;
 };
 
 struct DevTree {
@@ -98,6 +104,7 @@
     int opt_root_cull = 1;
     int opt_root_entry = 1;
     int opt_env_light = 0;
+    int opt_last_occluders = 1;
     int opt_path_history = 1;
     struct AutoPick {
         static constexpr int TRIALS = 4, PENDING = 4, DECIDED = 5;
@@ -115,6 +122,7 @@
     uint64_t scene_gen = 0;
     uint64_t geom_gen = 0;
     hipEvent_t geom_ev = nullptr;
+    float4* d_occ = nullptr;
     struct Refit {
         uint64_t scene_gen = 0;
         const float4* items = nullptr;
@@ -202,6 +210,7 @@
         if (P.ksph[i].mat == PT_MAT_REFR) return false;
     return true;
 }
+inline bool last_occluders_hold(const TreeState& t, bool anyhit_launch, bool root_cull) { return anyhit_launch && root_cull && t.n_occ > 0; }
 inline void scene_view(const pt_ctx* c, KScene& sc, pt_sphere_d* ksph = nullptr) {
     sc = KScene();
     sc.nodes = sc.tris = c->tree.d_nodes;
@@ -302,6 +311,9 @@
 int stage_mark(pt_ctx* c, int kind_of_work_since_last_mark);
 int build_bvh_impl(pt_ctx* c, const float* verts, size_t n_verts, const int32_t* tris, size_t n_tris, DevTree& out,
                    const int32_t* id_map = nullptr);
+struct OccTri { int32_t id; const float *v0, *v1, *v2; };
+int select_occluders(std::vector<OccTri>& tris, int32_t* ids, int cap);
+int occluders_collect(pt_ctx* c);
 void refit_release(pt_ctx* c);
 void denoise_release(pt_ctx* c);
 void env_release(pt_ctx* c);
diff --git a/g.p.u-pathtracer_amd/csrc/pt_k_wave.hip b/g.p.u-pathtracer_amd/csrc/pt_k_wave.hip
--- a/g.p.u-pathtracer_amd/csrc/pt_k_wave.hip
+++ b/g.p.u-pathtracer_amd/csrc/pt_k_wave.hip
@@ -294,10 +294,26 @@
     return make_float2(sh.t, __int_as_float(sh.sph_id));
 }
 
-template <bool BOUND>
+__device__ __forceinline__ bool wf_occluded(const KParams& P, bool walker, const PathState& ps, float ts) {
+    const float4* tab = P.wf.s_con;
+    const float t_max = wf_anyhit_start(ts);
+    const bool cull = P.cull != 0;
+    bool open = walker, hit = false;
+    for (int a = 0; a < 3 * PT_OCCLUDERS_MAX && __ballot(open) != 0ull; a += 3) {
+        const float4 q0 = pt_uld4(tab, a), q1 = pt_uld4(tab, a + 1), q2 = pt_uld4(tab, a + 2);
+        const float t = pt_mt_intersect(V3(q0.x, q0.y, q0.z), V3(q1.x, q1.y, q1.z), V3(q2.x, q2.y, q2.z), ps.o, ps.d, cull);
+        if (open && t > 0.0f && t < t_max) { hit = true; open = false; }
+        if (__float_as_int(q1.w) != 0) break;
+    }
+    return hit;
+}
+
+template <bool BOUND, bool OCCL = false>
 __device__ __forceinline__ int wf_survivor_slot(const KParams& P, bool alive, const PathState& ps, float ts, bool& walk_free, int& n_walk,
-                                                int& total, int* s_cnt, int* s_cnt_free, uint32_t& entry) {
+                                                int& total, int* s_cnt, int* s_cnt_free, uint32_t& entry, bool& occluded) {
+    static_assert(BOUND || !OCCL, "only a last segment is an any-hit query");
     walk_free = false;
+    occluded = false;
     entry = 0u;
     if (P.wf.root_cull) {
         const WideNode root = wide_node_load_uniform(P.sc, P.sc.wide_root);
@@ -314,6 +330,10 @@
             }
         }
     }
+    if constexpr (OCCL) {
+        occluded = wf_occluded(P, alive && !walk_free, ps, ts);
+        if (occluded) { walk_free = true; entry = 0u; }
+    }
     const int r = PT_SURVIVOR_RANK(P, alive && !walk_free, ps, n_walk, s_cnt);
     total = n_walk;
     if (!P.wf.root_cull) return r;
@@ -334,7 +354,7 @@
     }
 }
 
-template <bool COUNT, bool NEE, bool FIRST, bool LAST = false, int FOLD = 0, bool BOUND = false, bool HIST = false>
+template <bool COUNT, bool NEE, bool FIRST, bool LAST = false, int FOLD = 0, bool BOUND = false, bool HIST = false, bool OCCL = false>
 __global__ void __launch_bounds__(PT_BLOCK) k_wf_shade(const KParams P) {
     __shared__ int s_cnt[PT_BLOCK / 64];
     __shared__ int s_cnt2[PT_BLOCK / 64];
@@ -427,9 +447,17 @@
         return;
     }
     int n_walk, total;
-    bool walk_free;
+    bool walk_free, occluded;
     uint32_t entry;
-    const int r = wf_survivor_slot<BOUND>(P, alive, ps, bound.x, walk_free, n_walk, total, s_cnt, s_cnt_free, entry);
+    const int r = wf_survivor_slot<BOUND, OCCL>(P, alive, ps, bound.x, walk_free, n_walk, total, s_cnt, s_cnt_free, entry, occluded);
+    if constexpr (OCCL) bound.x = occluded ? 0.0f : bound.x;
+    if (COUNT && OCCL) {
+        const unsigned long long no = (unsigned long long)__popcll(__ballot(occluded));
+        if ((threadIdx.x & 63) == 0 && no) {
+            atomicAdd(&P.counters[PT_CNT_OCCLUDED], no);
+            atomicAdd(&P.counters[PT_CNT_WALK_FREE], 0ull - no);
+        }
+    }
     if (alive) {
         const size_t j = (size_t)region * PT_REGION + (size_t)r;
         pt_sst4(P.wf.ray0_out + j, make_float4(ps.o.x, ps.o.y, ps.o.z, ps.d.x));
@@ -496,7 +524,7 @@
     }
 }
 
-template <bool BOUND, bool HIST = false>
+template <bool BOUND, bool HIST = false, bool OCCL = false>
 __global__ void __launch_bounds__(PT_BLOCK, 8) k_wf_extend_packet_shade(const KParams P) {
     __shared__ int s_cnt[PT_BLOCK / 64];
     __shared__ int s_cnt_free[PT_BLOCK / 64];
@@ -523,9 +551,10 @@
     float2 bound = make_float2(PT_F32_MAX, __int_as_float(-1));
     if (BOUND && alive) bound = wf_sphere_bound(P, ps);
     int n_walk, total;
-    bool walk_free;
+    bool walk_free, occluded;
     uint32_t entry;
-    const int r = wf_survivor_slot<BOUND>(P, alive, ps, bound.x, walk_free, n_walk, total, s_cnt, s_cnt_free, entry);
+    const int r = wf_survivor_slot<BOUND, OCCL>(P, alive, ps, bound.x, walk_free, n_walk, total, s_cnt, s_cnt_free, entry, occluded);
+    if constexpr (OCCL) bound.x = occluded ? 0.0f : bound.x;
     if (alive) {
         const size_t j = (size_t)region * PT_REGION + (size_t)r;
         pt_sst4(P.wf.ray0_out + j, make_float4(ps.o.x, ps.o.y, ps.o.z, ps.d.x));
@@ -649,6 +678,7 @@
     bool root_cull;
     bool root_entry;
     bool history;
+    bool occluders;
     WaveExtend extend(uint32_t b, uint32_t depth) const {
         if (b == 0) return fuse_first ? EXT_FUSED : packet ? EXT_PACKET : EXT_FIRST;
         return anyhit && b + 1 == depth ? EXT_ANY : EXT_CLOSEST;
@@ -672,6 +702,7 @@
                P.sc.n_spheres <= PT_KSPHERES && !c->tree.records_woop;
     p.root_cull = L.count ? c->opt_root_cull == 2 : c->opt_root_cull >= 1;
     p.history = (L.count ? c->opt_path_history == 2 : c->opt_path_history >= 1) && path_history_holds(P);
+    p.occluders = (L.count ? c->opt_last_occluders == 2 : c->opt_last_occluders >= 1) && last_occluders_hold(c->tree, p.anyhit, p.root_cull);
     p.root_entry = p.root_cull && !nee && P.spp < PT_REC_MAX_SAMPLES_ENTRY && (L.count ? c->opt_root_entry == 2 : c->opt_root_entry >= 1);
     return p;
 }
@@ -685,7 +716,9 @@
     const size_t n_reg = (size_t)Q.wf.n_regions;
     if (kind == EXT_FUSED)
         return with_bool(p.history, [&](auto hist) {
-            return p.anyhit && Q.depth == 2 ? plain(k_wf_extend_packet_shade<true, hist()>, n_reg, WF_LDS_SHADE) : plain(k_wf_extend_packet_shade<false, hist()>, n_reg, WF_LDS_SHADE);
+            if (p.anyhit && Q.depth == 2)
+                return with_bool(p.occluders, [&](auto occl) { return plain(k_wf_extend_packet_shade<true, hist(), occl()>, n_reg, WF_LDS_SHADE); });
+            return plain(k_wf_extend_packet_shade<false, hist()>, n_reg, WF_LDS_SHADE);
         });
     if (kind == EXT_PACKET) {
 #ifdef PT_PACKET_RESIDENT_GRID
@@ -724,14 +757,14 @@
         if (p.count) {
             if (kind == SHADE_LAST_ANY) return go(k_wf_shade_last_any<true, 0, hist()>);
             return with_bool(first, [&](auto f) {
-                if (kind == SHADE_BOUND) return go(k_wf_shade<true, false, f(), false, 0, true, hist()>);
+                if (kind == SHADE_BOUND) return with_bool(p.occluders, [&](auto occl) { return go(k_wf_shade<true, false, f(), false, 0, true, hist(), occl()>); });
                 return go(k_wf_shade<true, false, f(), false, 0, false, hist()>);
             });
         }
         if (kind == SHADE_LAST_ANY) return with_int<4, 2, 1, 0>(p.fold_lp, [&](auto lp) { return go(k_wf_shade_last_any<false, lp(), hist()>); });
         if (kind == SHADE_LAST) return with_int<4, 2, 1, 0>(p.fold_lp, [&](auto lp) { return go(k_wf_shade<false, false, false, true, lp(), false, hist()>); });
         return with_bool(first, [&](auto f) {
-            if (kind == SHADE_BOUND) return go(k_wf_shade<false, false, f(), false, 0, true, hist()>);
+            if (kind == SHADE_BOUND) return with_bool(p.occluders, [&](auto occl) { return go(k_wf_shade<false, false, f(), false, 0, true, hist(), occl()>); });
             return go(k_wf_shade<false, false, f(), false, 0, false, hist()>);
         });
     });
@@ -755,7 +788,7 @@
         P.wf.s_con = (float4*)(buf.nee + 2 * w.b_ray);
         P.wf.s_hit = (float2*)(buf.nee + 3 * w.b_ray);
         P.wf.s_cnt = (int*)(buf.nee + 3 * w.b_ray + w.b_hit);
-    }
+    } else P.wf.s_con = plan.occluders ? c->d_occ : nullptr;
 
     hipStream_t st = c->stream;
     P.sc.n_top = 0;
diff --git a/g.p.u-pathtracer_amd/csrc/pt_kernels.h b/g.p.u-pathtracer_amd/csrc/pt_kernels.h
--- a/g.p.u-pathtracer_amd/csrc/pt_kernels.h
+++ b/g.p.u-pathtracer_amd/csrc/pt_kernels.h
@@ -181,6 +181,7 @@
     PT_CNT_IT_BEGIN, PT_CNT_ACT_BEGIN,
     PT_CNT_IT_LOOP, PT_CNT_STACK_OVF,
     PT_CNT_WALK_FREE,
+    PT_CNT_OCCLUDED,
     PT_CNT_N,
     PT_CNT_PACKET_GROUPS = PT_CNT_IT_SHADE,
     PT_CNT_ANY_RAYS = PT_CNT_ACT_SHADE
diff --git a/g.p.u-pathtracer_amd/csrc/pt_refit.hip b/g.p.u-pathtracer_amd/csrc/pt_refit.hip
--- a/g.p.u-pathtracer_amd/csrc/pt_refit.hip
+++ b/g.p.u-pathtracer_amd/csrc/pt_refit.hip
@@ -350,6 +350,7 @@
                            R.wide_list + R.wide_off[ht], nw);
     }
     HIP_TRY(c, hipGetLastError());
+    if (const int rc = occluders_collect(c); rc != PT_OK) { c->tree.n_occ = 0; return rc; }
     HIP_TRY(c, span_end(c));
     if (!c->geom_ev) HIP_TRY(c, hipEventCreateWithFlags(&c->geom_ev, hipEventDisableTiming));
     HIP_TRY(c, hipEventRecord(c->geom_ev, st));
diff --git a/g.p.u-pathtracer_amd/csrc/pt_tree.hip b/g.p.u-pathtracer_amd/csrc/pt_tree.hip
--- a/g.p.u-pathtracer_amd/csrc/pt_tree.hip
+++ b/g.p.u-pathtracer_amd/csrc/pt_tree.hip
@@ -55,7 +55,58 @@
     if (i == 0) out[0] = root;
 }
 
+struct OccList { int32_t id[PT_OCCLUDERS_MAX]; uint32_t n = 0; };
+__global__ void __launch_bounds__(256) k_collect_occluders(const float4* __restrict__ rec, uint32_t n_rec, const OccList L, float4* __restrict__ table) {
+    const uint32_t i = blockIdx.x * 256u + threadIdx.x;
+    if (i >= n_rec) return;
+    const float4 q0 = rec[4 * (size_t)i];
+    const int id = __float_as_int(q0.w);
+    for (uint32_t k = 0; k < L.n; k++) {
+        if (L.id[k] != id) continue;
+        const float4 q1 = rec[4 * (size_t)i + 1], q2 = rec[4 * (size_t)i + 2];
+        table[3 * k + 0] = q0;
+        table[3 * k + 1] = make_float4(q1.x, q1.y, q1.z, __int_as_float(k + 1 == L.n ? 1 : 0));
+        table[3 * k + 2] = q2;
+    }
+}
+
 namespace ptmi {
+int select_occluders(std::vector<OccTri>& tris, int32_t* ids, int cap) {
+    std::stable_sort(tris.begin(), tris.end(), [](const OccTri& a, const OccTri& b) { return a.id < b.id; });
+    tris.erase(std::unique(tris.begin(), tris.end(), [](const OccTri& a, const OccTri& b) { return a.id == b.id; }), tris.end());
+    std::vector<double> area(tris.size());
+    double total = 0.0;
+    for (size_t i = 0; i < tris.size(); i++) {
+        const OccTri& t = tris[i];
+        const double a[3] = {(double)t.v1[0] - t.v0[0], (double)t.v1[1] - t.v0[1], (double)t.v1[2] - t.v0[2]};
+        const double b[3] = {(double)t.v2[0] - t.v0[0], (double)t.v2[1] - t.v0[1], (double)t.v2[2] - t.v0[2]};
+        const double x = a[1] * b[2] - a[2] * b[1], y = a[2] * b[0] - a[0] * b[2], z = a[0] * b[1] - a[1] * b[0];
+        area[i] = 0.5 * std::sqrt(x * x + y * y + z * z);
+        total += area[i];
+    }
+    std::vector<size_t> big;
+    for (size_t i = 0; i < tris.size(); i++)
+        if (area[i] * (double)PT_OCCLUDER_AREA_DIV >= total && area[i] > 0.0) big.push_back(i);
+    std::stable_sort(big.begin(), big.end(), [&](size_t a, size_t b) { return area[a] > area[b]; });
+    const int n = (int)std::min<size_t>(big.size(), (size_t)std::max(cap, 0));
+    for (int k = 0; k < n; k++) ids[k] = tris[big[(size_t)k]].id;
+    return n;
+}
+
+int occluders_collect(pt_ctx* c) {
+    const TreeState& t = c->tree;
+    if (t.n_occ == 0 || !t.has_bvh || t.records_woop) return PT_OK;
+    if (!c->d_occ) HIP_TRY(c, hipMalloc((void**)&c->d_occ, 3 * PT_OCCLUDERS_MAX * sizeof(float4)));
+    OccList L;
+    L.n = t.n_occ;
+    std::memcpy(L.id, t.occ_ids, sizeof L.id);
+    const uint32_t n_rec = (uint32_t)t.n_refs;
+    HIP_TRY(c, hipMemsetAsync(c->d_occ, 0, 3 * PT_OCCLUDERS_MAX * sizeof(float4), c->stream));
+    hipLaunchKernelGGL(k_collect_occluders, dim3((n_rec + 255) / 256), dim3(256), 0, c->stream, t.d_nodes + 4 * (size_t)t.n_inner, n_rec, L, c->d_occ);
+    HIP_TRY(c, hipGetLastError());
+    return PT_OK;
+}
+
 
 static int tree_cost(pt_ctx* c, const TreeState& t, double* node_visits, double* tri_tests) {
     const unsigned n_blocks = (unsigned)((t.n_wide + 255) / 256);
@@ -131,14 +182,18 @@
     return rc;
 }
 
-static int adopt_tree(pt_ctx* c, DevTree&& t) {
+static int adopt_tree(pt_ctx* c, DevTree&& t, const OccList& occ) {
     HIP_TRY(c, hipSetDevice(c->device));
     HIP_TRY(c, hipStreamSynchronize(c->stream));
     refit_release(c);
     (void)hipFree(c->tree.d_nodes);
     c->tree = t.release();
     c->scene_gen++;
-    return PT_OK;
+    c->tree.n_occ = c->tree.records_woop ? 0u : occ.n;
+    std::memcpy(c->tree.occ_ids, occ.id, sizeof occ.id);
+    const int rc = occluders_collect(c);
+    if (rc != PT_OK) c->tree.n_occ = 0;
+    return rc;
 }
 }
 
@@ -161,6 +216,13 @@
     for (const ptscene::Ref& r : T.refs) max_id = std::max(max_id, r.id);
     if (c->d_tri_matid && (size_t)max_id >= c->n_tri_matid)
         return fail(c, PT_ERR_INVALID, "pt_upload_bvh: the triangle-material array on this context does not cover this BVH's triangle ids (clear or re-upload it first)");
+    OccList occ;
+    {
+        std::vector<OccTri> soup;
+        soup.reserve(T.refs.size());
+        for (const ptscene::Ref& r : T.refs) soup.push_back({r.id, r.v, r.v + 3, r.v + 6});
+        occ.n = (uint32_t)select_occluders(soup, occ.id, PT_OCCLUDERS_MAX);
+    }
     const int rebuild = c->opt_tri_test == 0 ? c->opt_rebuild : 0;
     std::vector<int32_t> ids;
     std::vector<float> verts;
@@ -190,7 +252,7 @@
         if (reclustered(b) == PT_OK && tree_cost(c, b.s, &cost_b, &unused) == PT_OK && cost_b < cost_a) a = std::move(b);
         else c->err.clear();
     }
-    return adopt_tree(c, std::move(a));
+    return adopt_tree(c, std::move(a), occ);
 }
 
 int pt_build_bvh(pt_ctx* c, const float* verts, size_t n_verts, const int32_t* tris, size_t n_tris) {
@@ -202,7 +264,26 @@
         for (size_t i = 0; i < 3 * n_tris; i++) std::memcpy(&flat[3 * i], verts + 3 * (size_t)tris[i], 3 * sizeof(float));
         rc = optimise_device_tree(c, t, flat.data(), nullptr, n_tris);
     }
-    return rc == PT_OK ? adopt_tree(c, std::move(t)) : rc;
+    if (rc != PT_OK) return rc;
+    OccList occ;
+    {
+        std::vector<OccTri> soup(n_tris);
+        for (size_t i = 0; i < n_tris; i++)
+            soup[i] = {(int32_t)i, verts + 3 * (size_t)tris[3 * i], verts + 3 * (size_t)tris[3 * i + 1], verts + 3 * (size_t)tris[3 * i + 2]};
+        occ.n = (uint32_t)select_occluders(soup, occ.id, PT_OCCLUDERS_MAX);
+    }
+    return adopt_tree(c, std::move(t), occ);
+}
+
+int pt_occluder_ids(const float* verts, size_t n_verts, const int32_t* tris, size_t n_tris, int32_t* ids_out, int cap) {
+    if (!verts || !tris || !ids_out || cap < 0) return fail(nullptr, PT_ERR_INVALID, "pt_occluder_ids: null array or negative cap");
+    std::vector<OccTri> soup(n_tris);
+    for (size_t i = 0; i < n_tris; i++) {
+        for (int k = 0; k < 3; k++)
+            if (tris[3 * i + k] < 0 || (size_t)tris[3 * i + k] >= n_verts) return fail(nullptr, PT_ERR_INVALID, "pt_occluder_ids: vertex index out of range");
+        soup[i] = {(int32_t)i, verts + 3 * (size_t)tris[3 * i], verts + 3 * (size_t)tris[3 * i + 1], verts + 3 * (size_t)tris[3 * i + 2]};
+    }
+    return select_occluders(soup, ids_out, std::min(cap, PT_OCCLUDERS_MAX));
 }
 
 int pt_last_build_ms(pt_ctx* c, float* ms) {
diff --git a/g.p.u-pathtracer_amd/csrc/ptmi.hip b/g.p.u-pathtracer_amd/csrc/ptmi.hip
--- a/g.p.u-pathtracer_amd/csrc/ptmi.hip
+++ b/g.p.u-pathtracer_amd/csrc/ptmi.hip
@@ -99,6 +99,7 @@
     {PT_OPT_LAST_ANYHIT, &pt_ctx::opt_last_anyhit, OptionRow::RANGE, {0, 2}, PT_ERR_INVALID, "pt_set_option: last any-hit must be 0 (off), 1 (product launches) or 2 (instrumented launches too)"},
     {PT_OPT_ROOT_CULL, &pt_ctx::opt_root_cull, OptionRow::RANGE, {0, 2}, PT_ERR_INVALID, "pt_set_option: root cull must be 0 (off), 1 (product launches) or 2 (instrumented launches too)"},
     {PT_OPT_ROOT_ENTRY, &pt_ctx::opt_root_entry, OptionRow::RANGE, {0, 2}, PT_ERR_INVALID, "pt_set_option: root entry must be 0 (off), 1 (product launches) or 2 (instrumented launches too)"},
+    {PT_OPT_LAST_OCCLUDERS, &pt_ctx::opt_last_occluders, OptionRow::RANGE, {0, 2}, PT_ERR_INVALID, "pt_set_option: last occluders must be 0 (off), 1 (product launches) or 2 (instrumented launches too)"},
     {PT_OPT_ENV_LIGHT, &pt_ctx::opt_env_light, OptionRow::RANGE, {0, 1}, PT_ERR_INVALID, "pt_set_option: env light must be 0 (the map is no light) or 1 (sampled under PT_FLAG_NEE)"},
     {PT_OPT_PATH_HISTORY, &pt_ctx::opt_path_history, OptionRow::RANGE, {0, 2}, PT_ERR_INVALID, "pt_set_option: path history must be 0 (off), 1 (product launches) or 2 (instrumented launches too)"},
 };
@@ -150,6 +151,7 @@
     (void)hipFree(c->d_mat_table);
     (void)hipFree(c->d_light_slot);
     (void)hipFree(c->d_tri_lights);
+    (void)hipFree(c->d_occ);
     (void)hipFree(c->d_counters);
     (void)hipFree(c->d_queue);
     (void)hipFree(c->d_samples);
diff --git a/g.p.u-pathtracer_amd/tracer.py b/g.p.u-pathtracer_amd/tracer.py
--- a/g.p.u-pathtracer_amd/tracer.py
+++ b/g.p.u-pathtracer_amd/tracer.py
@@ -249,10 +249,10 @@
         return buf[:nb.value], buf[nb.value:nb.value + nr.value], buf[nb.value + nr.value:], d.value
 
     def wave_stats(self):
-        out = (C.c_uint64 * 11)()
-        self._check(self._lib.pt_get_wave_stats(self._ctx, out, 11))
+        out = (C.c_uint64 * 12)()
+        self._check(self._lib.pt_get_wave_stats(self._ctx, out, 12))
         names = ("it_node", "act_node", "it_rec", "act_rec", "it_shade", "act_shade", "it_begin", "act_begin", "it_loop", "stack_overflows",
-                 "walk_free")
+                 "walk_free", "occluded")
         return dict(zip(names, [int(v) for v in out]))
 
     def last_build_ms(self):
diff --git a/include/ptmi.h b/include/ptmi.h
--- a/include/ptmi.h
+++ b/include/ptmi.h
@@ -74,7 +74,8 @@
     PT_OPT_ROOT_CULL = 30,
     PT_OPT_ROOT_ENTRY = 33,
     PT_OPT_PATH_HISTORY = 34,
-    PT_OPT_ENV_LIGHT = 35
+    PT_OPT_ENV_LIGHT = 35,
+    PT_OPT_LAST_OCCLUDERS = 36
 };
 
 typedef struct pt_camera {
@@ -147,6 +148,7 @@
 int pt_last_build_ms(pt_ctx* ctx, float* ms_out);
 
 int pt_refit_bvh(pt_ctx* ctx, const float* tri_verts_dev, size_t n_tris, uint32_t* n_dropped_dev);
+int pt_occluder_ids(const float* verts, size_t n_verts, const int32_t* tris, size_t n_tris, int32_t* ids_out, int cap);
 
 typedef struct pt_material {
     float col[3];
@@ -219,7 +221,7 @@
                 float* out_color_dev, float* out_length_dev, uint32_t* rgba_dev);
 
 int pt_get_counters(pt_ctx* ctx, pt_counters* out);
-#define PT_WAVE_STATS 11
+#define PT_WAVE_STATS 12
 int pt_get_wave_stats(pt_ctx* ctx, uint64_t* out, int n);
 int pt_last_kernel_ms(pt_ctx* ctx, float* ms_out);
 enum {
```

New measurement: 18870 Mrays/s (median of 6 runs). 5.0% higher.
